# hjanime/recoup

Hardware: NVIDIA B200
Metric: reads/s through coverage + profileMatrix (reads -> per-base coverage -> regions x bins) (higher is better)
Workload: dtype int32 coverage / f64 matrix

## Files before the change

### recoup_b200/csrc/coverage_split.cu

```cuda
#include <algorithm>
#include <cstdlib>
#include <chrono>
#include <cstdio>

#include <type_traits>
#include <vector>

#include <cooperative_groups.h>

#include "cov_common.cuh"
#include "r_rng.cuh"
#include "rcp_internal.cuh"

namespace rcp {

using namespace covk;

namespace {

constexpr int BLK_SHIFT = 14;
#ifndef RCP_SUB_SHIFT
#define RCP_SUB_SHIFT 10
#endif
constexpr int SUB_SHIFT = RCP_SUB_SHIFT;
constexpr int NG = 1024;
constexpr int RING = 32;
constexpr int CH = 16;
#ifndef RCP_SPLIT_ST
#define RCP_SPLIT_ST 1024
#endif
constexpr int ST = RCP_SPLIT_ST;
constexpr int ROUND_VEC = 2048;
constexpr int VPT = ROUND_VEC / ST;
constexpr int SLAB = 64;
constexpr int MIN_P = 16, MAX_P = 22;
constexpr int GT = 1024;
constexpr int CS = 1024;
constexpr int WT = 7 * ROW;
constexpr int WT_ONE = SMALL_MAX;
static_assert(NG % ST == 0 && ROUND_VEC % ST == 0, "the flush phase maps thread t to the groups t, t + ST, ...");
static_assert(RING == 2 * CH, "a ring holds two chunks");
static_assert(SLAB >= 64, "one flush phase of a warp needs up to 64 chunks");

__device__ __forceinline__ void sp_mark_block(uint32_t* __restrict__ tab, uint32_t b) {
    atomicOr(tab + (b >> 4), 1u << (b & 15u));
    if (b > 0) atomicOr(tab + ((b - 1u) >> 4), 0x10000u << ((b - 1u) & 15u));
}

__global__ void __launch_bounds__(CTA)
sp_plan_kernel(int64_t R, const int32_t* __restrict__ chrom, const int32_t* __restrict__ start,
               const int32_t* __restrict__ end, const int8_t* __restrict__ strand,
               const uint32_t* __restrict__ chrom_off, const int64_t* __restrict__ chrom_len,
               int n_chrom, int ignore_strand, int strand_filter, uint32_t* __restrict__ gs_out,
               int32_t* __restrict__ plen, uint8_t* __restrict__ flags, int64_t* __restrict__ ntile,
               int64_t* __restrict__ padded, uint32_t* __restrict__ tab, unsigned int* __restrict__ err,
               unsigned long long* __restrict__ pstats ,
               unsigned long long* __restrict__ zero5 ) {
    const int64_t r = (int64_t)blockIdx.x * CTA + threadIdx.x;
    if (r < 5) zero5[r] = 0ull;
    unsigned long long my_len = 0;
    if (r < R) {
        const int st = strand ? (int)strand[r] : 0;
        uint32_t gs;
        int64_t L;
        const bool null = window_geometry(chrom[r], start[r], end[r], n_chrom, chrom_off, chrom_len,
                                          err, &gs, &L);
        const int32_t len = null ? 0 : (int32_t)L;
        gs_out[r] = gs;
        plen[r] = len;
        flags[r] = (uint8_t)((st < 0 ? 1u : 0u) | (class_mask(st, ignore_strand, strand_filter) << 1));
        ntile[r] = len > WT_ONE ? ((int64_t)len + WT - 1) / WT : (len > 0 ? 1 : 0);
        padded[r] = ((int64_t)len + PAD - 1) / PAD * PAD;
        my_len = (unsigned long long)len;
        if (len > 0) {
            const uint32_t b1 = (gs + (uint32_t)len - 1u) >> BLK_SHIFT;
            for (uint32_t b = gs >> BLK_SHIFT; b <= b1; b++) sp_mark_block(tab, b);
        }
    }
    unsigned long long my_max = my_len, my_inv = my_len ? 0x100000000ull - my_len : 0ull;
    for (int d = 16; d > 0; d >>= 1) {
        my_len += __shfl_xor_sync(0xffffffffu, my_len, d);
        my_max = max(my_max, __shfl_xor_sync(0xffffffffu, my_max, d));
        my_inv = max(my_inv, __shfl_xor_sync(0xffffffffu, my_inv, d));
    }
    if ((threadIdx.x & 31) == 0 && my_len) {
        atomicAdd(&pstats[0], my_len);
        atomicMax(&pstats[1], my_max);
        atomicMax(&pstats[2], my_inv);
    }
}

__device__ __forceinline__ int64_t sp_owner_of(const int64_t* __restrict__ off, int64_t R, int64_t t) {
    int64_t lo = 0, hi = R;
    while (hi - lo > 1) {
        const int64_t mid = lo + ((hi - lo) >> 1);
        if (__ldg(off + mid) <= t) lo = mid;
        else hi = mid;
    }
    return lo;
}

struct __align__(16) SpDesc {
    int64_t out;
    uint32_t c0;
    uint32_t n;
    int32_t tlen;
    uint32_t cts;
    uint32_t flags;
    uint32_t region;
};

__global__ void __launch_bounds__(CTA)
sp_tiles_kernel(int64_t R, int64_t T, const int64_t* __restrict__ off_tile, const uint32_t* __restrict__ gs,
                const int32_t* __restrict__ plen, const uint8_t* __restrict__ flags,
                const int64_t* __restrict__ cov_off ,
                const int32_t* __restrict__ edge, int n_bins,
                uint32_t max_w, uint32_t pmask, const uint32_t* __restrict__ boff, SpDesc* __restrict__ desc,
                uint32_t* __restrict__ tabs,
                const uint32_t* __restrict__ lxs, const uint32_t* __restrict__ lmax, uint32_t ln,
                uint2* __restrict__ lrange, unsigned long long* __restrict__ bound) {
    const int64_t t = (int64_t)blockIdx.x * CTA + threadIdx.x;
    const unsigned live = __ballot_sync(0xffffffffu, t < T);
    if (t >= T) return;
    const int64_t r = sp_owner_of(off_tile, R, t);
    const int L = plen[r];
    uint32_t o_lo = 0, tlen = (uint32_t)L;
    if (L > WT_ONE) {
        o_lo = (uint32_t)(t - off_tile[r]) * WT;
        tlen = (uint32_t)min(WT, L - (int)o_lo);
    }
    const uint32_t q0 = (flags[r] & 1u) ? (uint32_t)L - o_lo - tlen : o_lo;
    const uint32_t tstart = gs[r] + q0;
    const uint32_t first = tstart >= max_w ? tstart - max_w + 1u : 0u;
    SpDesc d;
    d.out = cov_off ? cov_off[r] + o_lo : (int64_t)o_lo;
    if (!cov_off) {
        int a = 0, b = n_bins;
        while (b - a > 1) {
            const int mid = (a + b) >> 1;
            if (__ldg(edge + mid) <= (int)o_lo) a = mid;
            else b = mid;
        }
        d.out |= (int64_t)a << 32;
    }
    d.c0 = __ldg(boff + (first >> SUB_SHIFT));
    d.n = __ldg(boff + ((tstart + tlen - 1u) >> SUB_SHIFT) + 1u) - d.c0;
    d.tlen = (int32_t)tlen;
    d.cts = tstart & pmask;
    d.flags = flags[r];
    d.region = (uint32_t)r;
    desc[t] = d;
    uint32_t most = d.n;
    if (ln) {
        tabs[t] = tstart;
        const uint32_t hi = tstart + tlen - 1u;
        uint32_t a = 0, b = ln;
        while (a < b) {
            const uint32_t mid = a + ((b - a) >> 1);
            if (__ldg(lxs + mid) < hi + 1u) a = mid + 1;
            else b = mid;
        }
        const uint32_t c1 = a;
        a = 0;
        b = c1;
        while (a < b) {
            const uint32_t mid = a + ((b - a) >> 1);
            if (__ldg(lmax + mid) < tstart + 1u) a = mid + 1;
            else b = mid;
        }
        lrange[t] = make_uint2(a, c1);
        most = most + (c1 - a) < most ? 0xffffffffu : most + (c1 - a);
    }
    if (bound) {
        most = __reduce_max_sync(live, most);
        if ((threadIdx.x & 31) == 0) atomicMax(bound, (unsigned long long)most);
    }
}

__device__ __forceinline__ uint2 lds64(uint32_t a) {
    uint2 v;
    asm volatile("ld.shared.v2.u32 {%0, %1}, [%2];" : "=r"(v.x), "=r"(v.y) : "r"(a));
    return v;
}
__device__ __forceinline__ uint32_t lds32(uint32_t a) {
    uint32_t v;
    asm volatile("ld.shared.u32 %0, [%1];" : "=r"(v) : "r"(a));
    return v;
}
__device__ __forceinline__ uint4 lds128(uint32_t a) {
    uint4 v;
    asm volatile("ld.shared.v4.u32 {%0, %1, %2, %3}, [%4];" : "=r"(v.x), "=r"(v.y), "=r"(v.z), "=r"(v.w) : "r"(a));
    return v;
}
__device__ __forceinline__ void sts32(uint32_t a, uint32_t v) {
    asm volatile("st.shared.u32 [%0], %1;" ::"r"(a), "r"(v) : "memory");
}
__device__ __forceinline__ void sts64(uint32_t a, uint32_t x, uint32_t y) {
    asm volatile("st.shared.v2.u32 [%0], {%1, %2};" ::"r"(a), "r"(x), "r"(y) : "memory");
}
__device__ __forceinline__ int lds_s8(uint32_t a) {
    int v;
    asm volatile("ld.shared.s8 %0, [%1];" : "=r"(v) : "r"(a));
    return v;
}
__device__ __forceinline__ void sts8(uint32_t a, int v) {
    asm volatile("st.shared.u8 [%0], %1;" ::"r"(a), "r"(v) : "memory");
}
__device__ __forceinline__ uint32_t atoms_add(uint32_t a, uint32_t v) {
    uint32_t old;
    asm volatile("atom.shared.add.u32 %0, [%1], %2;" : "=r"(old) : "r"(a), "r"(v) : "memory");
    return old;
}

struct SplitOut {
    uint32_t* pool;
    uint16_t* meta;
    uint32_t* pool_next;
};

constexpr size_t sp_split_smem(int words) {
    return (size_t)NG * RING * 4 + (size_t)NG * 4 + (size_t)words * 4;
}
constexpr size_t SP_SMEM_MAX = 232448;

template <bool STRANDED>
__global__ void __launch_bounds__(ST, 1)
sp_split_kernel(int64_t n, const uint32_t* __restrict__ g_start, const uint32_t* __restrict__ g_end1,
                const int8_t* __restrict__ strand, const uint32_t* __restrict__ tab_g, int words, int P,
                uint32_t max_pack_w, SplitOut out) {
    extern __shared__ __align__(16) unsigned char sp_smem[];
    const int tid = threadIdx.x;
    const unsigned lane = tid & 31, lt = (1u << lane) - 1u;
    const uint32_t ring_a = (uint32_t)__cvta_generic_to_shared(sp_smem);
    const uint32_t cnt_a = ring_a + NG * RING * 4;
    const uint32_t tab_a = cnt_a + NG * 4;
    for (int i = tid; i < words; i += ST) sts32(tab_a + i * 4, tab_g[i]);
    for (int i = tid; i < NG; i += ST) sts32(cnt_a + i * 4, 0u);
    __syncthreads();
    const uint32_t pmask = (1u << P) - 1u;
    const int wsh = STRANDED ? P + 2 : P;
    uint32_t slab_next = 0, slab_end = 0;
    uint32_t spare = 0;
    bool have_spare = false;
    bool hot = false;

    uint32_t a_rem = 0, a_old = 0, a_new = 0;
    auto alloc = [&](uint32_t total) {
        a_rem = slab_end - slab_next;
        a_old = slab_next;
        a_new = 0;
        if (total > a_rem) {
            if (!have_spare && lane == 0) spare = atomicAdd(out.pool_next, (uint32_t)SLAB);
            a_new = __shfl_sync(0xffffffffu, spare, 0);
            have_spare = false;
            slab_next = a_new + (total - a_rem);
            slab_end = a_new + SLAB;
        } else {
            slab_next += total;
        }
        if (!have_spare && slab_end - slab_next < (uint32_t)SLAB / 2) {
            if (lane == 0) spare = atomicAdd(out.pool_next, (uint32_t)SLAB);
            have_spare = true;
        }
    };
    auto chunk_at = [&](uint32_t i) { return i < a_rem ? a_old + i : a_new + (i - a_rem); };

    auto flush_phase = [&](bool final_pass) {
#pragma unroll 1
        for (int grp = tid; grp < NG; grp += ST) {
            const uint32_t w = lds32(cnt_a + grp * 4);
            const uint32_t raw = w & 0xffffu, start = w >> 16;
            const uint32_t nn = min(raw, (uint32_t)RING);
            const uint32_t k = final_pass ? (nn > 0u ? 1u : 0u) : nn / CH;
            const unsigned m1 = __ballot_sync(0xffffffffu, k >= 1u), m2 = __ballot_sync(0xffffffffu, k >= 2u);
            const uint32_t total = __popc(m1) + __popc(m2);
            if (total) {
                const uint32_t idx = __popc(m1 & lt) + __popc(m2 & lt);
                alloc(total);
                for (uint32_t j = 0; j < k; j++) {
                    const uint32_t c = chunk_at(idx + j);
                    const uint32_t src = ring_a + (uint32_t)grp * RING * 4 + (((start + CH * j) & (RING - 1)) << 2);
                    uint4* dst = reinterpret_cast<uint4*>(out.pool + (size_t)c * CH);
                    const uint4 a = lds128(src), b = lds128(src + 16), cc = lds128(src + 32), d = lds128(src + 48);
                    __stcs(dst, a);
                    __stcs(dst + 1, b);
                    __stcs(dst + 2, cc);
                    __stcs(dst + 3, d);
                    out.meta[c] = (uint16_t)(((uint32_t)grp << 5) | (final_pass ? nn : (uint32_t)CH));
                }
            }
            if (k || raw > (uint32_t)RING)
                sts32(cnt_a + grp * 4, final_pass ? 0u : ((((start + CH * k) & (RING - 1)) << 16) | (nn - CH * k)));
        }
    };

    auto keep_read = [&](uint32_t s, uint32_t e1) -> bool {
        const uint32_t t = lds32(tab_a + ((s >> (BLK_SHIFT + 2)) & 0xfffffffcu)) >> ((s >> BLK_SHIFT) & 15u);
        const bool cross = ((e1 - 1u) >> BLK_SHIFT) != (s >> BLK_SHIFT);
        return ((t & 1u) | (cross & ((t >> 16) & 1u))) & (e1 - s <= max_pack_w);
    };
    auto pack = [&](uint32_t s, uint32_t e1, int st) -> uint32_t {
        uint32_t word = (s & pmask) | ((e1 - s) << wsh);
        if (STRANDED) word |= (st > 0 ? 0u : (st < 0 ? 1u : 2u)) << P;
        return word;
    };
    auto insert = [&](uint32_t g, uint32_t pk) -> bool {
        const uint32_t old = atoms_add(cnt_a + g * 4, 1u);
        const uint32_t slot = old & 0xffffu;
        if (slot >= (uint32_t)RING) return false;
        sts32(ring_a + g * (RING * 4) + ((((old >> 16) + slot) & (RING - 1)) << 2), pk);
        return true;
    };
    auto direct = [&](bool want, uint32_t g, uint32_t pk) -> bool {
        const unsigned mo = __ballot_sync(0xffffffffu, want);
        if (mo == 0u) return want;
        const uint32_t g0 = __shfl_sync(0xffffffffu, g, __ffs(mo) - 1);
        const uint32_t nact = __popc(mo);
        if (nact < (uint32_t)CH || !__all_sync(0xffffffffu, !want || g == g0)) return want;
        const uint32_t nfull = nact / CH;
        alloc(nfull);
        const uint32_t r = __popc(mo & lt);
        if (want && r < nfull * CH) {
            const uint32_t c = chunk_at(r / CH);
            out.pool[(size_t)c * CH + (r & (CH - 1))] = pk;
            if ((r & (CH - 1)) == 0) out.meta[c] = (uint16_t)((g0 << 5) | (uint32_t)CH);
            return false;
        }
        return want;
    };

    constexpr int RPT = 4 * VPT;
    uint32_t fg[RPT], fp[RPT];
    uint32_t nf = 0;
    auto take = [&](uint32_t sv, uint32_t ev, int tv) {
        const uint32_t g = sv >> P, pk = pack(sv, ev, tv);
        bool want = keep_read(sv, ev);
        if (hot) want = direct(want, g, pk);
        if (want && !insert(g, pk)) {
            fg[nf] = g;
            fp[nf] = pk;
            nf++;
        }
    };
    auto finish_round = [&]() {
        for (;;) {
            hot = hot || __any_sync(0xffffffffu, nf != 0u);
            const int any = __syncthreads_or(nf != 0u);
            flush_phase(false);
            __syncthreads();
            if (!any) break;
            uint32_t mx = nf;
            for (int d = 16; d > 0; d >>= 1) mx = max(mx, __shfl_xor_sync(0xffffffffu, mx, d));
            uint32_t kept = 0;
            for (uint32_t i = 0; i < mx; i++) {
                const bool mine = i < nf;
                const uint32_t g = mine ? fg[i] : 0u, pk = mine ? fp[i] : 0u;
                bool want = mine;
                if (hot) want = direct(want, g, pk);
                if (want && !insert(g, pk)) {
                    fg[kept] = g;
                    fp[kept] = pk;
                    kept++;
                }
            }
            nf = kept;
        }
    };

    __shared__ int next_round[2];
    const int64_t n_vec = n >> 2;
    const int rounds = (int)((n_vec + ROUND_VEC - 1) / ROUND_VEC);
    if (tid == 0) {
        next_round[0] = (int)atomicAdd(out.pool_next + 1, 1u);
        next_round[1] = (int)atomicAdd(out.pool_next + 1, 1u);
    }
    __syncthreads();
    int round = next_round[0], nr = next_round[1];
    __syncthreads();
    uint4 s4[VPT], e4[VPT];
    char4 t4[VPT];
    auto load = [&](int rd, int h) {
        const int64_t v = (int64_t)rd * ROUND_VEC + h * ST + tid;
        s4[h] = e4[h] = make_uint4(0, 0, 0, 0);
        t4[h] = make_char4(0, 0, 0, 0);
        if (rd < rounds && v < n_vec) {
            s4[h] = __ldcs(reinterpret_cast<const uint4*>(g_start) + v);
            e4[h] = __ldcs(reinterpret_cast<const uint4*>(g_end1) + v);
            if (STRANDED && strand) t4[h] = __ldcs(reinterpret_cast<const char4*>(strand) + v);
        }
    };
#pragma unroll
    for (int h = 0; h < VPT; h++) load(round, h);
    for (int it = 0; round < rounds; it++) {
        unsigned after = 0;
        if (tid == 0) after = atomicAdd(out.pool_next + 1, 1u);
#pragma unroll
        for (int h = 0; h < VPT; h++) {
            take(s4[h].x, e4[h].x, t4[h].x);
            take(s4[h].y, e4[h].y, t4[h].y);
            take(s4[h].z, e4[h].z, t4[h].z);
            take(s4[h].w, e4[h].w, t4[h].w);
            load(nr, h);
        }
        if (tid == 0) next_round[it & 1] = (int)min(after, 0x7fffffffu);
        finish_round();
        round = nr;
        nr = next_round[it & 1];
    }
    if (blockIdx.x == 0) {
        const int64_t i = n_vec * 4 + tid;
        const bool in = i < n;
        const uint32_t sv = in ? g_start[i] : 0u, ev = in ? g_end1[i] : 0u;
        take(sv, ev, (in && STRANDED && strand) ? (int)strand[i] : 0);
        finish_round();
    }
    flush_phase(true);
}

__device__ __forceinline__ void sp_slot_range(uint32_t n_slots, uint32_t* lo, uint32_t* hi) {
    const uint32_t per = ((n_slots + gridDim.x - 1) / gridDim.x + CS - 1) / CS * CS;
    *lo = min(n_slots, blockIdx.x * per);
    *hi = min(n_slots, *lo + per);
}

__global__ void __launch_bounds__(CS)
sp_chunk_lists_kernel(const uint16_t* __restrict__ meta, const uint32_t* __restrict__ pool_next,
                      uint32_t* __restrict__ col , uint32_t* __restrict__ cb,
                      uint32_t* __restrict__ list ) {
    static_assert(CS == NG, "thread g of a CTA owns group g");
    __shared__ uint32_t h[NG];
    __shared__ uint32_t wsum[NG / 32];
    const int g = threadIdx.x;
    h[g] = 0;
    __syncthreads();
    uint32_t lo, hi;
    sp_slot_range(*pool_next, &lo, &hi);
    for (uint32_t i = lo + threadIdx.x; i < hi; i += CS) {
        const uint32_t m = meta[i];
        if (m & 31u) atomicAdd(&h[m >> 5], 1u);
    }
    __syncthreads();
    col[(size_t)blockIdx.x * NG + g] = h[g];
    cooperative_groups::this_grid().sync();
    uint32_t tot = 0, before = 0;
    for (unsigned c = 0; c < gridDim.x; c++) {
        const uint32_t v = __ldcg(col + (size_t)c * NG + g);
        tot += v;
        if (c < blockIdx.x) before += v;
    }
    uint32_t inc = tot;
    const unsigned lane = g & 31;
#pragma unroll
    for (int d = 1; d < 32; d <<= 1) {
        const uint32_t o = __shfl_up_sync(0xffffffffu, inc, d);
        if (lane >= (unsigned)d) inc += o;
    }
    if (lane == 31) wsum[g >> 5] = inc;
    __syncthreads();
    uint32_t run = inc - tot;
    for (int k = 0; k < (g >> 5); k++) run += wsum[k];
    if (blockIdx.x == 0) {
        cb[g] = run;
        if (g == NG - 1) cb[NG] = run + tot;
    }
    h[g] = run + before;
    __syncthreads();
    for (uint32_t i = lo + threadIdx.x; i < hi; i += CS) {
        const uint32_t m = meta[i];
        if (m & 31u) list[atomicAdd(&h[m >> 5], 1u)] = (i << 5) | (m & 31u);
    }
}

constexpr size_t GSMEM = 220 * 1024;

__global__ void __launch_bounds__(GT, 1)
sp_group_kernel(const uint32_t* __restrict__ pool, const uint32_t* __restrict__ list,
                const uint32_t* __restrict__ cb, int n_groups, int nb ,
                uint32_t pmask, uint32_t* __restrict__ cand, uint32_t* __restrict__ boff) {
    extern __shared__ __align__(16) uint32_t gsm[];
    uint32_t* h = gsm;
    uint32_t* out = gsm + nb;
    const uint32_t cap = (uint32_t)(GSMEM / 4) - (uint32_t)nb;
    __shared__ uint32_t wsum[GT / 32];
    const int tid = threadIdx.x, g = blockIdx.x;
    for (int i = tid; i < nb; i += GT) h[i] = 0;
    __syncthreads();
    const uint32_t c0 = cb[g], c1 = cb[g + 1];
    const uint32_t q4 = (tid & 3) * 4, cw = tid >> 2;
    constexpr uint32_t CPS = GT / 4, U = 4;
    auto stream = [&](auto&& use) {
        uint32_t le[U], ln[U];
        uint4 e[U];
#pragma unroll
        for (uint32_t u = 0; u < U; u++) {
            const uint32_t i = c0 + cw + u * CPS;
            ln[u] = i < c1 ? __ldg(list + i) : 0u;
        }
        for (uint32_t i0 = c0 + cw; i0 < c1; i0 += CPS * U) {
#pragma unroll
            for (uint32_t u = 0; u < U; u++) {
                le[u] = ln[u];
                e[u] = make_uint4(0u, 0u, 0u, 0u);
                if (q4 < (le[u] & 31u))
                    e[u] = __ldg(reinterpret_cast<const uint4*>(pool + (size_t)(le[u] >> 5) * CH + q4));
            }
#pragma unroll
            for (uint32_t u = 0; u < U; u++) {
                const uint32_t i = i0 + CPS * U + u * CPS;
                ln[u] = i < c1 ? __ldg(list + i) : 0u;
            }
#pragma unroll
            for (uint32_t u = 0; u < U; u++) {
                const uint32_t f = le[u] & 31u;
                use(e[u], q4 < f, q4 + 1 < f, q4 + 2 < f, q4 + 3 < f);
            }
        }
    };
    auto sub = [&](uint32_t e) { return (e & pmask) >> SUB_SHIFT; };
    stream([&](uint4 e, bool v0, bool v1, bool v2, bool v3) {
        if (v0) atomicAdd(&h[sub(e.x)], 1u);
        if (v1) atomicAdd(&h[sub(e.y)], 1u);
        if (v2) atomicAdd(&h[sub(e.z)], 1u);
        if (v3) atomicAdd(&h[sub(e.w)], 1u);
    });
    auto place = [&](uint32_t* dst) {
        stream([&](uint4 e, bool v0, bool v1, bool v2, bool v3) {
            uint32_t p0 = 0, p1 = 0, p2 = 0, p3 = 0;
            if (v0) p0 = atomicAdd(&h[sub(e.x)], 1u);
            if (v1) p1 = atomicAdd(&h[sub(e.y)], 1u);
            if (v2) p2 = atomicAdd(&h[sub(e.z)], 1u);
            if (v3) p3 = atomicAdd(&h[sub(e.w)], 1u);
            if (v0) dst[p0] = e.x;
            if (v1) dst[p1] = e.y;
            if (v2) dst[p2] = e.z;
            if (v3) dst[p3] = e.w;
        });
    };
    __syncthreads();
    constexpr int NW = GT / 32;
    const int pw = (nb + NW - 1) / NW;
    const unsigned lane = tid & 31;
    const int wb0 = (tid >> 5) * pw, wb1 = min(nb, wb0 + pw);
    uint32_t carry = 0;
    for (int b = wb0 + (int)lane; b - (int)lane < wb1; b += 32) {
        const uint32_t c = b < wb1 ? h[b] : 0u;
        uint32_t inc = c;
#pragma unroll
        for (int d = 1; d < 32; d <<= 1) {
            const uint32_t o = __shfl_up_sync(0xffffffffu, inc, d);
            if (lane >= (unsigned)d) inc += o;
        }
        if (b < wb1) h[b] = carry + inc - c;
        carry += __shfl_sync(0xffffffffu, inc, 31);
    }
    if (lane == 0) wsum[tid >> 5] = carry;
    __syncthreads();
    uint32_t wbase = 0, total = 0;
    for (int k = 0; k < NW; k++) {
        if (k < (tid >> 5)) wbase += wsum[k];
        total += wsum[k];
    }
    const uint32_t base = c0 * CH;
    for (int b = wb0 + (int)lane; b < wb1; b += 32) {
        const uint32_t o = h[b] + wbase;
        h[b] = o;
        boff[(size_t)g * nb + b] = base + o;
    }
    if (g == n_groups - 1 && tid == 0) boff[(size_t)n_groups * nb] = base + total;
    __syncthreads();
    if (total > cap) {
        place(cand + base);
        for (uint32_t i = base + total + tid; i < c1 * CH; i += GT) cand[i] = 0u;
        return;
    }
    place(out);
    const uint32_t full = (c1 - c0) * CH;
    for (uint32_t i = total + tid; i < min(full, (total + 3u) & ~3u); i += GT) out[i] = 0u;
    __syncthreads();
    const uint32_t n4 = (total + 3u) >> 2;
    uint4* dst = reinterpret_cast<uint4*>(cand + base);
    for (uint32_t i = tid; i < n4; i += GT) dst[i] = reinterpret_cast<const uint4*>(out)[i];
    for (uint32_t i = n4 * 4 + tid; i < full; i += GT) cand[base + i] = 0u;
}

struct LongIdx {
    uint32_t n;
    const uint32_t* xs;
    const uint32_t* e1;
    const int8_t* st;
    const uint32_t* maxe1;
};

constexpr int LONG_PER = CTA * 16;
__global__ void __launch_bounds__(CTA)
sp_long_collect_kernel(int64_t n, const uint32_t* __restrict__ s, const uint32_t* __restrict__ e1,
                       uint32_t max_pack_w, unsigned int* __restrict__ cursor_g, uint32_t cap,
                       uint32_t* __restrict__ keys, uint32_t* __restrict__ idx) {
    __shared__ unsigned cnt, cursor;
    if (threadIdx.x == 0) cnt = 0;
    __syncthreads();
    const unsigned lane = threadIdx.x & 31;
    const int64_t lo = (int64_t)blockIdx.x * LONG_PER, hi = min(n, lo + LONG_PER);
    unsigned c = 0;
    for (int64_t i = lo + threadIdx.x; i < hi; i += CTA) c += (e1[i] - s[i] > max_pack_w) && (e1[i] > s[i]);
    for (int d = 16; d > 0; d >>= 1) c += __shfl_xor_sync(0xffffffffu, c, d);
    if (lane == 0 && c) atomicAdd(&cnt, c);
    __syncthreads();
    if (cnt == 0) return;
    if (threadIdx.x == 0) cursor = atomicAdd(cursor_g, cnt);
    __syncthreads();
    for (int64_t b0 = lo + (threadIdx.x & ~31u); b0 < hi; b0 += CTA) {
        const int64_t i = b0 + lane;
        const bool is = i < hi && e1[i] - s[i] > max_pack_w && e1[i] > s[i];
        const unsigned m = __ballot_sync(0xffffffffu, is);
        if (m == 0u) continue;
        unsigned k = 0;
        if (lane == 0) k = atomicAdd(&cursor, (unsigned)__popc(m));
        k = __shfl_sync(0xffffffffu, k, 0) + __popc(m & ((1u << lane) - 1u));
        if (is && k < cap) {
            keys[k] = s[i];
            idx[k] = (uint32_t)i;
        }
    }
}

__global__ void __launch_bounds__(CTA)
sp_long_gather_kernel(uint32_t n, const uint32_t* __restrict__ idx, const uint32_t* __restrict__ e1,
                      const int8_t* __restrict__ st, uint32_t* __restrict__ o_e1, int8_t* __restrict__ o_st) {
    const uint32_t i = blockIdx.x * CTA + threadIdx.x;
    if (i >= n) return;
    o_e1[i] = e1[idx[i]];
    if (st) o_st[i] = st[idx[i]];
}

__device__ __forceinline__ uint32_t sp_lower_bound(const uint32_t* __restrict__ a, uint32_t lo, uint32_t hi, uint32_t v) {
    while (lo < hi) {
        const uint32_t mid = lo + ((hi - lo) >> 1);
        if (__ldg(a + mid) < v) lo = mid + 1;
        else hi = mid;
    }
    return lo;
}
__device__ __forceinline__ uint2 sp_long_range(const LongIdx& lg, uint32_t lo, uint32_t hi) {
    const uint32_t c1 = sp_lower_bound(lg.xs, 0, lg.n, hi + 1u);
    const uint32_t c0 = sp_lower_bound(lg.maxe1, 0, c1, lo + 1u);
    return make_uint2(c0, c1);
}

__device__ __forceinline__ SpDesc sp_load_desc(const SpDesc* __restrict__ p) {
    const int4 a = __ldg(reinterpret_cast<const int4*>(p));
    const int4 b = __ldg(reinterpret_cast<const int4*>(p) + 1);
    SpDesc d;
    d.out = (int64_t)(((uint64_t)(uint32_t)a.y << 32) | (uint32_t)a.x);
    d.c0 = (uint32_t)a.z;
    d.n = (uint32_t)a.w;
    d.tlen = b.x;
    d.cts = (uint32_t)b.y;
    d.flags = (uint32_t)b.z;
    d.region = (uint32_t)b.w;
    return d;
}

template <bool STRANDED>
__device__ __forceinline__ bool sp_apply(uint32_t e, const SpDesc& d, int P, int* diff) {
    const int sh = 32 - P;
    const int rel = ((int)((e - d.cts) << sh)) >> sh;
    uint32_t w = e >> (STRANDED ? P + 2 : P);
    if (STRANDED && !((d.flags >> (1u + ((e >> P) & 3u))) & 1u)) w = 0;
    int lo = max(rel, 0), hi = min(rel + (int)w, d.tlen);
    if (lo >= hi) return false;
    if (d.flags & 1u) {
        const int l2 = d.tlen - hi;
        hi = d.tlen - lo;
        lo = l2;
    }
    atomicAdd(diff + lo, 1);
    if (hi < d.tlen) atomicSub(diff + hi, 1);
    return true;
}

template <bool STRANDED, bool REV>
__device__ __forceinline__ bool sp_apply_fast(uint32_t e, uint32_t cts, int tlen, uint32_t cls, int P,
                                              uint32_t diff_a) {
    const int sh = 32 - P;
    const int rel = ((int)((e - cts) << sh)) >> sh;
    int w = (int)(e >> (STRANDED ? P + 2 : P));
    if (STRANDED) w = ((cls >> ((e >> P) & 3u)) & 1u) ? w : 0;
    const int lo = max(rel, 0), hi = min(rel + w, tlen);
    const int a = REV ? tlen - hi : lo;
    const int b = REV ? tlen - lo : hi;
    asm volatile(
        "{\n\t"
        ".reg .pred p, q;\n\t"
        "setp.lt.s32 p, %0, %1;\n\t"
        "setp.lt.and.s32 q, %2, %3, p;\n\t"
        "@p red.shared.add.s32 [%4], 1;\n\t"
        "@q red.shared.add.s32 [%5], -1;\n\t"
        "}" ::"r"(lo), "r"(hi), "r"(b), "r"(tlen), "r"(diff_a + (uint32_t)a * 4u), "r"(diff_a + (uint32_t)b * 4u)
        : "memory");
    return lo < hi;
}

template <int RPW, class O = int32_t>
__device__ __forceinline__ void warp_scan_store_fwd(int* diff, int tlen, O* __restrict__ dst) {
    const int lane = threadIdx.x & 31;
    int* mine = diff + lane * 4 * RPW;
    int4 v[RPW];
    int sum = 0;
#pragma unroll
    for (int k = 0; k < RPW; k++) {
        v[k] = *(reinterpret_cast<const int4*>(mine) + k);
        sum += (v[k].x + v[k].y) + (v[k].z + v[k].w);
    }
    const int inc = warp_inclusive_scan(sum);
    int run = inc - sum;
    if (sizeof(O) == 2) __syncwarp();
#pragma unroll
    for (int k = 0; k < RPW; k++) {
        int4 o;
// ... 302 lines not shown
    int32_t* xoff;
    uint2* lrange;
};

__global__ void __launch_bounds__(CTA)
sp_list_plan_kernel(int64_t G, ListPlan lp, const int32_t* __restrict__ chrom, const int32_t* __restrict__ start,
                    const int32_t* __restrict__ end, const uint32_t* __restrict__ chrom_off,
                    const int64_t* __restrict__ chrom_len, int n_chrom, int32_t* __restrict__ plen,
                    uint8_t* __restrict__ flags, int64_t* __restrict__ ntile, int64_t* __restrict__ padded,
                    unsigned int* __restrict__ err, unsigned long long* __restrict__ pstats, LongIdx lg) {
    const int64_t g = (int64_t)blockIdx.x * CTA + threadIdx.x;
    unsigned long long my_len = 0;
    if (g < G) {
        const int64_t a = lp.ptr[g], b = lp.ptr[g + 1];
        bool null = (b <= a);
        bool simple = true;
        int64_t L = 0;
        int st0 = 0;
        uint32_t lo = 0xffffffffu, hi = 0;
        if (!null) {
            const int c = chrom[a];
            st0 = lp.rstrand ? (int)lp.rstrand[a] : 0;
            if (c < 0 || c >= n_chrom) {
                atomicOr(err, 1u);
                null = true;
            } else {
                const int64_t clen = chrom_len[c];
                const uint32_t coff = chrom_off[c];
                int64_t prev_end = -1;
                for (int64_t i = a; i < b; i++) {
                    int64_t s = start[i], e = end[i];
                    if (s <= prev_end || e < s || (lp.rstrand && lp.rstrand[i] != lp.rstrand[a])) simple = false;
                    prev_end = e;
                    if (chrom[i] != c) atomicOr(err, 4u);
                    if (e < s - 1) { atomicOr(err, 2u); null = true; }
                    if (s < 0 || e > clen) null = true;
                    if (s == 0) s = 1;
                    int64_t w = e - s + 1;
                    if (w < 0) w = 0;
                    const uint32_t gs = coff + (uint32_t)(s > 0 ? s : 0);
                    lp.xgs[i] = gs;
                    lp.xge[i] = gs + (uint32_t)w - 1u;
                    lp.xoff[i] = (int32_t)L;
                    L += w;
                    if (w > 0) {
                        lo = min(lo, gs);
                        hi = max(hi, gs + (uint32_t)w - 1u);
                    }
                }
                if (L == 0 || L > 0x7fffffff) null = true;
            }
        }
        const int32_t len = null ? 0 : (int32_t)L;
        lp.lrange[g] = (lg.n && !null) ? sp_long_range(lg, lo, hi) : make_uint2(0u, 0u);
        plen[g] = len;
        flags[g] = (uint8_t)((st0 < 0 ? 1u : 0u) | (simple ? 2u : 0u));
        ntile[g] = len > WT_ONE ? ((int64_t)len + WT - 1) / WT : (len > 0 ? 1 : 0);
        padded[g] = ((int64_t)len + PAD - 1) / PAD * PAD;
        my_len = (unsigned long long)len;
    }
    unsigned long long my_max = my_len;
    for (int d = 16; d > 0; d >>= 1) {
        my_len += __shfl_xor_sync(0xffffffffu, my_len, d);
        my_max = max(my_max, __shfl_xor_sync(0xffffffffu, my_max, d));
    }
    if ((threadIdx.x & 31) == 0 && my_len) {
        atomicAdd(&pstats[0], my_len);
        atomicMax(&pstats[1], my_max);
    }
}

__device__ __forceinline__ int sp_multiplicity(const ListPlan& lp, int64_t a, int64_t b, int64_t q, bool simple,
                                               uint32_t rs, uint32_t re1, int rst, int ignore_strand,
                                               int strand_filter) {
    if (simple) {
        if (!strand_ok(rst, lp.rstrand ? (int)__ldg(lp.rstrand + a) : 0, ignore_strand, strand_filter)) return 0;
        int mult = 1;
        for (int64_t z = q + 1; z < b && __ldg(lp.xgs + z) < re1; z++) mult++;
        for (int64_t z = q - 1; z >= a && __ldg(lp.xge + z) >= rs; z--) mult++;
        return mult;
    }
    int mult = 0;
    for (int64_t z = a; z < b; z++) {
        const uint32_t zs = __ldg(lp.xgs + z), ze = __ldg(lp.xge + z);
        if (ze + 1u == zs) continue;
        if (rs <= ze && re1 > zs &&
            strand_ok(rst, lp.rstrand ? (int)__ldg(lp.rstrand + z) : 0, ignore_strand, strand_filter))
            mult++;
    }
    return mult;
}

__global__ void __launch_bounds__(CTA)
sp_list_tiles_kernel(int64_t G, int64_t T, const int64_t* __restrict__ off_tile, const int32_t* __restrict__ plen,
                     const uint8_t* __restrict__ flags, const int64_t* __restrict__ cov_off,
                     SpDesc* __restrict__ desc) {
    const int64_t t = (int64_t)blockIdx.x * CTA + threadIdx.x;
    if (t >= T) return;
    const int64_t g = sp_owner_of(off_tile, G, t);
    const int L = plen[g];
    uint32_t o_lo = 0, tlen = (uint32_t)L;
    if (L > WT_ONE) {
        o_lo = (uint32_t)(t - off_tile[g]) * WT;
        tlen = (uint32_t)min(WT, L - (int)o_lo);
    }
    SpDesc d;
    d.out = cov_off[g] + o_lo;
    d.c0 = d.n = 0;
    d.tlen = (int32_t)tlen;
    d.cts = (flags[g] & 1u) ? (uint32_t)L - o_lo - tlen : o_lo;
    d.flags = flags[g];
    d.region = (uint32_t)g;
    desc[t] = d;
}

template <bool STRANDED>
__global__ void __launch_bounds__(CTA, 4)
sp_ltile_kernel(int64_t T, const SpDesc* __restrict__ desc, ListPlan lp, const uint32_t* __restrict__ cand,
                const uint32_t* __restrict__ boff, int P, uint32_t max_w, int ignore_strand, int strand_filter,
                int32_t* __restrict__ cov, uint8_t* __restrict__ region_hit, LongIdx lg) {
    __shared__ __align__(16) int sm[WARPS][WT_ONE];
    const int warp = threadIdx.x >> 5;
    const uint32_t lane = threadIdx.x & 31;
    int* diff = sm[warp];
    const int64_t step = (int64_t)gridDim.x * WARPS;
    const int sh = 32 - P;
    const uint32_t pmask = (1u << P) - 1u;
    for (int64_t t = (int64_t)blockIdx.x * WARPS + warp; t < T; t += step) {
        const SpDesc d = sp_load_desc(desc + t);
        const int64_t a = lp.ptr[d.region], b = lp.ptr[d.region + 1];
        const int tlen = d.tlen, t0 = (int)d.cts, t1 = t0 + tlen;
        const bool rev = d.flags & 1u, simple = (d.flags & 2u) != 0;
        const int rows = (tlen + ROW - 1) / ROW;
        for (int k = 0; k < rows; k++) reinterpret_cast<int4*>(diff)[k * 32 + lane] = make_int4(0, 0, 0, 0);
        __syncwarp();
        int64_t qa = a, qb = b;
        while (qb - qa > 1) {
            const int64_t mid = (qa + qb) >> 1;
            if (__ldg(lp.xoff + mid) <= t0) qa = mid;
            else qb = mid;
        }
        bool hit = false;
        for (int64_t q = qa; q < b; q++) {
            const int xo = __ldg(lp.xoff + q);
            if (xo >= t1) break;
            const uint32_t s = __ldg(lp.xgs + q), e = __ldg(lp.xge + q);
            if (e + 1u == s) continue;
            const int w = (int)(e - s) + 1;
            const int k0 = max(xo, t0), k1 = min(xo + w, t1);
            if (k0 >= k1) continue;
            const uint32_t ps = s + (uint32_t)(k0 - xo), pe = s + (uint32_t)(k1 - 1 - xo);
            const uint32_t first = ps >= max_w ? ps - max_w + 1u : 0u;
            const uint32_t c0 = __ldg(boff + (first >> SUB_SHIFT)), c1 = __ldg(boff + (pe >> SUB_SHIFT) + 1);
            auto fetch = [&](uint32_t i0, uint32_t* wv) {
#pragma unroll
                for (int k = 0; k < 4; k++) {
                    const uint32_t i = i0 + (uint32_t)k * 32u + lane;
                    wv[k] = i < c1 ? __ldg(cand + i) : 0u;
                }
            };
            uint32_t wv[4], wn[4];
            if (c0 < c1) fetch(c0, wv);
            for (uint32_t i0 = c0; i0 < c1; i0 += 128) {
                if (i0 + 128 < c1) fetch(i0 + 128, wn);
#pragma unroll
                for (int k = 0; k < 4; k++) {
                    const uint32_t word = wv[k];
                    const int rel = ((int)((word - (ps & pmask)) << sh)) >> sh;
                    const uint32_t wd = word >> (STRANDED ? P + 2 : P);
                    if (wd == 0u) continue;
                    const int64_t rs64 = (int64_t)ps + rel;
                    const uint32_t rs = (uint32_t)rs64, re1 = rs + wd;
                    if (!(rs <= pe && re1 > ps)) continue;
                    int rst = 0;
                    if (STRANDED) {
                        const uint32_t cls = (word >> P) & 3u;
                        rst = cls == 0u ? 1 : (cls == 1u ? -1 : 0);
                    }
                    if (strand_filter != RCP_STRAND_ANY && rst != strand_filter) continue;
                    const int mult = sp_multiplicity(lp, a, b, q, simple, rs, re1, rst, ignore_strand, strand_filter);
                    if (mult == 0) continue;
                    hit = true;
                    const int ka = k0 + (int)(max(rs, ps) - ps) - t0;
                    const int kb1 = k0 + (int)(min(re1 - 1u, pe) - ps) + 1 - t0;
                    if (!rev) {
                        atomicAdd(diff + ka, mult);
                        if (kb1 < tlen) atomicSub(diff + kb1, mult);
                    } else {
                        atomicAdd(diff + (tlen - kb1), mult);
                        if (ka > 0) atomicSub(diff + (tlen - ka), mult);
                    }
                }
#pragma unroll
                for (int k = 0; k < 4; k++) wv[k] = wn[k];
            }
        }
        if (lg.n) {
            const uint2 lr = lp.lrange[d.region];
            for (uint32_t i = lr.x + lane; i < lr.y; i += 32) {
                const uint32_t rs = __ldg(lg.xs + i), re1 = __ldg(lg.e1 + i);
                const int rst = lg.st ? (int)__ldg(lg.st + i) : 0;
                if (strand_filter != RCP_STRAND_ANY && rst != strand_filter) continue;
                int mult = 0;
                for (int64_t z = a; z < b; z++) {
                    const uint32_t zs = __ldg(lp.xgs + z), ze = __ldg(lp.xge + z);
                    if (ze + 1u == zs) continue;
                    if (rs <= ze && re1 > zs &&
                        strand_ok(rst, lp.rstrand ? (int)__ldg(lp.rstrand + z) : 0, ignore_strand, strand_filter))
                        mult++;
                }
                if (mult == 0) continue;
                for (int64_t q = qa; q < b; q++) {
                    const int xo = __ldg(lp.xoff + q);
                    if (xo >= t1) break;
                    const uint32_t s = __ldg(lp.xgs + q), e = __ldg(lp.xge + q);
                    if (e + 1u == s || !(rs <= e && re1 > s)) continue;
                    const int pa = xo + (int)(max(rs, s) - s), pb = xo + (int)(min(re1 - 1u, e) - s);
                    if (pb < t0 || pa >= t1) continue;
                    const int ka = max(pa, t0) - t0, kb1 = min(pb, t1 - 1) + 1 - t0;
                    hit = true;
                    if (!rev) {
                        atomicAdd(diff + ka, mult);
                        if (kb1 < tlen) atomicSub(diff + kb1, mult);
                    } else {
                        atomicAdd(diff + (tlen - kb1), mult);
                        if (ka > 0) atomicSub(diff + (tlen - ka), mult);
                    }
                }
            }
        }
        hit = __any_sync(0xffffffffu, hit);
        __syncwarp();
        int32_t* dst = cov + d.out;
        switch (rows) {
            case 1: warp_scan_store_fwd<1>(diff, tlen, dst); break;
            case 2: warp_scan_store_fwd<2>(diff, tlen, dst); break;
            case 3: warp_scan_store_fwd<3>(diff, tlen, dst); break;
            case 4: warp_scan_store_fwd<4>(diff, tlen, dst); break;
            case 5: warp_scan_store_fwd<5>(diff, tlen, dst); break;
            case 6: warp_scan_store_fwd<6>(diff, tlen, dst); break;
            case 7: warp_scan_store_fwd<7>(diff, tlen, dst); break;
            default: {
                int pre = 0;
                for (int row = 0; row < rows; row++)
                    pre += warp_row_scan_store(diff + row * ROW, pre, 0, false, tlen - row * ROW, dst + row * ROW);
            }
        }
        if (hit && lane == 0) region_hit[d.region] = 1;
        if (lane == 0) tma_store_wait_read();
        __syncwarp();
    }
}

__global__ void __launch_bounds__(CTA)
sp_null_kernel(int64_t R, const int32_t* __restrict__ plen, const uint8_t* __restrict__ region_hit,
               const uint32_t* __restrict__ cb, int32_t* __restrict__ len, uint8_t* __restrict__ is_null,
               unsigned long long* __restrict__ stats ) {
    const int64_t r = (int64_t)blockIdx.x * CTA + threadIdx.x;
    unsigned long long my_null = 0, my_len = 0;
    if (r < R) {
        const bool null = plen[r] == 0 || region_hit[r] == 0;
        const int32_t out = null ? 0 : plen[r];
        len[r] = out;
        is_null[r] = null ? 1 : 0;
        my_null = null ? 1 : 0;
        my_len = (unsigned long long)out;
    }
    unsigned long long my_max = my_len;
    for (int d = 16; d > 0; d >>= 1) {
        my_null += __shfl_xor_sync(0xffffffffu, my_null, d);
        my_len += __shfl_xor_sync(0xffffffffu, my_len, d);
        my_max = max(my_max, __shfl_xor_sync(0xffffffffu, my_max, d));
    }
    if ((threadIdx.x & 31) == 0) {
        if (my_null) atomicAdd(&stats[0], my_null);
        if (my_len) atomicAdd(&stats[1], my_len);
        if (my_max) atomicMax(&stats[2], my_max);
    }
    if (r == 0) stats[3] = (unsigned long long)cb[NG] * CH;
}

}

struct DebugLap {
    bool on;
    std::chrono::steady_clock::time_point t0;
    explicit DebugLap() : on(getenv("RCP_DEBUG_TIMING") != nullptr), t0(std::chrono::steady_clock::now()) {}
    void lap(const char* what) {
        if (!on) return;
        cudaStreamSynchronize(g_ctx.stream);
        const auto now = std::chrono::steady_clock::now();
        fprintf(stderr, "[rcp split] %-32s %8.3f ms\n", what, std::chrono::duration<double, std::milli>(now - t0).count());
        t0 = now;
    }
};

struct SortedCands {
    uint32_t* cand = nullptr;
    uint32_t* boff = nullptr;
    uint32_t* cb = nullptr;
};

static int split_and_sort(ReadsIdx& rd, const uint32_t* tab, int words, int P, int n_groups, bool stranded,
                          bool st_arr, uint32_t max_pack_w, Arena& K, Arena& B, SortedCands* sc) {
    const int nb = 1 << (P - SUB_SHIFT);
    const uint32_t pmask = (1u << P) - 1u;
    const int split_grid = g_ctx.sm_count;
    const int sort_grid = 64;
    const size_t pool_cap = (size_t)(rd.n / CH + 1) + (size_t)split_grid * NG +
                            (size_t)split_grid * (ST / 32) * SLAB * 2 + SLAB;
    RCP_TRY(K.reserve(Arena::pad(pool_cap * CH * 4) + Arena::pad((NG + 1) * 4) +
                      Arena::pad(((size_t)n_groups * nb + 1) * 4)));
    sc->cand = K.take<uint32_t>(pool_cap * CH);
    sc->cb = K.take<uint32_t>(NG + 1);
    sc->boff = K.take<uint32_t>((size_t)n_groups * nb + 1);
    RCP_TRY(B.reserve(Arena::pad(pool_cap * CH * 4) + Arena::pad(pool_cap * 2) + Arena::pad(pool_cap * 4) +
                      Arena::pad(16) + Arena::pad((size_t)sort_grid * NG * 4)));
    uint32_t* pool_next = B.take<uint32_t>(4);
    uint16_t* meta = B.take<uint16_t>(pool_cap);
    const size_t zero_b = B.used;
    uint32_t* pool = B.take<uint32_t>(pool_cap * CH);
    uint32_t* list = B.take<uint32_t>(pool_cap);
    uint32_t* col = B.take<uint32_t>((size_t)sort_grid * NG);
    if (B.used > B.cap || K.used > K.cap) return fail(RCP_ERR_CUDA, "internal: split arena overrun");
    DebugLap dbg;
    dbg.lap("  split_and_sort: arenas");
    {
        StageTimer t(ST_SP_SPLIT);
        RCP_CUDA(cudaMemsetAsync(B.base, 0, zero_b, g_ctx.stream));
        const size_t smem = sp_split_smem(words);
        SplitOut out = {pool, meta, pool_next};
        if (stranded) {
            RCP_CUDA(cudaFuncSetAttribute(sp_split_kernel<true>, cudaFuncAttributeMaxDynamicSharedMemorySize, (int)smem));
            sp_split_kernel<true><<<split_grid, ST, smem, g_ctx.stream>>>(rd.n, rd.g_start, rd.g_end1,
                                                                         st_arr ? rd.d_strand : nullptr, tab, words, P,
                                                                         max_pack_w, out);
        } else {
            RCP_CUDA(cudaFuncSetAttribute(sp_split_kernel<false>, cudaFuncAttributeMaxDynamicSharedMemorySize, (int)smem));
            sp_split_kernel<false><<<split_grid, ST, smem, g_ctx.stream>>>(rd.n, rd.g_start, rd.g_end1, nullptr, tab,
                                                                          words, P, max_pack_w, out);
        }
        RCP_LAUNCHED();
    }
    dbg.lap("  split_and_sort: split kernel");
    {
        StageTimer t(ST_SP_SORT);
        {
            const uint16_t* a_meta = meta;
            const uint32_t* a_next = pool_next;
            void* args[] = {(void*)&a_meta, (void*)&a_next, (void*)&col, (void*)&sc->cb, (void*)&list};
            RCP_CUDA(cudaLaunchCooperativeKernel((const void*)sp_chunk_lists_kernel, dim3((unsigned)sort_grid), dim3(CS),
                                                 args, 0, g_ctx.stream));
            RCP_LAUNCHED();
        }
        dbg.lap("  split_and_sort: chunk lists");
        RCP_CUDA(cudaFuncSetAttribute(sp_group_kernel, cudaFuncAttributeMaxDynamicSharedMemorySize, (int)GSMEM));
        sp_group_kernel<<<n_groups, GT, GSMEM, g_ctx.stream>>>(pool, list, sc->cb, n_groups, nb, pmask, sc->cand,
                                                               sc->boff);
        RCP_LAUNCHED();
    }
    dbg.lap("  split_and_sort: group sort");
    return RCP_OK;
}

struct SplitGeom {
    int words, P, n_groups, nb;
    uint32_t pmask;
    bool ok;
};
static SplitGeom split_geometry(const ReadsIdx& rd) {
    SplitGeom g;
    const int64_t span = (int64_t)rd.chrom_off[(size_t)rd.n_chrom];
    g.words = (int)((span >> (BLK_SHIFT + 4)) + 2);
    g.P = MIN_P;
    while (g.P < MAX_P && ((span + (1ll << g.P) - 1) >> g.P) > NG) g.P++;
    g.n_groups = (int)std::max<int64_t>(1, (span + (1ll << g.P) - 1) >> g.P);
    g.nb = 1 << (g.P - SUB_SHIFT);
    g.pmask = (1u << g.P) - 1u;
    g.ok = g.n_groups <= NG && rd.n < 0x7ffffff0ll && sp_split_smem(g.words) <= SP_SMEM_MAX;
    return g;
}

static LongIdx long_index(const ReadsIdx& rd) {
    LongIdx lg;
    lg.n = (uint32_t)rd.ln_n;
    lg.xs = rd.ln_xs;
    lg.e1 = rd.ln_e1;
    lg.st = rd.ln_st;
    lg.maxe1 = rd.ln_maxe1;
    return lg;
}

static int reads_build_binned(ReadsIdx& rd) {
    if (rd.bn_cand) return RCP_OK;
    DebugLap dbg;
    RCP_TRY(reads_resolve(rd));
    dbg.lap("binned: resolve reads");
    const SplitGeom g = split_geometry(rd);
    const bool stranded = rd.d_strand != nullptr;
    const int wbits = 32 - g.P - (stranded ? 2 : 0);
    if (!g.ok || wbits < 7) return RCP_SPLIT_NOT_APPLICABLE;
    const uint32_t max_pack_w = std::min<uint32_t>((1u << wbits) - 1u, 8191u);
    rd.bn_max_pack_w = max_pack_w;
    if (rd.max_width > max_pack_w) {
        if (rd.long_thr != max_pack_w) return RCP_SPLIT_NOT_APPLICABLE;
        if (rd.n_long > rd.n / 8) return RCP_SPLIT_NOT_APPLICABLE;
        const size_t n = (size_t)rd.n_long;
        uint32_t* idx = nullptr;
        unsigned int* d_cur = nullptr;
        RCP_TRY(dalloc(&d_cur, 1));
        RCP_CUDA(cudaMemsetAsync(d_cur, 0, 4, g_ctx.stream));
        RCP_TRY(dalloc(&rd.ln_xs, n));
        RCP_TRY(dalloc(&rd.ln_e1, n));
        RCP_TRY(dalloc(&rd.ln_maxe1, n));
        if (rd.d_strand) RCP_TRY(dalloc(&rd.ln_st, n));
        RCP_TRY(dalloc(&idx, n));
        sp_long_collect_kernel<<<(unsigned)blocks_for(rd.n, LONG_PER), CTA, 0, g_ctx.stream>>>(
            rd.n, rd.g_start, rd.g_end1, max_pack_w, d_cur, (uint32_t)n, rd.ln_xs, idx);
        RCP_LAUNCHED();
        dfree(d_cur);
        dbg.lap("  long: collect");
        RCP_TRY(sort_pairs_u32(rd.ln_xs, idx, (int64_t)n, rd.key_bits));
        dbg.lap("  long: sort");
        if (n > 0) {
            sp_long_gather_kernel<<<blocks_for((int64_t)n, CTA), CTA, 0, g_ctx.stream>>>((uint32_t)n, idx, rd.g_end1,
                                                                                        rd.d_strand, rd.ln_e1, rd.ln_st);
            RCP_LAUNCHED();
        }
        RCP_TRY(running_max_u32_device(rd.ln_e1, rd.ln_maxe1, (int64_t)n));
        rd.ln_n = (int64_t)n;
        dfree(idx);
        dbg.lap("binned: long-read list");
    }
    Arena K, B, Tb;
    RCP_TRY(Tb.reserve(Arena::pad((size_t)g.words * 4)));
    uint32_t* tab = Tb.take<uint32_t>((size_t)g.words);
    RCP_CUDA(cudaMemsetAsync(tab, 0xff, (size_t)g.words * 4, g_ctx.stream));
    SortedCands sc;
    RCP_TRY(split_and_sort(rd, tab, g.words, g.P, g.n_groups, stranded, stranded, max_pack_w, K, B, &sc));
    rd.bn_base = K.base;
    K.base = nullptr;
    rd.bn_cand = sc.cand;
    rd.bn_boff = sc.boff;
    rd.bn_cb = sc.cb;
    rd.bn_P = g.P;
    rd.bn_stranded = stranded;
    dbg.lap("binned: split + sort");
    return RCP_OK;
}

struct FusedReq {
    int n_bins, seed, sample_kind;
    double scale;
    double* d_out;
    int64_t ld;
    uint8_t* d_is_null;
};

static int split_impl(ReadsIdx& rd, int64_t R, const int32_t* chrom, const int32_t* start,
                      const int32_t* end, const int8_t* strand, int ignore_strand,
                      int strand_filter, int mem, Coverage* cv, const FusedReq* fz) {
    const bool stranded = !((strand_filter == RCP_STRAND_ANY) && (ignore_strand || strand == nullptr));
    const bool st_arr = stranded && rd.d_strand != nullptr;
    const int64_t span = (int64_t)rd.chrom_off[(size_t)rd.n_chrom];
    const int words = (int)((span >> (BLK_SHIFT + 4)) + 2);
    int P = MIN_P;
    while (P < MAX_P && ((span + (1ll << P) - 1) >> P) > NG) P++;
    const int n_groups = (int)std::max<int64_t>(1, (span + (1ll << P) - 1) >> P);
    const int wbits = 32 - P - (stranded ? 2 : 0);
    if (n_groups > NG || rd.n >= 0x7ffffff0ll || sp_split_smem(words) > SP_SMEM_MAX)
        return RCP_SPLIT_NOT_APPLICABLE;
    const bool have_index = rd.bn_cand && rd.bn_P == P && (rd.bn_stranded || !stranded);
    if (!have_index && !rd.pending && (rd.max_width > 8191u || rd.max_width >= (1u << wbits)))
        return RCP_SPLIT_NOT_APPLICABLE;
    const uint32_t pmask = (1u << P) - 1u;

    DevIn<int32_t> d_chrom, d_start, d_end;
    DevIn<int8_t> d_strand;
    RCP_TRY(d_chrom.init(chrom, (size_t)R, mem));
    RCP_TRY(d_start.init(start, (size_t)R, mem));
    RCP_TRY(d_end.init(end, (size_t)R, mem));
    RCP_TRY(d_strand.init(strand, (size_t)R, mem));

    Arena A;
    const size_t r = (size_t)R;
    RCP_TRY(A.reserve(Arena::pad(64) + Arena::pad((size_t)words * 4) + Arena::pad(r * 4) * 2 + Arena::pad(r) * 2 +
                      Arena::pad(r * 8) * 2 + Arena::pad((r + 1) * 8)));
    unsigned int* err = A.take<unsigned int>(16);
    unsigned long long* pstats = reinterpret_cast<unsigned long long*>(err + 4);
    uint32_t* tab = A.take<uint32_t>((size_t)words);
    uint8_t* region_hit = A.take<uint8_t>(r);
    const size_t zero_bytes = A.used;
    uint32_t* gs = A.take<uint32_t>(r);
    int32_t* plen = A.take<int32_t>(r);
    uint8_t* flags = A.take<uint8_t>(r);
    int64_t* ntile = A.take<int64_t>(r);
    int64_t* padded = A.take<int64_t>(r);
    int64_t* off_tile = A.take<int64_t>(r + 1);
    if (A.used > A.cap) return fail(RCP_ERR_CUDA, "internal: split plan arena overrun");

    cv->n_regions = R;
    RCP_TRY(dalloc(&cv->off, r + 1));
    RCP_TRY(dalloc(&cv->len, r));
    RCP_TRY(dalloc(&cv->is_null, r));
    RCP_TRY(dalloc(&cv->d_stats, 5));
    auto give_up = [&]() {
        dfree(cv->off);
        dfree(cv->len);
        dfree(cv->is_null);
        dfree(cv->d_stats);
        return RCP_SPLIT_NOT_APPLICABLE;
    };
    {
        StageTimer t(ST_SP_PLAN);
        RCP_CUDA(cudaMemsetAsync(A.base, 0, zero_bytes, g_ctx.stream));
        if (R == 0) RCP_CUDA(cudaMemsetAsync(cv->d_stats, 0, 40, g_ctx.stream));
        if (R > 0) {
            sp_plan_kernel<<<blocks_for(R, CTA), CTA, 0, g_ctx.stream>>>(
                R, d_chrom.ptr, d_start.ptr, d_end.ptr, d_strand.ptr, rd.d_chrom_off, rd.d_chrom_len,
                rd.n_chrom, ignore_strand, strand_filter, gs, plen, flags, ntile, padded, tab, err,
                pstats, cv->d_stats);
            RCP_LAUNCHED();
        }
        RCP_TRY(exclusive_scan2_i64(ntile, off_tile, off_tile + R, padded, cv->off, cv->off + R, R));
    }
    struct Host {
        int64_t T, total_padded;
        unsigned long long pstats[3];
        unsigned int err;
    } h = {0, 0, {0, 0, 0}, 0};
    Arena K, B;
    SortedCands sc;
    {
        FetchItem items[8] = {{off_tile + R, &h.T, 8}, {cv->off + R, &h.total_padded, 8}, {pstats, h.pstats, 24},
                              {err, &h.err, 4}};
        int n_items = 4;
        reads_pending_items(rd, items, &n_items);
        RCP_TRY(fetch_begin(items, n_items));
        if (!have_index) RCP_TRY(split_and_sort(rd, tab, words, P, n_groups, stranded, st_arr, 0xffffffffu, K, B, &sc));
        RCP_TRY(fetch_end(items, n_items));
        RCP_TRY(reads_finish(rd));
    }
    if (h.err & 1u) return fail(RCP_ERR_DATA, "a region has a chromosome id outside [0, n_chrom)");
    if (h.err & 2u) return fail(RCP_ERR_DATA, "a region has end < start - 1");
    const int64_t T = h.T;
    if (T > 0x7fffffff) return fail(RCP_ERR_UNSUPPORTED, "more than 2^31-1 coverage tiles");
    const uint32_t max_w = have_index ? std::max(1u, std::min(rd.max_width, rd.bn_max_pack_w))
                                      : (rd.max_width > 0 ? rd.max_width : 1u);
    if (!have_index && (max_w > 8191u || max_w >= (1u << wbits))) return give_up();

    FusedBins fb = {nullptr, 0, R, nullptr};
    Arena F;
    if (fz) {
        const int64_t max_len = (int64_t)h.pstats[1];
        const int64_t min_len = h.pstats[2] ? 0x100000000ll - (int64_t)h.pstats[2] : 0;
        const int n = fz->n_bins;
        if (max_len != min_len || (max_len > 0 && max_len < n)) return give_up();
        const int64_t Lc = max_len > 0 ? max_len : n;
        std::vector<int32_t> edge((size_t)n + 1);
        {
            std::vector<int> perm((size_t)n), scratch((size_t)n), rank((size_t)n);
            RRng* rng = new RRng;
            rng->seed((uint32_t)fz->seed, fz->sample_kind);
            rng->sample(n, n, scratch.data(), perm.data());
            delete rng;
            for (int pos = 0; pos < n; pos++) rank[(size_t)perm[(size_t)pos] - 1] = pos + 1;
            const int64_t b = Lc / n, d = Lc - b * n;
            int64_t at = 0;
            for (int i = 0; i < n; i++) {
                edge[(size_t)i] = (int32_t)at;
                at += b + (rank[(size_t)i] <= d ? 1 : 0);
            }
            edge[(size_t)n] = (int32_t)at;
        }
        RCP_TRY(F.reserve(Arena::pad(((size_t)n + 1) * 4) + Arena::pad((size_t)n * r * 8)));
        int32_t* d_edge = F.take<int32_t>((size_t)n + 1);
        fb.acc = F.take<unsigned long long>((size_t)n * r);
        RCP_CUDA(cudaMemcpyAsync(d_edge, edge.data(), ((size_t)n + 1) * 4, cudaMemcpyHostToDevice, g_ctx.stream));
        RCP_CUDA(cudaMemsetAsync(fb.acc, 0, (size_t)n * r * 8, g_ctx.stream));
        fb.edge = d_edge;
        fb.n = n;
    } else {
        cv->path = RCP_PATH_SPLIT;
        cv->total_padded = h.total_padded;
        cv->total_len = (int64_t)h.pstats[0];
        cv->max_len = (int32_t)h.pstats[1];
        cv->n_null = 0;
        cv->stats_pending = true;
        RCP_TRY(dalloc(&cv->cov, (size_t)h.total_padded));
        if (getenv("RCP_COVERAGE_WIDE") == nullptr) cv->d_bound = cv->d_stats + 4;
    }
    unsigned long long* bound = cv->d_bound ? cv->d_stats + 4 : nullptr;

    bool words_stranded = stranded;
    if (have_index) {
        sc.cand = rd.bn_cand;
        sc.boff = rd.bn_boff;
        sc.cb = rd.bn_cb;
        words_stranded = rd.bn_stranded;
    }
    uint32_t* cand = sc.cand;
    uint32_t* boff = sc.boff;
    uint32_t* cb = sc.cb;
    LongIdx lg = long_index(rd);
    if (!have_index) lg.n = 0;
    Arena D;
    RCP_TRY(D.reserve(Arena::pad((size_t)(T + 1) * sizeof(SpDesc)) + (lg.n ? Arena::pad((size_t)(T + 1) * 4) +
                                                                            Arena::pad((size_t)(T + 1) * 8) : 0)));
    SpDesc* desc = D.take<SpDesc>((size_t)T + 1);
    uint32_t* tabs = lg.n ? D.take<uint32_t>((size_t)T + 1) : nullptr;
    uint2* lrange = lg.n ? D.take<uint2>((size_t)T + 1) : nullptr;
    if (T > 0) {
        StageTimer t(ST_SP_PLAN);
        sp_tiles_kernel<<<blocks_for(T, CTA), CTA, 0, g_ctx.stream>>>(R, T, off_tile, gs, plen, flags,
                                                                     fz ? nullptr : cv->off, fb.edge, fb.n, max_w, pmask, boff,
                                                                     desc, tabs,
                                                                     lg.xs, lg.maxe1, lg.n, lrange, bound);
        RCP_LAUNCHED();
    }
    if (T > 0) {
        {
            StageTimer t(fz ? ST_FUSED : ST_SP_TILE);
            const int64_t want = blocks_for(T, WARPS);
            auto launch = [&](auto kern) -> int {
                int per_sm = 0;
                RCP_CUDA(cudaFuncSetAttribute(kern, cudaFuncAttributeMaxDynamicSharedMemorySize, (int)WTILE_SMEM));
                RCP_CUDA(cudaOccupancyMaxActiveBlocksPerMultiprocessor(&per_sm, kern, CTA, WTILE_SMEM));
                per_sm = std::max(per_sm, 1);
                kern<<<(unsigned)std::min<int64_t>(want, (int64_t)g_ctx.sm_count * per_sm), CTA, WTILE_SMEM,
                       g_ctx.stream>>>(
                    T, desc, cand, P, cv->cov, region_hit, fb, lg, tabs, lrange, bound);
                RCP_LAUNCHED();
                return RCP_OK;
            };
            if (fz) RCP_TRY(words_stranded ? launch(sp_wtile_kernel<true, true>) : launch(sp_wtile_kernel<false, true>));
            else RCP_TRY(words_stranded ? launch(sp_wtile_kernel<true, false>) : launch(sp_wtile_kernel<false, false>));
        }
    }
    if (fz) {
        if (R > 0) {
            StageTimer t(ST_FUSED);
            sp_bins_finish_kernel<<<dim3(blocks_for(R, CTA), (unsigned)fb.n), CTA, 0, g_ctx.stream>>>(
                fb, plen, region_hit, fz->scale, fz->d_out, fz->ld, fz->d_is_null);
            RCP_LAUNCHED();
        }
        return RCP_OK;
    }
    if (R > 0) {
        StageTimer t(ST_SP_PLAN);
        sp_null_kernel<<<blocks_for(R, CTA), CTA, 0, g_ctx.stream>>>(R, plen, region_hit, cb, cv->len, cv->is_null,
                                                                    cv->d_stats);
        RCP_LAUNCHED();
    }
    return RCP_OK;
}

int coverage_ranges_split(ReadsIdx& rd, int64_t R, const int32_t* chrom, const int32_t* start,
                          const int32_t* end, const int8_t* strand, int ignore_strand,
                          int strand_filter, int mem, Coverage* cv) {
    return split_impl(rd, R, chrom, start, end, strand, ignore_strand, strand_filter, mem, cv, nullptr);
}

int coverage_profile_split(ReadsIdx& rd, int64_t R, const int32_t* chrom, const int32_t* start,
                           const int32_t* end, const int8_t* strand, int ignore_strand,
                           int strand_filter, int mem, int n_bins, int seed, int sample_kind,
                           double scale, double* d_out, int64_t ld, uint8_t* d_is_null) {
    if (n_bins < 1 || n_bins > 30000) return RCP_SPLIT_NOT_APPLICABLE;
    Coverage scratch;
    const FusedReq fz = {n_bins, seed, sample_kind, scale, d_out, ld, d_is_null};
    const int rc = split_impl(rd, R, chrom, start, end, strand, ignore_strand, strand_filter, mem, &scratch, &fz);
    coverage_release(scratch);
    return rc;
}

int coverage_list_split(ReadsIdx& rd, int64_t G, const int64_t* ptr, int64_t n_ranges, const int32_t* chrom,
                        const int32_t* start, const int32_t* end, const int8_t* strand, int ignore_strand,
                        int strand_filter, int mem, Coverage* cv) {
    DebugLap dbg;
    {
        const int rc = reads_build_binned(rd);
        if (rc != RCP_OK) return rc;
    }
    dbg.lap("list: binned index");
    const SplitGeom g = split_geometry(rd);
    const uint32_t max_w = std::max(1u, std::min(rd.max_width, rd.bn_max_pack_w));
    const LongIdx lg = long_index(rd);
    DevIn<int64_t> d_ptr;
    DevIn<int32_t> d_chrom, d_start, d_end;
    DevIn<int8_t> d_strand;
    RCP_TRY(d_ptr.init(ptr, (size_t)G + 1, mem));
    RCP_TRY(d_chrom.init(chrom, (size_t)n_ranges, mem));
    RCP_TRY(d_start.init(start, (size_t)n_ranges, mem));
    RCP_TRY(d_end.init(end, (size_t)n_ranges, mem));
    RCP_TRY(d_strand.init(strand, (size_t)n_ranges, mem));
    Arena A;
    const size_t r = (size_t)G, nr = (size_t)n_ranges;
    RCP_TRY(A.reserve(Arena::pad(64) + Arena::pad(r) * 2 + Arena::pad(r * 4) + Arena::pad(r * 8) * 3 +
                      Arena::pad((r + 1) * 8) + Arena::pad(nr * 4) * 3));
    unsigned int* err = A.take<unsigned int>(16);
    unsigned long long* pstats = reinterpret_cast<unsigned long long*>(err + 4);
    uint8_t* region_hit = A.take<uint8_t>(r);
    const size_t zero_bytes = A.used;
    uint8_t* flags = A.take<uint8_t>(r);
    int32_t* plen = A.take<int32_t>(r);
    int64_t* ntile = A.take<int64_t>(r);
    int64_t* padded = A.take<int64_t>(r);
    int64_t* off_tile = A.take<int64_t>(r + 1);
    ListPlan lp;
    lp.ptr = d_ptr.ptr;
    lp.rstrand = d_strand.ptr;
    lp.xgs = A.take<uint32_t>(nr);
    lp.xge = A.take<uint32_t>(nr);
    lp.xoff = A.take<int32_t>(nr);
    lp.lrange = A.take<uint2>(r);
    if (A.used > A.cap) return fail(RCP_ERR_CUDA, "internal: list plan arena overrun");
    cv->n_regions = G;
    RCP_TRY(dalloc(&cv->off, r + 1));
    RCP_TRY(dalloc(&cv->len, r));
    RCP_TRY(dalloc(&cv->is_null, r));
    RCP_TRY(dalloc(&cv->d_stats, 4));
    struct Host {
        int64_t T, total_padded;
        unsigned long long pstats[2];
        unsigned int err;
    } h = {0, 0, {0, 0}, 0};
    {
        StageTimer t(ST_COV_LIST);
        RCP_CUDA(cudaMemsetAsync(A.base, 0, zero_bytes, g_ctx.stream));
        RCP_CUDA(cudaMemsetAsync(cv->d_stats, 0, 32, g_ctx.stream));
        if (G > 0) {
            sp_list_plan_kernel<<<blocks_for(G, CTA), CTA, 0, g_ctx.stream>>>(
                G, lp, d_chrom.ptr, d_start.ptr, d_end.ptr, rd.d_chrom_off, rd.d_chrom_len, rd.n_chrom, plen, flags,
                ntile, padded, err, pstats, lg);
            RCP_LAUNCHED();
        }
        RCP_TRY(exclusive_scan2_i64(ntile, off_tile, off_tile + G, padded, cv->off, cv->off + G, G));
        const FetchItem items[4] = {{off_tile + G, &h.T, 8}, {cv->off + G, &h.total_padded, 8}, {pstats, h.pstats, 16},
                                    {err, &h.err, 4}};
        RCP_TRY(fetch_and_sync(items, 4));
    }
    dbg.lap("list: plan + fetch");
    if (h.err & 1u) return fail(RCP_ERR_DATA, "a range has a chromosome id outside [0, n_chrom)");
    if (h.err & 2u) return fail(RCP_ERR_DATA, "a range has end < start - 1");
    if (h.err & 4u) return fail(RCP_ERR_DATA, "the ranges of one list element lie on different chromosomes");
    const int64_t T = h.T;
    if (T > 0x7fffffff) return fail(RCP_ERR_UNSUPPORTED, "more than 2^31-1 coverage tiles");
    cv->path = 0;
    cv->total_padded = h.total_padded;
    cv->total_len = (int64_t)h.pstats[0];
    cv->max_len = (int32_t)h.pstats[1];
    cv->n_null = 0;
    cv->stats_pending = true;
    RCP_TRY(dalloc(&cv->cov, (size_t)h.total_padded));
    Arena D;
    RCP_TRY(D.reserve(Arena::pad((size_t)(T + 1) * sizeof(SpDesc))));
    SpDesc* desc = D.take<SpDesc>((size_t)T + 1);
    StageTimer t(ST_COV_LIST);
    if (T > 0) {
        sp_list_tiles_kernel<<<blocks_for(T, CTA), CTA, 0, g_ctx.stream>>>(G, T, off_tile, plen, flags, cv->off, desc);
        RCP_LAUNCHED();
        const unsigned grid = (unsigned)std::min<int64_t>(blocks_for(T, WARPS), (int64_t)g_ctx.sm_count * 4);
        if (rd.bn_stranded)
            sp_ltile_kernel<true><<<grid, CTA, 0, g_ctx.stream>>>(T, desc, lp, rd.bn_cand, rd.bn_boff, g.P, max_w,
                                                                 ignore_strand, strand_filter, cv->cov, region_hit, lg);
        else
            sp_ltile_kernel<false><<<grid, CTA, 0, g_ctx.stream>>>(T, desc, lp, rd.bn_cand, rd.bn_boff, g.P, max_w,
                                                                  ignore_strand, strand_filter, cv->cov, region_hit, lg);
        RCP_LAUNCHED();
    }
    if (G > 0) {
        sp_null_kernel<<<blocks_for(G, CTA), CTA, 0, g_ctx.stream>>>(G, plen, region_hit, rd.bn_cb, cv->len, cv->is_null,
                                                                    cv->d_stats);
        RCP_LAUNCHED();
    }
    dbg.lap("list: tiles");
    return RCP_OK;
}

}
```

### recoup_b200/csrc/import.cu

```cuda
#include <cstring>
#include <map>
#include <memory>
#include <string>
#include <vector>
#include <algorithm>

#include "cov_common.cuh"
#include "rcp_internal.cuh"

namespace rcp {

using namespace covk;

namespace {

struct Decoded {
    int64_t n = 0;
    int32_t* chrom = nullptr;
    int32_t* start = nullptr;
    int32_t* end = nullptr;
    int8_t* strand = nullptr;
};
std::map<int, std::unique_ptr<Decoded>> g_decoded;
int g_next_decoded = 1 << 20;
// ... 706 lines not shown
                                                                             wh, chunk_base, out, err);
        RCP_LAUNCHED();
        return RCP_OK;
    });
}

}

void decoded_release_all() {
    for (auto& kv : g_decoded) decoded_release(*kv.second);
    g_decoded.clear();
}

}

using namespace rcp;

extern "C" {

int rcp_bam_index(const uint8_t* rec, int64_t n_bytes, int64_t* n_records_out, int64_t* offsets_out,
                  int64_t capacity) {
    if (n_bytes < 0 || (n_bytes > 0 && rec == nullptr) || n_records_out == nullptr)
        return fail(RCP_ERR_ARG, "rcp_bam_index: bad argument");
    int64_t p = 0, n = 0;
    while (p < n_bytes) {
        if (n_bytes - p < 4) return fail(RCP_ERR_DATA, "BAM records: truncated block_size at byte %lld", (long long)p);
        int32_t bs;
        memcpy(&bs, rec + p, 4);
        if (bs < 32 || (int64_t)bs + 4 > n_bytes - p)
            return fail(RCP_ERR_DATA, "BAM records: record %lld at byte %lld has block_size %d", (long long)n,
                        (long long)p, (int)bs);
        if (offsets_out) {
            if (n + 1 >= capacity)
                return fail(RCP_ERR_ARG, "rcp_bam_index: offsets_out has %lld entries, the file more records", (long long)capacity);
            offsets_out[n] = p;
        }
        p += 4 + (int64_t)bs;
        n++;
    }
    if (offsets_out) {
        if (capacity < 1) return fail(RCP_ERR_ARG, "rcp_bam_index: offsets_out needs records + 1 entries");
        offsets_out[n] = p;
    }
    *n_records_out = n;
    return RCP_OK;
}

int rcp_bam_decode(const uint8_t* rec, int64_t n_bytes, const int64_t* offsets, int64_t n_records, int n_ref,
                   const int64_t* ref_len, int splice_split, int mem, int* decoded_out, int64_t* n_out) {
    RCP_TRY(bam_check_args("rcp_bam_decode", rec, n_bytes, offsets, n_records, n_ref, ref_len, mem, decoded_out, n_out));
    DevIn<uint8_t> d_rec;
    DevIn<int64_t> d_off, d_len;
    RCP_TRY(d_rec.init(rec, (size_t)n_bytes, mem));
    RCP_TRY(d_off.init(offsets, (size_t)n_records + 1, mem));
    RCP_TRY(d_len.init(ref_len, (size_t)std::max(n_ref, 1), RCP_MEM_HOST));
    return bam_decode_file_order<false>(d_rec.ptr, n_bytes, d_off.ptr, n_records, n_ref, d_len.ptr,
                                        splice_split ? 1 : 0, Filter{}, decoded_out, n_out);
}

int rcp_bam_decode_param(const uint8_t* rec, int64_t n_bytes, const int64_t* offsets, int64_t n_records, int n_ref,
                         const int64_t* ref_len, int splice_split, int mem, const int32_t* flag, int mapq_min,
                         int simple_cigar, int n_which, const int32_t* which_ref, const int32_t* which_start,
                         const int32_t* which_end, int n_tags, const char* tag_names, const int32_t* tag_ptr,
                         const int32_t* tag_type, const int64_t* int_values, const char* const* str_values,
                         int* decoded_out, int64_t* n_out) {
    RCP_TRY(bam_check_args("rcp_bam_decode_param", rec, n_bytes, offsets, n_records, n_ref, ref_len, mem,
                           decoded_out, n_out));
    Filter f = {};
    f.keep0 = flag ? (uint32_t)flag[0] : 0xfffu;
    f.keep1 = flag ? (uint32_t)flag[1] : 0xfffu;
    f.mapq_min = mapq_min;
    f.simple_cigar = simple_cigar ? 1 : 0;
    if (n_tags < 0 || n_tags > 32) return fail(RCP_ERR_UNSUPPORTED, "tagFilter: %d tags (at most 32)", n_tags);
    if (n_tags > 0 && (tag_names == nullptr || tag_ptr == nullptr || tag_type == nullptr))
        return fail(RCP_ERR_ARG, "rcp_bam_decode_param: bad tag filter");
    std::vector<Tag> tags((size_t)n_tags);
    std::vector<int64_t> ival;
    std::vector<uint32_t> soff(1, 0);
    std::string sbytes;
    for (int k = 0; k < n_tags; k++) {
        const int32_t a = tag_ptr[k], b = tag_ptr[k + 1];
        if (a < 0 || b < a || (k == 0 && a != 0) || (tag_type[k] != 0 && tag_type[k] != 1))
            return fail(RCP_ERR_ARG, "rcp_bam_decode_param: bad tag filter (tag %d)", k);
        Tag& t = tags[(size_t)k];
        t.name = (uint32_t)(uint8_t)tag_names[2 * k] | ((uint32_t)(uint8_t)tag_names[2 * k + 1] << 8);
        t.is_str = (uint32_t)tag_type[k];
        if (t.is_str) {
            t.v0 = (uint32_t)(soff.size() - 1);
            for (int32_t j = a; j < b; j++) {
                if (str_values == nullptr || str_values[j] == nullptr)
                    return fail(RCP_ERR_ARG, "rcp_bam_decode_param: tag %d: NULL string value", k);
                sbytes += str_values[j];
                soff.push_back((uint32_t)sbytes.size());
            }
            t.v1 = (uint32_t)(soff.size() - 1);
        } else {
            if (b > a && int_values == nullptr) return fail(RCP_ERR_ARG, "rcp_bam_decode_param: int_values is NULL");
            t.v0 = (uint32_t)ival.size();
            for (int32_t j = a; j < b; j++) ival.push_back(int_values[j]);
            t.v1 = (uint32_t)ival.size();
        }
    }
    std::vector<uint32_t> table;
    if (n_tags > 0) {
        const size_t w_tags = 4 * (size_t)n_tags, w_int = 2 * ival.size(), w_str = soff.size() + (sbytes.size() + 3) / 4;
        if ((w_tags + w_int + w_str) * 4 > 32768)
            return fail(RCP_ERR_UNSUPPORTED, "tagFilter: the filter values take more than 32 KB");
        table.assign(w_tags + w_int + w_str, 0u);
        memcpy(table.data(), tags.data(), w_tags * 4);
        memcpy(table.data() + w_tags, ival.data(), w_int * 4);
        memcpy(table.data() + w_tags + w_int, soff.data(), soff.size() * 4);
        memcpy(table.data() + w_tags + w_int + soff.size(), sbytes.data(), sbytes.size());
        f.n_tags = n_tags;
        f.n_int = (int)ival.size();
        f.n_str = (int)soff.size() - 1;
        f.table_words = (int)table.size();
    }
    if (n_which < 0 || (n_which > 0 && (which_ref == nullptr || which_start == nullptr || which_end == nullptr)))
        return fail(RCP_ERR_ARG, "rcp_bam_decode_param: bad which ranges");
    const size_t W = (size_t)n_which;
    std::vector<int32_t> wtab;
    if (n_which > 0) {
        wtab.assign(5 * W + (size_t)n_ref + 1, 0);
        std::vector<int32_t> cnt((size_t)n_ref + 1, 0);
        for (size_t i = 0; i < W; i++) {
            const int32_t c = which_ref[i], s = which_start[i], e = which_end[i];
            if (c < 0 || c >= n_ref)
                return fail(RCP_ERR_ARG, "which: range %zu is on reference %d, the header has %d", i, (int)c, n_ref);
            if (s < 1 || e < s || e > 536870912)
                return fail(RCP_ERR_ARG, "which: range %zu [%d, %d] needs 1 <= start <= end <= 536870912", i, (int)s,
                            (int)e);
            wtab[i] = c;
            wtab[W + i] = s;
            wtab[2 * W + i] = e;
            cnt[(size_t)c + 1]++;
        }
        int32_t* ref_off = wtab.data() + 5 * W;
        for (int c = 0; c < n_ref; c++) ref_off[c + 1] = ref_off[c] + cnt[(size_t)c + 1];
        std::vector<int32_t> fill(ref_off, ref_off + n_ref);
        for (size_t i = 0; i < W; i++) {
            const int32_t at = fill[(size_t)wtab[i]]++;
            wtab[3 * W + (size_t)at] = wtab[W + i];
            wtab[4 * W + (size_t)at] = wtab[2 * W + i];
        }
        for (int c = 0; c < n_ref; c++) {
            std::sort(wtab.begin() + 3 * W + ref_off[c], wtab.begin() + 3 * W + ref_off[c + 1]);
            std::sort(wtab.begin() + 4 * W + ref_off[c], wtab.begin() + 4 * W + ref_off[c + 1]);
        }
    }
    DevIn<uint8_t> d_rec;
    DevIn<int64_t> d_off, d_len;
    DevIn<uint32_t> d_table;
    RCP_TRY(d_rec.init(rec, (size_t)n_bytes, mem));
    RCP_TRY(d_off.init(offsets, (size_t)n_records + 1, mem));
    RCP_TRY(d_len.init(ref_len, (size_t)std::max(n_ref, 1), RCP_MEM_HOST));
    RCP_TRY(d_table.init(table.empty() ? nullptr : table.data(), table.size(), RCP_MEM_HOST));
    f.table = d_table.ptr;
    const int split = splice_split ? 1 : 0;
    if (n_which == 0)
        return bam_decode_file_order<true>(d_rec.ptr, n_bytes, d_off.ptr, n_records, n_ref, d_len.ptr, split, f,
                                           decoded_out, n_out);
    return bam_decode_which(d_rec.ptr, n_bytes, d_off.ptr, n_records, n_ref, d_len.ptr, split, f, wtab, n_which,
                            decoded_out, n_out);
}

int rcp_bed_decode(const char* text, int64_t n_bytes, int n_names, const char* const* names, int mem,
                   int* decoded_out, int64_t* n_out) {
    RCP_TRY(require_ready());
    if (n_bytes < 0 || (n_bytes > 0 && text == nullptr) || n_names < 1 || names == nullptr ||
        decoded_out == nullptr || n_out == nullptr)
        return fail(RCP_ERR_ARG, "rcp_bed_decode: bad argument");
    if (mem != RCP_MEM_HOST && mem != RCP_MEM_DEVICE) return fail(RCP_ERR_ARG, "bad mem kind");
    std::vector<int32_t> order((size_t)n_names);
    for (int i = 0; i < n_names; i++) {
        if (names[i] == nullptr) return fail(RCP_ERR_ARG, "rcp_bed_decode: names[%d] is NULL", i);
        order[(size_t)i] = i;
    }
    std::sort(order.begin(), order.end(), [&](int32_t x, int32_t y) {
        const size_t lx = strlen(names[x]), ly = strlen(names[y]);
        const int c = memcmp(names[x], names[y], std::min(lx, ly));
        return c != 0 ? c < 0 : lx < ly;
    });
    std::string blob;
    std::vector<int32_t> noff((size_t)n_names + 1);
    for (int i = 0; i < n_names; i++) {
        noff[(size_t)i] = (int32_t)blob.size();
        blob += names[order[(size_t)i]];
        if (i > 0 && blob.compare((size_t)noff[(size_t)i - 1], (size_t)(noff[(size_t)i] - noff[(size_t)i - 1]),
                                  names[order[(size_t)i]]) == 0)
            return fail(RCP_ERR_ARG, "rcp_bed_decode: seqlevel '%s' appears twice", names[order[(size_t)i]]);
    }
    noff[(size_t)n_names] = (int32_t)blob.size();
    const size_t padded = ((size_t)n_bytes + 15) / 16 * 16 + 16;
    uint8_t* d_text = nullptr;
    RCP_TRY(dalloc(&d_text, padded));
    struct Free {
        uint8_t*& p;
        ~Free() { dfree(p); }
    } free_text{d_text};
    if (n_bytes > 0)
        RCP_CUDA(cudaMemcpyAsync(d_text, text, (size_t)n_bytes,
                                 mem == RCP_MEM_HOST ? cudaMemcpyHostToDevice : cudaMemcpyDeviceToDevice, g_ctx.stream));
    const int64_t n_vec = (n_bytes + 15) / 16;
    const unsigned blocks = std::max(1u, blocks_for(n_vec, CTA));
    Arena A;
    RCP_TRY(A.reserve(Arena::pad(16) + Arena::pad(((size_t)blocks + 1) * 4) * 2 + Arena::pad(blob.size() + 1) +
                      Arena::pad(((size_t)n_names + 1) * 4) * 2));
    unsigned int* err = A.take<unsigned int>(4);
    uint32_t* bcnt = A.take<uint32_t>((size_t)blocks + 1);
    uint32_t* bbase = A.take<uint32_t>((size_t)blocks + 1);
    char* d_blob = A.take<char>(blob.size() + 1);
    int32_t* d_noff = A.take<int32_t>((size_t)n_names + 1);
    int32_t* d_id = A.take<int32_t>((size_t)n_names + 1);
    RCP_CUDA(cudaMemsetAsync(err, 0, 16, g_ctx.stream));
    RCP_CUDA(cudaMemcpyAsync(d_blob, blob.data(), blob.size(), cudaMemcpyHostToDevice, g_ctx.stream));
    RCP_CUDA(cudaMemcpyAsync(d_noff, noff.data(), noff.size() * 4, cudaMemcpyHostToDevice, g_ctx.stream));
    RCP_CUDA(cudaMemcpyAsync(d_id, order.data(), order.size() * 4, cudaMemcpyHostToDevice, g_ctx.stream));
    bed_nl_count_kernel<<<blocks, CTA, 0, g_ctx.stream>>>(reinterpret_cast<const uint4*>(d_text), n_bytes, bcnt);
    RCP_LAUNCHED();
    RCP_TRY(exclusive_scan_u32(bcnt, bbase, (int64_t)blocks, err + 1));
    unsigned int h_nl = 0;
    uint8_t last = '\n';
    {
        FetchItem it[1] = {{err + 1, &h_nl, 4}};
        RCP_TRY(fetch_and_sync(it, 1));
        if (n_bytes > 0) {
            RCP_CUDA(cudaMemcpyAsync(&last, d_text + n_bytes - 1, 1, cudaMemcpyDeviceToHost, g_ctx.stream));
            RCP_CUDA(cudaStreamSynchronize(g_ctx.stream));
        }
    }
    const int64_t n_nl = (int64_t)h_nl, n_lines = n_nl + ((n_bytes > 0 && last != '\n') ? 1 : 0);
    if (n_lines >= 0x7ffffff0ll) return fail(RCP_ERR_UNSUPPORTED, "more than 2^31 - 17 lines");
    Arena B;
    RCP_TRY(B.reserve(Arena::pad(((size_t)n_nl + 2) * 8) + Arena::pad(((size_t)n_lines + 1) * 4) * 2));
    int64_t* starts = B.take<int64_t>((size_t)n_nl + 2);
    uint32_t* counts = B.take<uint32_t>((size_t)n_lines + 1);
    uint32_t* where = B.take<uint32_t>((size_t)n_lines + 1);
    bed_nl_write_kernel<<<blocks, CTA, 0, g_ctx.stream>>>(reinterpret_cast<const uint4*>(d_text), n_bytes, bbase, starts);
    RCP_LAUNCHED();
    const NameTable nt = {d_blob, d_noff, d_id, n_names};
    const Out none = {nullptr, nullptr, nullptr, nullptr};
    if (n_lines > 0) {
        bed_lines_kernel<false><<<blocks_for(n_lines, CTA), CTA, 0, g_ctx.stream>>>(d_text, n_bytes, starts, n_nl, n_lines,
                                                                                  nt, counts, nullptr, none, err);
        RCP_LAUNCHED();
        RCP_TRY(exclusive_scan_u32(counts, where, n_lines, err + 2));
    }
    unsigned int h_err = 0, h_total = 0;
    FetchItem items[2] = {{err, &h_err, 4}, {err + 2, &h_total, 4}};
    RCP_TRY(fetch_and_sync(items, 2));
    if (h_err & 1u) return fail(RCP_ERR_DATA, "BED: a chromosome name is not among the %d seqlevels", n_names);
    if (h_err & 2u) return fail(RCP_ERR_DATA, "BED: a data line has fewer than three fields or a bad coordinate");
    if (h_err & 4u) return fail(RCP_ERR_DATA, "BED: a strand field is not one of + - . *");
    Decoded* d;
    int h;
    RCP_TRY(new_decoded(&d, &h));
    int rc = alloc_out(*d, (int64_t)h_total);
    if (rc == RCP_OK && n_lines > 0) {
        const Out out = {d->chrom, d->start, d->end, d->strand};
        bed_lines_kernel<true><<<blocks_for(n_lines, CTA), CTA, 0, g_ctx.stream>>>(d_text, n_bytes, starts, n_nl, n_lines, nt,
                                                                                 nullptr, where, out, err);
        g_ctx.launches++;
        if (cudaGetLastError() != cudaSuccess) rc = fail(RCP_ERR_CUDA, "bed_lines_kernel launch failed");
    }
    if (rc != RCP_OK) {
        decoded_release(*d);
        g_decoded.erase(h);
        return rc;
    }
    *decoded_out = h;
    *n_out = (int64_t)h_total;
    return RCP_OK;
}

int rcp_decoded_fetch(int decoded, int32_t* chrom, int32_t* start, int32_t* end, int8_t* strand, int64_t capacity) {
    RCP_TRY(require_ready());
    auto it = g_decoded.find(decoded);
    if (it == g_decoded.end()) return fail(RCP_ERR_HANDLE, "unknown decoded handle %d", decoded);
    const Decoded& d = *it->second;
    if (capacity < d.n) return fail(RCP_ERR_ARG, "rcp_decoded_fetch: capacity %lld < %lld ranges", (long long)capacity, (long long)d.n);
    const size_t n = (size_t)d.n;
    if (n == 0) return RCP_OK;
    if (chrom) RCP_CUDA(cudaMemcpyAsync(chrom, d.chrom, n * 4, cudaMemcpyDeviceToHost, g_ctx.stream));
    if (start) RCP_CUDA(cudaMemcpyAsync(start, d.start, n * 4, cudaMemcpyDeviceToHost, g_ctx.stream));
    if (end) RCP_CUDA(cudaMemcpyAsync(end, d.end, n * 4, cudaMemcpyDeviceToHost, g_ctx.stream));
    if (strand) RCP_CUDA(cudaMemcpyAsync(strand, d.strand, n, cudaMemcpyDeviceToHost, g_ctx.stream));
    RCP_CUDA(cudaStreamSynchronize(g_ctx.stream));
    return RCP_OK;
}

int rcp_decoded_free(int decoded) {
    auto it = g_decoded.find(decoded);
    if (it == g_decoded.end()) return fail(RCP_ERR_HANDLE, "unknown decoded handle %d", decoded);
    decoded_release(*it->second);
    g_decoded.erase(it);
    return RCP_OK;
}

int rcp_reads_load_decoded(int decoded, int n_chrom, const int64_t* chrom_len, int frag_len, int* reads_out) {
    RCP_TRY(require_ready());
    auto it = g_decoded.find(decoded);
    if (it == g_decoded.end()) return fail(RCP_ERR_HANDLE, "unknown decoded handle %d", decoded);
    const Decoded& d = *it->second;
    return rcp_reads_load(d.n, d.chrom, d.start, d.end, d.strand, n_chrom, chrom_len, frag_len, RCP_MEM_DEVICE,
                          reads_out);
}

int rcp_decoded_width_quantile(int decoded, double prob, double* quantile_out, int64_t* n_le_out) {
    RCP_TRY(require_ready());
    auto it = g_decoded.find(decoded);
    if (it == g_decoded.end()) return fail(RCP_ERR_HANDLE, "unknown decoded handle %d", decoded);
    const Decoded& d = *it->second;
    return rcp_reads_width_quantile(d.n, d.start, d.end, prob, RCP_MEM_DEVICE, quantile_out, n_le_out);
}

int rcp_reads_load_decoded_select(int decoded, double max_width, int64_t k, const int32_t* idx, int n_chrom,
                                  const int64_t* chrom_len, int frag_len, int64_t* n_kept_out, int* reads_out) {
    RCP_TRY(require_ready());
    auto it = g_decoded.find(decoded);
    if (it == g_decoded.end()) return fail(RCP_ERR_HANDLE, "unknown decoded handle %d", decoded);
    if (k < 0 || (k > 0 && idx == nullptr)) return fail(RCP_ERR_ARG, "rcp_reads_load_decoded_select: bad index");
    const Decoded& d = *it->second;
    DevIn<int32_t> d_idx;
    RCP_TRY(d_idx.init(idx, (size_t)k, RCP_MEM_HOST));
    return rcp_reads_load_select(d.n, d.chrom, d.start, d.end, d.strand, max_width, k, d_idx.ptr, n_chrom, chrom_len,
                                 frag_len, RCP_MEM_DEVICE, n_kept_out, reads_out);
}

}
```

### recoup_b200/csrc/index.cu

```cuda
#include <algorithm>
#include <chrono>
#include <cstdio>
#include <cstdlib>

#include "rcp_internal.cuh"

namespace rcp {

namespace {

constexpr int TPB = 256;

struct ExcBuf {
    uint32_t* xw;
    uint32_t* e1;
    int8_t* st;
    uint32_t cap;
    unsigned int* count;
    uint32_t* w_out;
};

__device__ __forceinline__ bool map_read(int c, int64_t s, int64_t e, int st, int n_chrom,
                                         const uint32_t* __restrict__ chrom_off,
                                         const int64_t* __restrict__ chrom_len, int frag_len,
                                         uint32_t* gs, uint32_t* ge1, unsigned int* err) {
    if (c < 0 || c >= n_chrom) { *err |= 1u; return false; }
    if (s < 1 || e < s) { *err |= 2u; return false; }
    const int64_t len = chrom_len[c];
    if (frag_len > 0) {
        if (st < 0) s = e - frag_len + 1;
        else e = s + frag_len - 1;
    }
    if (s < 1) s = 1;
    if (e > len) e = len;
    if (s > len || e < s) { *err |= 4u; return false; }
    *gs = chrom_off[c] + (uint32_t)s;
    *ge1 = chrom_off[c] + (uint32_t)e + 1u;
    return true;
}

__global__ void __launch_bounds__(TPB)
chrom_max_end_kernel(int64_t n, const int32_t* __restrict__ chrom, const int32_t* __restrict__ start,
                     const int32_t* __restrict__ end, const int8_t* __restrict__ strand, int n_chrom,
                     int frag_len, int fixed_width, unsigned long long* __restrict__ max_end) {
    const int64_t stride = (int64_t)gridDim.x * TPB;
    int last_c = -1;
    long long best = 0;
    for (int64_t i = (int64_t)blockIdx.x * TPB + threadIdx.x; i < n; i += stride) {
        const int c = chrom[i];
        if (c < 0 || c >= n_chrom) continue;
        const long long s = start[i];
        long long e = end ? (long long)end[i] : s + fixed_width - 1;
        if (frag_len > 0 && !(strand && strand[i] < 0)) e = s + frag_len - 1;
        if (c != last_c) {
            if (last_c >= 0 && best > 0) atomicMax(max_end + last_c, (unsigned long long)best);
            last_c = c;
            best = 0;
        }
        best = max(best, e);
    }
    if (last_c >= 0 && best > 0) atomicMax(max_end + last_c, (unsigned long long)best);
}

template <int VEC, bool HAS_END>
__global__ void __launch_bounds__(TPB)
reads_to_global_kernel(int64_t n, const int32_t* __restrict__ chrom,
                       const int32_t* __restrict__ start, const int32_t* __restrict__ end,
                       const int8_t* __restrict__ strand, const uint32_t* __restrict__ chrom_off,
                       const int64_t* __restrict__ chrom_len, int n_chrom, int frag_len,
                       int fixed_width ,
                       uint32_t long_thr ,
                       uint32_t* __restrict__ g_start, uint32_t* __restrict__ g_end1,
                       uint32_t* __restrict__ xs_out, int8_t* __restrict__ strand_out,
                       unsigned int* __restrict__ err, unsigned long long* __restrict__ cls_count,
                       ExcBuf exc) {
    unsigned int my_err = 0;
    unsigned int np = 0, nm = 0, ns = 0, wmax = 0, nlong = 0;
    bool exc_full = false;
    uint32_t w = (uint32_t)frag_len;
    if (frag_len <= 0) {
        uint32_t a = 0, b = 0;
        unsigned int e0 = 0;
        if (map_read(chrom[0], start[0], HAS_END ? (int64_t)end[0] : (int64_t)start[0] + fixed_width - 1,
                     strand ? (int)strand[0] : 0, n_chrom, chrom_off,
                     chrom_len, 0, &a, &b, &e0))
            w = b - a;
    }
    if (blockIdx.x == 0 && threadIdx.x == 0) *exc.w_out = w;

    auto one = [&](int c, int s, int64_t e, int st, uint32_t* gs, uint32_t* ge1) {
        *gs = 0;
        *ge1 = 0;
        if (map_read(c, s, e, st, n_chrom, chrom_off, chrom_len, frag_len, gs, ge1, &my_err)) {
            wmax = max(wmax, *ge1 - *gs);
            nlong += (*ge1 - *gs > long_thr);
            if (*ge1 - *gs != w && !exc_full) {
                if (*reinterpret_cast<volatile unsigned int*>(exc.count) > exc.cap) {
                    exc_full = true;
                } else {
                    const unsigned int k = atomicAdd(exc.count, 1u);
                    if (k < exc.cap) {
                        exc.xw[k] = *gs + w;
                        exc.e1[k] = *ge1;
                        exc.st[k] = (int8_t)(st > 0 ? 1 : (st < 0 ? -1 : 0));
                    }
                }
            }
        }
        np += st > 0;
        nm += st < 0;
        ns += st == 0;
    };
    auto sgn = [](int st) { return (int8_t)(st > 0 ? 1 : (st < 0 ? -1 : 0)); };

    const int64_t stride = (int64_t)gridDim.x * TPB;
    const int64_t n_vec = (VEC == 4) ? (n >> 2) : 0;
    for (int64_t v = (int64_t)blockIdx.x * TPB + threadIdx.x; v < n_vec; v += stride) {
        const int4 c4 = __ldg(reinterpret_cast<const int4*>(chrom) + v);
        const int4 s4 = __ldg(reinterpret_cast<const int4*>(start) + v);
        int4 e4 = make_int4(0, 0, 0, 0);
        if (HAS_END) e4 = __ldg(reinterpret_cast<const int4*>(end) + v);
        const int64_t wm1 = (int64_t)fixed_width - 1;
        char4 t4 = make_char4(0, 0, 0, 0);
        if (strand) t4 = __ldg(reinterpret_cast<const char4*>(strand) + v);
        uint4 gs, ge;
        one(c4.x, s4.x, HAS_END ? (int64_t)e4.x : s4.x + wm1, t4.x, &gs.x, &ge.x);
        one(c4.y, s4.y, HAS_END ? (int64_t)e4.y : s4.y + wm1, t4.y, &gs.y, &ge.y);
        one(c4.z, s4.z, HAS_END ? (int64_t)e4.z : s4.z + wm1, t4.z, &gs.z, &ge.z);
        one(c4.w, s4.w, HAS_END ? (int64_t)e4.w : s4.w + wm1, t4.w, &gs.w, &ge.w);
        reinterpret_cast<uint4*>(g_start)[v] = gs;
        reinterpret_cast<uint4*>(g_end1)[v] = ge;
        if (xs_out) reinterpret_cast<uint4*>(xs_out)[v] = gs;
        if (strand_out)
            reinterpret_cast<char4*>(strand_out)[v] = make_char4(sgn(t4.x), sgn(t4.y), sgn(t4.z), sgn(t4.w));
    }
    for (int64_t i = n_vec * 4 + (int64_t)blockIdx.x * TPB + threadIdx.x; i < n; i += stride) {
        const int st = strand ? (int)strand[i] : 0;
        uint32_t gs, ge1;
        one(chrom[i], start[i], HAS_END ? (int64_t)end[i] : (int64_t)start[i] + fixed_width - 1, st, &gs, &ge1);
        g_start[i] = gs;
        g_end1[i] = ge1;
        if (xs_out) xs_out[i] = gs;
        if (strand_out) strand_out[i] = sgn(st);
    }
    __shared__ unsigned int sh[6];
    if (threadIdx.x < 6) sh[threadIdx.x] = 0;
    __syncthreads();
    for (int d = 16; d > 0; d >>= 1) {
        np += __shfl_xor_sync(0xffffffffu, np, d);
        nm += __shfl_xor_sync(0xffffffffu, nm, d);
        ns += __shfl_xor_sync(0xffffffffu, ns, d);
        my_err |= __shfl_xor_sync(0xffffffffu, my_err, d);
        wmax = max(wmax, __shfl_xor_sync(0xffffffffu, wmax, d));
        nlong += __shfl_xor_sync(0xffffffffu, nlong, d);
    }
    if ((threadIdx.x & 31) == 0) {
        if (nlong) atomicAdd(&sh[5], nlong);
        atomicAdd(&sh[0], np);
        atomicAdd(&sh[1], nm);
        atomicAdd(&sh[2], ns);
        atomicOr(&sh[3], my_err);
        atomicMax(&sh[4], wmax);
    }
    __syncthreads();
    if (threadIdx.x == 0) {
        if (sh[0]) atomicAdd(&cls_count[0], (unsigned long long)sh[0]);
        if (sh[1]) atomicAdd(&cls_count[1], (unsigned long long)sh[1]);
        if (sh[2]) atomicAdd(&cls_count[2], (unsigned long long)sh[2]);
        if (sh[3]) atomicOr(err, sh[3]);
        if (sh[4]) atomicMax(&cls_count[3], (unsigned long long)sh[4]);
        if (sh[5]) atomicAdd(exc.count + 2, sh[5]);
    }
}

__global__ void __launch_bounds__(TPB)
exc_select_kernel(uint32_t n_exc, const uint32_t* __restrict__ xw, const uint32_t* __restrict__ e1,
                  const int8_t* __restrict__ st, int want ,
                  uint32_t* __restrict__ cxs, uint32_t* __restrict__ cye) {
    const uint32_t i = blockIdx.x * TPB + threadIdx.x;
    if (i >= n_exc) return;
    const bool keep = (want == 2) || ((int)st[i] == want);
    cxs[i] = keep ? xw[i] : 0xffffffffu;
    cye[i] = keep ? e1[i] : 0xffffffffu;
}

__global__ void __launch_bounds__(TPB)
compact_strand_kernel(int64_t n, const uint32_t* __restrict__ g_start,
                      const uint32_t* __restrict__ g_end1, const int8_t* __restrict__ strand,
                      int want, uint32_t* __restrict__ xs, uint32_t* __restrict__ ye ,
                      unsigned long long* __restrict__ cursor) {
    const int64_t stride = (int64_t)gridDim.x * TPB;
    const unsigned lane = threadIdx.x & 31;
    const int64_t n_round = (n + 31) & ~(int64_t)31;
    for (int64_t i = (int64_t)blockIdx.x * TPB + threadIdx.x; i < n_round; i += stride) {
        const bool keep = (i < n) && ((int)strand[i] == want);
        const unsigned m = __ballot_sync(0xffffffffu, keep);
        if (m == 0) continue;
        unsigned long long base = 0;
        if (lane == 0) base = atomicAdd(cursor, (unsigned long long)__popc(m));
        base = __shfl_sync(0xffffffffu, base, 0);
        if (keep) {
            const unsigned long long o = base + __popc(m & ((1u << lane) - 1u));
            xs[o] = g_start[i];
            if (ye) ye[o] = g_end1[i];
        }
    }
}

__global__ void __launch_bounds__(TPB) iota_kernel(int64_t n, uint32_t* __restrict__ v) {
    const int64_t stride = (int64_t)gridDim.x * TPB;
    for (int64_t i = (int64_t)blockIdx.x * TPB + threadIdx.x; i < n; i += stride)
        v[i] = (uint32_t)i;
}

__global__ void __launch_bounds__(TPB)
gather_pairs_kernel(int64_t n, const uint32_t* __restrict__ perm,
                    const uint32_t* __restrict__ g_end1, const int8_t* __restrict__ strand,
                    uint32_t* __restrict__ p_end1, int8_t* __restrict__ p_strand) {
    const int64_t stride = (int64_t)gridDim.x * TPB;
    for (int64_t i = (int64_t)blockIdx.x * TPB + threadIdx.x; i < n; i += stride) {
        const uint32_t j = perm[i];
        p_end1[i] = g_end1[j];
        if (p_strand) p_strand[i] = strand[j];
    }
}

constexpr int MX_ITEMS = 8;
constexpr int MX_TILE = TPB * MX_ITEMS;

__device__ __forceinline__ uint32_t block_max_scan(uint32_t v, uint32_t* total) {
    __shared__ uint32_t wmax[TPB / 32];
    const unsigned lane = threadIdx.x & 31, warp = threadIdx.x >> 5;
#pragma unroll
    for (int d = 1; d < 32; d <<= 1) {
        uint32_t o = __shfl_up_sync(0xffffffffu, v, d);
        if (lane >= d) v = max(v, o);
    }
    if (lane == 31) wmax[warp] = v;
    __syncthreads();
    uint32_t pre = 0, tot = 0;
#pragma unroll
    for (int w = 0; w < TPB / 32; w++) {
        uint32_t s = wmax[w];
        if (w < (int)warp) pre = max(pre, s);
        tot = max(tot, s);
    }
    __syncthreads();
    *total = tot;
    return max(pre, v);
}

__global__ void __launch_bounds__(TPB)
max_reduce_kernel(const uint32_t* __restrict__ in, int64_t n, uint32_t* __restrict__ partial) {
    const int64_t base = (int64_t)blockIdx.x * MX_TILE;
    uint32_t m = 0;
#pragma unroll
    for (int k = 0; k < MX_ITEMS; k++) {
        int64_t i = base + (int64_t)k * TPB + threadIdx.x;
        if (i < n) m = max(m, in[i]);
    }
    uint32_t tot;
    block_max_scan(m, &tot);
    if (threadIdx.x == 0) partial[blockIdx.x] = tot;
}

__global__ void __launch_bounds__(TPB)
max_partials_kernel(uint32_t* __restrict__ partial, int64_t nb) {
    uint32_t carry = 0;
    for (int64_t b0 = 0; b0 < nb; b0 += TPB) {
        int64_t i = b0 + threadIdx.x;
        uint32_t v = (i < nb) ? partial[i] : 0;
        uint32_t tot;
        uint32_t inc = block_max_scan(v, &tot);
        uint32_t prev = __shfl_up_sync(0xffffffffu, inc, 1);
        __shared__ uint32_t last_of_warp[TPB / 32];
        if ((threadIdx.x & 31) == 31) last_of_warp[threadIdx.x >> 5] = inc;
        __syncthreads();
        uint32_t ex;
        if ((threadIdx.x & 31) != 0) ex = prev;
        else ex = (threadIdx.x == 0) ? 0u : last_of_warp[(threadIdx.x >> 5) - 1];
        __syncthreads();
        if (i < nb) partial[i] = max(carry, ex);
        carry = max(carry, tot);
    }
}

__global__ void __launch_bounds__(TPB)
max_apply_kernel(const uint32_t* __restrict__ in, uint32_t* __restrict__ out, int64_t n,
                 const uint32_t* __restrict__ partial) {
    const int64_t base = (int64_t)blockIdx.x * MX_TILE + (int64_t)threadIdx.x * MX_ITEMS;
    uint32_t v[MX_ITEMS];
    uint32_t m = 0;
#pragma unroll
    for (int k = 0; k < MX_ITEMS; k++) {
        int64_t i = base + k;
        v[k] = (i < n) ? in[i] : 0;
        m = max(m, v[k]);
    }
    uint32_t tot;
    uint32_t inc = block_max_scan(m, &tot);
    uint32_t prev = __shfl_up_sync(0xffffffffu, inc, 1);
    __shared__ uint32_t last_of_warp[TPB / 32];
    if ((threadIdx.x & 31) == 31) last_of_warp[threadIdx.x >> 5] = inc;
    __syncthreads();
    uint32_t run;
    if ((threadIdx.x & 31) != 0) run = prev;
    else run = (threadIdx.x == 0) ? 0u : last_of_warp[(threadIdx.x >> 5) - 1];
    run = max(run, partial[blockIdx.x]);
#pragma unroll
    for (int k = 0; k < MX_ITEMS; k++) {
        int64_t i = base + k;
        run = max(run, v[k]);
        if (i < n) out[i] = run;
    }
}

int running_max_u32(const uint32_t* in, uint32_t* out, int64_t n) {
    if (n <= 0) return RCP_OK;
    const int64_t nb = (n + MX_TILE - 1) / MX_TILE;
    uint32_t* partial = nullptr;
    RCP_TRY(dalloc(&partial, (size_t)nb));
    max_reduce_kernel<<<(unsigned)nb, TPB, 0, g_ctx.stream>>>(in, n, partial);
    RCP_LAUNCHED();
    max_partials_kernel<<<1, TPB, 0, g_ctx.stream>>>(partial, nb);
    RCP_LAUNCHED();
    max_apply_kernel<<<(unsigned)nb, TPB, 0, g_ctx.stream>>>(in, out, n, partial);
    RCP_LAUNCHED();
    dfree(partial);
    return RCP_OK;
}

inline unsigned grid_for(int64_t n) {
    int64_t b = (n + TPB - 1) / TPB;
    int64_t cap = (int64_t)g_ctx.sm_count * 16;
    if (b > cap) b = cap;
    if (b < 1) b = 1;
    return (unsigned)b;
}

}

int running_max_u32_device(const uint32_t* in, uint32_t* out, int64_t n) { return running_max_u32(in, out, n); }

void reads_release(ReadsIdx& r) {
    if (r.bn_base) device_free(r.bn_base);
    r.bn_base = nullptr;
    r.bn_cand = r.bn_boff = r.bn_cb = nullptr;
    dfree(r.ln_xs);
    dfree(r.ln_e1);
    dfree(r.ln_st);
    dfree(r.ln_maxe1);
    r.ln_n = 0;
    dfree(r.pd_err);
    dfree(r.pd_cnt);
    dfree(r.pd_w);
    dfree(r.pd_run_first);
    r.pending = false;
    dfree(r.d_chrom_len);
    dfree(r.d_chrom_off);
    dfree(r.d_len_na);
    dfree(r.g_start);
    dfree(r.g_end1);
    dfree(r.d_strand);
    for (int c = 0; c < CLS_N; c++) {
        dfree(r.cls[c].xs);
        dfree(r.cls[c].ye);
        dfree(r.cls[c].cxs);
        dfree(r.cls[c].cye);
        r.cls[c].built = false;
        r.cls[c].xs_sorted = false;
    }
    dfree(r.exc_xw);
    dfree(r.exc_e1);
    dfree(r.exc_st);
    dfree(r.p_end1);
    dfree(r.p_strand);
    dfree(r.p_maxend1);
    r.pairs_built = false;
}

int reads_build_class(ReadsIdx& r, int cls) {
    SortedClass& sc = r.cls[cls];
    if (sc.built) return RCP_OK;
    const bool uni = r.uniform_w != 0;
    const bool xs_done = sc.xs_sorted;
    if (cls == CLS_ALL) {
        sc.n = r.n;
        if (sc.xs == nullptr) {
            RCP_TRY(dalloc(&sc.xs, (size_t)r.n));
            RCP_CUDA(cudaMemcpyAsync(sc.xs, r.g_start, (size_t)r.n * 4, cudaMemcpyDeviceToDevice,
                                     g_ctx.stream));
        }
        if (!uni) {
            RCP_TRY(dalloc(&sc.ye, (size_t)r.n));
            RCP_CUDA(cudaMemcpyAsync(sc.ye, r.g_end1, (size_t)r.n * 4, cudaMemcpyDeviceToDevice,
                                     g_ctx.stream));
        }
    } else {
        RCP_TRY(dalloc(&sc.xs, (size_t)sc.n));
        if (!uni) RCP_TRY(dalloc(&sc.ye, (size_t)sc.n));
        if (sc.n > 0) {
            if (!r.has_strand) {
                RCP_CUDA(cudaMemcpyAsync(sc.xs, r.g_start, (size_t)r.n * 4,
                                         cudaMemcpyDeviceToDevice, g_ctx.stream));
                if (!uni)
                    RCP_CUDA(cudaMemcpyAsync(sc.ye, r.g_end1, (size_t)r.n * 4,
                                             cudaMemcpyDeviceToDevice, g_ctx.stream));
            } else {
                unsigned long long* cursor = nullptr;
                RCP_TRY(dalloc(&cursor, 1));
                RCP_CUDA(cudaMemsetAsync(cursor, 0, sizeof(unsigned long long), g_ctx.stream));
                const int want = cls == CLS_PLUS ? 1 : (cls == CLS_MINUS ? -1 : 0);
                compact_strand_kernel<<<grid_for(r.n), TPB, 0, g_ctx.stream>>>(
                    r.n, r.g_start, r.g_end1, r.d_strand, want, sc.xs, sc.ye, cursor);
                RCP_LAUNCHED();
                dfree(cursor);
            }
        }
    }
    if (uni && r.n_exc > 0) {
        sc.cn = r.n_exc;
        RCP_TRY(dalloc(&sc.cxs, (size_t)sc.cn));
        RCP_TRY(dalloc(&sc.cye, (size_t)sc.cn));
        const int want = cls == CLS_ALL ? 2 : (cls == CLS_PLUS ? 1 : (cls == CLS_MINUS ? -1 : 0));
        exc_select_kernel<<<(unsigned)((sc.cn + TPB - 1) / TPB), TPB, 0, g_ctx.stream>>>(
            (uint32_t)sc.cn, r.exc_xw, r.exc_e1, r.exc_st, r.has_strand ? want : 2, sc.cxs, sc.cye);
        RCP_LAUNCHED();
    }
    {
        StageTimer t(ST_INDEX_SORT);
        if (!xs_done) RCP_TRY(sort_keys_u32(sc.xs, sc.n, r.key_bits));
        sc.xs_sorted = true;
        if (!uni) RCP_TRY(sort_keys_u32(sc.ye, sc.n, r.key_bits));
        if (sc.cn > 0) {
            RCP_TRY(sort_keys_u32(sc.cxs, sc.cn, 32));
            RCP_TRY(sort_keys_u32(sc.cye, sc.cn, 32));
        }
    }
    r.device_bytes += (size_t)sc.n * (uni ? 4 : 8);
    sc.built = true;
    return RCP_OK;
}

int reads_build_pairs(ReadsIdx& r) {
    if (r.pairs_built) return RCP_OK;
    SortedClass& all = r.cls[CLS_ALL];
    uint32_t *keys = nullptr, *perm = nullptr;
    RCP_TRY(dalloc(&keys, (size_t)r.n));
    RCP_TRY(dalloc(&perm, (size_t)r.n));
    RCP_CUDA(cudaMemcpyAsync(keys, r.g_start, (size_t)r.n * 4, cudaMemcpyDeviceToDevice,
                             g_ctx.stream));
    iota_kernel<<<grid_for(r.n), TPB, 0, g_ctx.stream>>>(r.n, perm);
    RCP_LAUNCHED();
    {
        StageTimer t(ST_INDEX_SORT);
        RCP_TRY(sort_pairs_u32(keys, perm, r.n, r.key_bits));
    }
    if (!all.xs_sorted) {
        dfree(all.xs);
        all.xs = keys;
        all.n = r.n;
        all.xs_sorted = true;
        keys = nullptr;
    }
    RCP_TRY(dalloc(&r.p_end1, (size_t)r.n));
    if (r.has_strand) RCP_TRY(dalloc(&r.p_strand, (size_t)r.n));
    gather_pairs_kernel<<<grid_for(r.n), TPB, 0, g_ctx.stream>>>(r.n, perm, r.g_end1, r.d_strand,
                                                                r.p_end1, r.p_strand);
    RCP_LAUNCHED();
    RCP_TRY(dalloc(&r.p_maxend1, (size_t)r.n));
    RCP_TRY(running_max_u32(r.p_end1, r.p_maxend1, r.n));
    if (keys) dfree(keys);
    dfree(perm);
    r.device_bytes += (size_t)r.n * (8 + (r.has_strand ? 1 : 0));
    r.pairs_built = true;
    return RCP_OK;
}

__global__ void __launch_bounds__(TPB)
rle_expand_kernel(int64_t n, int64_t n_runs, const int32_t* __restrict__ run_value,
                  const uint32_t* __restrict__ run_first ,
                  int32_t* __restrict__ dense ) {
    const int64_t stride = (int64_t)gridDim.x * TPB;
    const int64_t n_vec = (n + 3) >> 2;
    for (int64_t v = (int64_t)blockIdx.x * TPB + threadIdx.x; v < n_vec; v += stride) {
        const uint32_t i0 = (uint32_t)(v * 4);
        int64_t a = 0, b = n_runs;
        while (b - a > 1) {
            const int64_t mid = (a + b) >> 1;
            if (__ldg(run_first + mid) <= i0) a = mid;
            else b = mid;
        }
        int64_t r = a;
        uint32_t next = __ldg(run_first + r + 1);
        int32_t val = __ldg(run_value + r);
        int32_t o[4];
#pragma unroll
        for (int k = 0; k < 4; k++) {
            while (i0 + k >= next && r + 1 < n_runs) {
                r++;
                next = __ldg(run_first + r + 1);
                val = __ldg(run_value + r);
            }
            o[k] = (i0 + k < next) ? val : -1;
        }
        reinterpret_cast<int4*>(dense)[v] = make_int4(o[0], o[1], o[2], o[3]);
    }
}

__global__ void __launch_bounds__(TPB)
rle_check_kernel(int64_t n_runs, const int32_t* __restrict__ run_len, unsigned int* __restrict__ err) {
    const int64_t i = (int64_t)blockIdx.x * TPB + threadIdx.x;
    if (i < n_runs && run_len[i] < 0) atomicOr(err, 8u);
}

int reads_load_impl(ReadsIdx& r, int64_t n, const int32_t* chrom, int64_t n_runs,
                    const int32_t* run_chrom, const int32_t* run_len, const int32_t* start,
                    const int32_t* end, const int8_t* strand, int n_chrom,
                    const int64_t* chrom_len, int frag_len, int mem, int fixed_width) {
    const bool dbg = getenv("RCP_DEBUG_TIMING") != nullptr;
    auto t_start = std::chrono::steady_clock::now();
    auto lap = [&](const char* what) {
        if (!dbg) return;
        auto now = std::chrono::steady_clock::now();
        fprintf(stderr, "[rcp_reads_load] %-28s %8.3f ms\n", what,
                std::chrono::duration<double, std::milli>(now - t_start).count());
        t_start = now;
    };
    r.n = n;
    r.n_chrom = n_chrom;
    r.has_strand = strand != nullptr;
    r.chrom_len.assign(chrom_len, chrom_len + n_chrom);
    r.chrom_off.resize((size_t)n_chrom + 1);
    r.len_na.assign((size_t)n_chrom, 0);
    r.any_na = false;
    for (int c = 0; c < n_chrom; c++)
        if (chrom_len[c] <= 0) {
            r.len_na[(size_t)c] = 1;
            r.any_na = true;
        }
    auto layout = [&]() -> int {
        uint64_t off = 0;
        for (int c = 0; c < n_chrom; c++) {
            r.chrom_off[c] = (uint32_t)off;
            off += (uint64_t)r.chrom_len[(size_t)c] + 2;
            if (off >= 0xfffffff0ull)
                return fail(RCP_ERR_UNSUPPORTED,
                            "genome longer than 2^32 positions: 64-bit coordinates not implemented");
        }
        r.chrom_off[n_chrom] = (uint32_t)off;
        r.key_bits = 1;
        while (r.key_bits < 32 && (1ull << r.key_bits) <= off) r.key_bits++;
        RCP_CUDA(cudaMemcpyAsync(r.d_chrom_len, r.chrom_len.data(), (size_t)n_chrom * 8,
                                 cudaMemcpyHostToDevice, g_ctx.stream));
        RCP_CUDA(cudaMemcpyAsync(r.d_chrom_off, r.chrom_off.data(), ((size_t)n_chrom + 1) * 4,
                                 cudaMemcpyHostToDevice, g_ctx.stream));
        return RCP_OK;
    };
    RCP_TRY(dalloc(&r.d_chrom_len, (size_t)n_chrom));
    RCP_TRY(dalloc(&r.d_chrom_off, (size_t)n_chrom + 1));
    if (!r.any_na) RCP_TRY(layout());

    DevIn<int32_t> d_chrom, d_start, d_end, d_run_chrom, d_run_len;
    DevIn<int8_t> d_strand;
    const bool rle = chrom == nullptr && n > 0;
    if (rle) {
        RCP_TRY(d_run_chrom.init(run_chrom, (size_t)n_runs, mem));
        RCP_TRY(d_run_len.init(run_len, (size_t)n_runs, mem));
    } else {
        RCP_TRY(d_chrom.init(chrom, (size_t)n, mem));
    }
    RCP_TRY(d_start.init(start, (size_t)n, mem));
    RCP_TRY(d_end.init(end, (size_t)n, mem));
    RCP_TRY(d_strand.init(strand, (size_t)n, mem));
    lap("staging copies enqueued");

    RCP_TRY(dalloc(&r.g_start, (size_t)n));
    RCP_TRY(dalloc(&r.g_end1, (size_t)n));
    if (r.has_strand) RCP_TRY(dalloc(&r.d_strand, (size_t)n));
    unsigned int* d_err = nullptr;
    unsigned long long* d_cnt = nullptr;
    unsigned int* d_w = nullptr;
    RCP_TRY(dalloc(&d_err, 1));
    RCP_TRY(dalloc(&d_cnt, 4));
    RCP_TRY(dalloc(&d_w, 4));
    RCP_CUDA(cudaMemsetAsync(d_err, 0, sizeof(unsigned int), g_ctx.stream));
    RCP_CUDA(cudaMemsetAsync(d_cnt, 0, 4 * sizeof(unsigned long long), g_ctx.stream));
    RCP_CUDA(cudaMemsetAsync(d_w, 0, 4 * sizeof(unsigned int), g_ctx.stream));
    uint32_t* run_first = nullptr;
    if (rle) {
        StageTimer t(ST_INDEX_MAP);
        RCP_TRY(dalloc(&run_first, (size_t)n_runs + 1));
        RCP_TRY(dalloc(&d_chrom.owned, ((size_t)n + 3) & ~(size_t)3));
        d_chrom.ptr = d_chrom.owned;
        rle_check_kernel<<<(unsigned)((n_runs + TPB - 1) / TPB), TPB, 0, g_ctx.stream>>>(n_runs, d_run_len.ptr, d_err);
        RCP_LAUNCHED();
        RCP_TRY(exclusive_scan_u32(reinterpret_cast<const uint32_t*>(d_run_len.ptr), run_first, n_runs,
                                   run_first + n_runs));
        rle_expand_kernel<<<grid_for((n + 3) / 4), TPB, 0, g_ctx.stream>>>(
            n, n_runs, d_run_chrom.ptr, run_first, d_chrom.owned);
        RCP_LAUNCHED();
    }
    if (r.any_na) {
        unsigned long long* d_max = nullptr;
        RCP_TRY(dalloc(&d_max, (size_t)n_chrom));
        RCP_CUDA(cudaMemsetAsync(d_max, 0, (size_t)n_chrom * 8, g_ctx.stream));
        if (n > 0) {
            chrom_max_end_kernel<<<grid_for(n), TPB, 0, g_ctx.stream>>>(n, d_chrom.ptr, d_start.ptr, d_end.ptr,
                                                                       d_strand.ptr, n_chrom, frag_len, fixed_width,
                                                                       d_max);
            RCP_LAUNCHED();
        }
        std::vector<unsigned long long> h_max((size_t)n_chrom, 0ull);
        RCP_CUDA(cudaMemcpyAsync(h_max.data(), d_max, (size_t)n_chrom * 8, cudaMemcpyDeviceToHost, g_ctx.stream));
        RCP_CUDA(cudaStreamSynchronize(g_ctx.stream));
        dfree(d_max);
        for (int c = 0; c < n_chrom; c++)
            if (r.len_na[(size_t)c])
                r.chrom_len[(size_t)c] = (int64_t)std::min<unsigned long long>(std::max<unsigned long long>(h_max[(size_t)c], 1ull),
                                                                               0x7ffffff0ull);
        RCP_TRY(layout());
        RCP_TRY(dalloc(&r.d_len_na, (size_t)n_chrom));
        RCP_CUDA(cudaMemcpyAsync(r.d_len_na, r.len_na.data(), (size_t)n_chrom, cudaMemcpyHostToDevice, g_ctx.stream));
    }
    {
        const int wbits = 32 - split_position_bits((int64_t)r.chrom_off[(size_t)n_chrom]) - (r.has_strand ? 2 : 0);
        r.long_thr = wbits >= 7 ? std::min<uint32_t>((1u << wbits) - 1u, 8191u) : 0xffffffffu;
    }
    ExcBuf exc;
    exc.cap = (uint32_t)std::min<int64_t>(std::max<int64_t>(n / 64, 4096), 65536);
    RCP_TRY(dalloc(&r.exc_xw, (size_t)exc.cap));
    RCP_TRY(dalloc(&r.exc_e1, (size_t)exc.cap));
    RCP_TRY(dalloc(&r.exc_st, (size_t)exc.cap));
    exc.xw = r.exc_xw;
    exc.e1 = r.exc_e1;
    exc.st = r.exc_st;
    exc.count = d_w;
    exc.w_out = d_w + 1;
    const bool eager_index = g_ctx.coverage_path == RCP_PATH_INDEX;
    if (eager_index) RCP_TRY(dalloc(&r.cls[CLS_ALL].xs, (size_t)n));
    if (n > 0) {
        StageTimer t(ST_INDEX_MAP);
        auto al16 = [](const void* q) { return (reinterpret_cast<uintptr_t>(q) & 15u) == 0; };
        const bool vec = al16(d_chrom.ptr) && al16(d_start.ptr) && (d_end.ptr == nullptr || al16(d_end.ptr)) &&
                         (d_strand.ptr == nullptr || (reinterpret_cast<uintptr_t>(d_strand.ptr) & 3u) == 0);
        const unsigned grid = grid_for(vec ? (n + 3) / 4 : n);
        auto launch = [&](auto kern) {
            kern<<<grid, TPB, 0, g_ctx.stream>>>(n, d_chrom.ptr, d_start.ptr, d_end.ptr, d_strand.ptr, r.d_chrom_off,
                                                 r.d_chrom_len, n_chrom, frag_len, fixed_width, r.long_thr, r.g_start,
                                                 r.g_end1,
                                                 r.cls[CLS_ALL].xs, r.d_strand, d_err, d_cnt, exc);
        };
        if (d_end.ptr) {
            if (vec) launch(reads_to_global_kernel<4, true>);
            else launch(reads_to_global_kernel<1, true>);
        } else {
            if (vec) launch(reads_to_global_kernel<4, false>);
            else launch(reads_to_global_kernel<1, false>);
        }
        RCP_LAUNCHED();
    }
    lap("map kernel enqueued");
    r.pending = true;
    r.pd_rle = rle;
    r.pd_err = d_err;
    r.pd_cnt = d_cnt;
    r.pd_w = d_w;
    r.pd_run_first = run_first;
    r.pd_run_total = rle ? run_first + n_runs : nullptr;
    r.pd_exc_cap = exc.cap;
    r.pd_eager_index = eager_index;
    r.device_bytes += (size_t)n * (8 + (r.has_strand ? 1 : 0));
    if (g_ctx.deferred_validation && !eager_index) return RCP_OK;
    RCP_TRY(reads_resolve(r));
    lap("sync (copies + map kernel)");
    return RCP_OK;
}

int reads_pending_items(ReadsIdx& r, FetchItem* items, int* n) {
    if (!r.pending) return RCP_OK;
    items[(*n)++] = {r.pd_err, &r.h_err, 4};
    items[(*n)++] = {r.pd_cnt, r.h_cnt, 32};
    items[(*n)++] = {r.pd_w, r.h_w, 16};
    if (r.pd_rle) items[(*n)++] = {r.pd_run_total, &r.h_total, 4};
    return RCP_OK;
}

int reads_resolve(ReadsIdx& r) {
    if (!r.pending) return RCP_OK;
    FetchItem items[4];
    int n = 0;
    reads_pending_items(r, items, &n);
    RCP_TRY(fetch_and_sync(items, n));
    return reads_finish(r);
}

int reads_finish(ReadsIdx& r) {
    if (!r.pending) return RCP_OK;
    r.pending = false;
    const int64_t n = r.n;
    const unsigned int h_err = r.h_err;
    dfree(r.pd_err);
    dfree(r.pd_cnt);
    dfree(r.pd_w);
    dfree(r.pd_run_first);
    r.pd_run_total = nullptr;
    if (h_err & 8u) return fail(RCP_ERR_DATA, "a seqnames run has a negative length");
    if (r.pd_rle && (int64_t)r.h_total != n)
        return fail(RCP_ERR_DATA, "the seqnames run lengths sum to %u, not to the %lld reads", r.h_total,
                    (long long)n);
    if (h_err == 0 && n > 0 && r.h_w[1] > 0 && r.h_w[0] <= r.pd_exc_cap) {
        r.uniform_w = r.h_w[1];
        r.n_exc = (int64_t)r.h_w[0];
    } else {
        r.uniform_w = 0;
        r.n_exc = 0;
    }
    if (r.n_exc == 0) {
        dfree(r.exc_xw);
        dfree(r.exc_e1);
        dfree(r.exc_st);
    }
    if (h_err & 1u) return fail(RCP_ERR_DATA, "a read has a chromosome id outside [0, n_chrom)");
    if (h_err & 2u) return fail(RCP_ERR_DATA, "a read violates 1 <= start <= end");
    if (h_err & 4u) return fail(RCP_ERR_DATA, "a read starts beyond the end of its chromosome");
    r.cls[CLS_PLUS].n = (int64_t)r.h_cnt[0];
    r.cls[CLS_MINUS].n = (int64_t)r.h_cnt[1];
    r.cls[CLS_STAR].n = (int64_t)r.h_cnt[2];
    r.max_width = (uint32_t)r.h_cnt[3];
    r.n_long = (int64_t)r.h_w[2];
    if (r.pd_eager_index) RCP_TRY(reads_build_class(r, CLS_ALL));
    return RCP_OK;
}

namespace {

__global__ void __launch_bounds__(TPB)
keep_flags_kernel(int64_t n, const int32_t* __restrict__ start, const int32_t* __restrict__ end,
                  double max_width, uint32_t* __restrict__ flag) {
    const int64_t i = (int64_t)blockIdx.x * TPB + threadIdx.x;
    if (i >= n) return;
    const double w = (double)end[i] - (double)start[i] + 1.0;
    flag[i] = !(w > max_width);
}

__global__ void __launch_bounds__(TPB)
kept_positions_kernel(int64_t n, const uint32_t* __restrict__ flag, const uint32_t* __restrict__ rank,
                      uint32_t* __restrict__ kept_pos) {
    const int64_t i = (int64_t)blockIdx.x * TPB + threadIdx.x;
    if (i < n && flag[i]) kept_pos[rank[i]] = (uint32_t)i;
}

__global__ void __launch_bounds__(TPB)
select_gather_kernel(int64_t k, int64_t n_kept, const int32_t* __restrict__ idx,
                     const uint32_t* __restrict__ kept_pos, const int32_t* __restrict__ chrom,
                     const int32_t* __restrict__ start, const int32_t* __restrict__ end,
                     const int8_t* __restrict__ strand, int32_t* __restrict__ o_chrom,
                     int32_t* __restrict__ o_start, int32_t* __restrict__ o_end,
                     int8_t* __restrict__ o_strand, unsigned int* __restrict__ err) {
    const int64_t j = (int64_t)blockIdx.x * TPB + threadIdx.x;
    if (j >= k) return;
    int64_t p = idx ? (int64_t)idx[j] - 1 : j;
    if (p < 0 || p >= n_kept) {
        atomicOr(err, 1u);
        p = 0;
    }
    const int64_t i = kept_pos ? (int64_t)kept_pos[p] : p;
    o_chrom[j] = chrom[i];
    o_start[j] = start[i];
    o_end[j] = end[i];
    if (o_strand) o_strand[j] = strand[i];
}

}

int reads_load_select_impl(ReadsIdx& r, int64_t n, const int32_t* chrom, const int32_t* start,
                           const int32_t* end, const int8_t* strand, double max_width, int64_t k,
                           const int32_t* idx, int n_chrom, const int64_t* chrom_len, int frag_len,
                           int mem, int64_t* n_kept_out) {
    DevIn<int32_t> d_chrom, d_start, d_end, d_idx;
    DevIn<int8_t> d_strand;
    RCP_TRY(d_chrom.init(chrom, (size_t)n, mem));
    RCP_TRY(d_start.init(start, (size_t)n, mem));
    RCP_TRY(d_end.init(end, (size_t)n, mem));
    RCP_TRY(d_strand.init(strand, (size_t)n, mem));
    RCP_TRY(d_idx.init(idx, (size_t)k, mem));
    const bool filter = max_width >= 0.0 && n > 0;
    int64_t n_kept = n;
    uint32_t *flag = nullptr, *rank = nullptr, *kept_pos = nullptr;
    unsigned int* d_err = nullptr;
    RCP_TRY(dalloc(&d_err, 1));
    RCP_CUDA(cudaMemsetAsync(d_err, 0, 4, g_ctx.stream));
    int rc = RCP_OK;
    if (filter) {
        StageTimer t(ST_INDEX_MAP);
        rc = dalloc(&flag, (size_t)n);
        if (rc == RCP_OK) rc = dalloc(&rank, (size_t)n + 1);
        if (rc == RCP_OK) {
            keep_flags_kernel<<<(unsigned)((n + TPB - 1) / TPB), TPB, 0, g_ctx.stream>>>(n, d_start.ptr, d_end.ptr, max_width, flag);
            g_ctx.launches++;
            rc = exclusive_scan_u32(flag, rank, n, rank + n);
        }
        uint32_t h_kept = 0;
        if (rc == RCP_OK) {
            cudaError_t e = cudaMemcpyAsync(&h_kept, rank + n, 4, cudaMemcpyDeviceToHost, g_ctx.stream);
            if (e == cudaSuccess) e = cudaStreamSynchronize(g_ctx.stream);
            if (e != cudaSuccess) rc = fail(RCP_ERR_CUDA, "width filter failed: %s", cudaGetErrorString(e));
        }
        n_kept = (int64_t)h_kept;
        if (rc == RCP_OK) rc = dalloc(&kept_pos, (size_t)n_kept);
        if (rc == RCP_OK && n_kept > 0) {
            kept_positions_kernel<<<(unsigned)((n + TPB - 1) / TPB), TPB, 0, g_ctx.stream>>>(n, flag, rank, kept_pos);
            g_ctx.launches++;
        }
    }
    if (n_kept_out) *n_kept_out = n_kept;
    const int64_t m = idx ? k : n_kept;
    int32_t *o_chrom = nullptr, *o_start = nullptr, *o_end = nullptr;
    int8_t* o_strand = nullptr;
    if (rc == RCP_OK) rc = dalloc(&o_chrom, (size_t)m);
    if (rc == RCP_OK) rc = dalloc(&o_start, (size_t)m);
    if (rc == RCP_OK) rc = dalloc(&o_end, (size_t)m);
    if (rc == RCP_OK && strand) rc = dalloc(&o_strand, (size_t)m);
    unsigned int h_err = 0;
    if (rc == RCP_OK && m > 0) {
        if (n_kept == 0) {
            rc = fail(RCP_ERR_DATA, "an index selects from an empty set of reads");
        } else {
            StageTimer t(ST_INDEX_MAP);
            select_gather_kernel<<<(unsigned)((m + TPB - 1) / TPB), TPB, 0, g_ctx.stream>>>(
                m, n_kept, d_idx.ptr, kept_pos, d_chrom.ptr, d_start.ptr, d_end.ptr, d_strand.ptr, o_chrom,
                o_start, o_end, o_strand, d_err);
            g_ctx.launches++;
            cudaError_t e = cudaMemcpyAsync(&h_err, d_err, 4, cudaMemcpyDeviceToHost, g_ctx.stream);
            if (e == cudaSuccess) e = cudaStreamSynchronize(g_ctx.stream);
            if (e != cudaSuccess) rc = fail(RCP_ERR_CUDA, "read selection failed: %s", cudaGetErrorString(e));
            if (rc == RCP_OK && h_err)
                rc = fail(RCP_ERR_DATA, "a selection index is outside 1..%lld", (long long)n_kept);
        }
    }
    if (rc == RCP_OK)
        rc = reads_load_impl(r, m, o_chrom, 0, nullptr, nullptr, o_start, o_end, o_strand, n_chrom, chrom_len,
                             frag_len, RCP_MEM_DEVICE, 0);
    dfree(flag);
    dfree(rank);
    dfree(kept_pos);
    dfree(d_err);
    dfree(o_chrom);
    dfree(o_start);
    dfree(o_end);
    dfree(o_strand);
    return rc;
}

}
```

### recoup_b200/csrc/rcp_internal.cuh

```cuda
#pragma once
#include <cuda_runtime.h>
#include <stdint.h>

#include <string>
#include <vector>

#include "recoup_b200.h"

namespace rcp {

struct Ctx {
    bool ready = false;
    int device = -1;
    int sm_count = 0;
    int cc_major = 0, cc_minor = 0;
    size_t mem_bytes = 0;
    cudaStream_t stream = nullptr;
    int64_t launches = 0;
    int coverage_path = RCP_PATH_AUTO;
    bool deferred_validation = false;
};
extern Ctx g_ctx;

int fail(int code, const char* fmt, ...);
constexpr int RCP_SWITCH_TO_INDEX = -1000;
constexpr int RCP_SPLIT_NOT_APPLICABLE = -1001;
int require_ready();

#define RCP_CUDA(call)                                                                         \
    do {                                                                                       \
        cudaError_t _e = (call);                                                               \
        if (_e != cudaSuccess)                                                                 \
            return ::rcp::fail(RCP_ERR_CUDA, "%s failed at %s:%d: %s", #call, __FILE__,        \
                               __LINE__, cudaGetErrorString(_e));                              \
    } while (0)

#define RCP_TRY(expr)                                                                          \
    do {                                                                                       \
        int _rc = (expr);                                                                      \
        if (_rc != RCP_OK) return _rc;                                                         \
    } while (0)

#define RCP_LAUNCHED()                                                                         \
    do {                                                                                       \
        ::rcp::g_ctx.launches++;                                                               \
        RCP_CUDA(cudaGetLastError());                                                          \
    } while (0)

enum Stage {
    ST_INDEX_MAP = 0,
    ST_INDEX_SORT,
    ST_COV_PLAN,
    ST_COV_TILE,
    ST_COV_SMALL,
    ST_COV_LIST,
    ST_COV_CONCAT,
    ST_PROF_BIN,
    ST_PROF_INTERP,
    ST_PROF_BASE,
    ST_FUSED,
    ST_BKT_PLAN,
    ST_BKT_COUNT,
    ST_BKT_SCATTER,
    ST_BKT_TILE,
    ST_BKT_SMALL,
    ST_BLK_FILTER,
    ST_BLK_HIST,
    ST_BLK_SCATTER,
    ST_BLK_TILE,
    ST_BLK_SMALL,
    ST_SP_PLAN,
    ST_SP_SPLIT,
    ST_SP_SORT,
    ST_SP_TILE,
    ST_SP_SMALL,
    ST_N
};
struct StageTimer {
    int slot;
    explicit StageTimer(int stage);
    ~StageTimer();
};

int device_alloc(void** p, size_t bytes);
void device_free(void* p);

template <class T>
inline int dalloc(T** p, size_t n) {
    *p = nullptr;
    if (n == 0) n = 1;
    return device_alloc((void**)p, n * sizeof(T));
}
template <class T>
inline void dfree(T*& p) {
    if (p) device_free((void*)p);
    p = nullptr;
}

struct FetchItem {
    const void* dev;
    void* host;
    int bytes;
};
int fetch_and_sync(const FetchItem* items, int n);
int fetch_begin(const FetchItem* items, int n);
int fetch_end(const FetchItem* items, int n);

struct Arena {
    char* base = nullptr;
    size_t used = 0, cap = 0;
    static size_t pad(size_t bytes) { return (bytes + 255) & ~(size_t)255; }
    int reserve(size_t bytes) {
        cap = bytes;
        used = 0;
        return device_alloc(reinterpret_cast<void**>(&base), bytes > 0 ? bytes : 1);
    }
    template <class T>
    T* take(size_t n) {
        T* p = reinterpret_cast<T*>(base + used);
        used += pad(n * sizeof(T));
        return p;
    }
    ~Arena() {
        if (base) device_free(base);
    }
};

template <class T>
struct DevIn {
    const T* ptr = nullptr;
    T* owned = nullptr;
    int init(const T* src, size_t n, int mem) {
        if (mem == RCP_MEM_DEVICE || src == nullptr) {
            ptr = src;
            return RCP_OK;
        }
        RCP_TRY(dalloc(&owned, n));
        RCP_CUDA(cudaMemcpyAsync(owned, src, n * sizeof(T), cudaMemcpyHostToDevice, g_ctx.stream));
        ptr = owned;
        return RCP_OK;
    }
    ~DevIn() { dfree(owned); }
};

struct InflateJob {
    int64_t in_off = 0, in_len = 0, out_off = 0;
    uint32_t out_cap = 0, out_len = 0;
    uint32_t crc = 0;
};
enum {
    INFLATE_RAW_CRC = 0,
    INFLATE_ZLIB = 1,
    INFLATE_COPY = 2
};
int64_t inflate_jobs(const uint8_t* data, InflateJob* jobs, int64_t n_jobs, uint8_t* out, int n_threads,
                     int kind);

enum { CLS_ALL = 0, CLS_PLUS = 1, CLS_MINUS = 2, CLS_STAR = 3, CLS_N = 4 };

struct SortedClass {
    bool built = false;
    bool xs_sorted = false;
    int64_t n = 0;
    uint32_t* xs = nullptr;
    uint32_t* ye = nullptr;
    int64_t cn = 0;
    uint32_t* cxs = nullptr;
    uint32_t* cye = nullptr;
};

struct ReadsIdx {
    int64_t n = 0;
    int n_chrom = 0;
    bool has_strand = false;
    uint32_t max_width = 0;
    uint32_t uniform_w = 0;
    int64_t n_exc = 0;
    uint32_t* exc_xw = nullptr;
    uint32_t* exc_e1 = nullptr;
    int8_t* exc_st = nullptr;
    int key_bits = 32;
    std::vector<int64_t> chrom_len;
    std::vector<uint32_t> chrom_off;
    int64_t* d_chrom_len = nullptr;
    uint32_t* d_chrom_off = nullptr;
    bool any_na = false;
    std::vector<uint8_t> len_na;
    uint8_t* d_len_na = nullptr;
    uint32_t* g_start = nullptr;
    uint32_t* g_end1 = nullptr;
    int8_t* d_strand = nullptr;
    SortedClass cls[CLS_N];
    bool pairs_built = false;
    uint32_t* p_end1 = nullptr;
    int8_t* p_strand = nullptr;
    uint32_t* p_maxend1 = nullptr;
    size_t device_bytes = 0;
    char* bn_base = nullptr;
    uint32_t* bn_cand = nullptr;
    uint32_t* bn_boff = nullptr;
    uint32_t* bn_cb = nullptr;
    int bn_P = 0;
    bool bn_stranded = false;
    int64_t ln_n = 0;
    uint32_t bn_max_pack_w = 0;
    uint32_t* ln_xs = nullptr;
    uint32_t* ln_e1 = nullptr;
    int8_t* ln_st = nullptr;
    uint32_t* ln_maxe1 = nullptr;
    bool pending = false;
    bool pd_rle = false;
    unsigned int* pd_err = nullptr;
    unsigned long long* pd_cnt = nullptr;
    unsigned int* pd_w = nullptr;
    uint32_t* pd_run_total = nullptr;
    uint32_t* pd_run_first = nullptr;
    uint32_t pd_exc_cap = 0;
    bool pd_eager_index = false;
    unsigned int h_err = 0, h_w[4] = {0, 0, 0, 0}, h_total = 0;
    uint32_t long_thr = 0;
    int64_t n_long = 0;
    unsigned long long h_cnt[4] = {0, 0, 0, 0};
};

inline int split_position_bits(int64_t span) {
    int P = 16;
    while (P < 22 && ((span + (1ll << P) - 1) >> P) > 1024) P++;
    return P;
}

int reads_pending_items(ReadsIdx& r, FetchItem* items, int* n);
int reads_finish(ReadsIdx& r);
int reads_resolve(ReadsIdx& r);

int reads_build_class(ReadsIdx& r, int cls);
int reads_build_pairs(ReadsIdx& r);
void reads_release(ReadsIdx& r);

struct Coverage {
    int64_t n_regions = 0;
    int64_t total_padded = 0;
    int64_t total_len = 0;
    int64_t n_null = 0;
    int32_t max_len = 0;
    int path = 0;
    int64_t candidates = 0;
    unsigned long long* d_stats = nullptr;
    bool stats_pending = false;
    double scale = 1.0;
    int value_type = RCP_VALUE_INT32;
    const unsigned long long* d_bound = nullptr;
    int32_t* cov = nullptr;
    int64_t* off = nullptr;
    int32_t* len = nullptr;
    uint8_t* is_null = nullptr;
};
void coverage_release(Coverage& c);
int coverage_resolve_stats(Coverage& c);

constexpr unsigned long long NARROW_MAX = 0xffffull;
__device__ __forceinline__ bool cov_narrow(const unsigned long long* bound) {
    return bound != nullptr && *bound <= NARROW_MAX;
}
__device__ __forceinline__ int32_t cov_at(const int32_t* cov, int64_t i, bool narrow) {
    return narrow ? (int32_t)reinterpret_cast<const uint16_t*>(cov)[i] : cov[i];
}
int coverage_na_rule(const ReadsIdx& rd, Coverage& cv, int64_t R, const int32_t* d_chrom, const int8_t* d_strand,
                     const int64_t* d_end_pos);

ReadsIdx* get_reads(int h);
Coverage* get_coverage(int h);
int new_coverage(Coverage** out, int* handle);

int sort_keys_u32(uint32_t* keys_in_out, int64_t n, int end_bit);
int sort_pairs_u32(uint32_t* keys_in_out, uint32_t* vals_in_out, int64_t n, int end_bit);
int running_max_u32_device(const uint32_t* in, uint32_t* out, int64_t n);
int exclusive_scan_i64(const int64_t* in, int64_t* out, int64_t n, int64_t* d_total);
int exclusive_scan_u32(const uint32_t* in, uint32_t* out, int64_t n, uint32_t* d_total);
int exclusive_scan_u32_bounded(const uint32_t* in, uint32_t* out, int64_t n_upper, const uint32_t* n_dev,
                               uint32_t* d_total);
int sort_pairs_u64_i32(unsigned long long*& keys, int32_t*& vals, int64_t n);
struct RRng;
void r_sample_int(RRng& rng, int64_t n, int64_t k, int32_t* out);
int exclusive_scan2_i64(const int64_t* in0, int64_t* out0, int64_t* d_total0, const int64_t* in1,
                        int64_t* out1, int64_t* d_total1, int64_t n);

}
```

Measured before the change: 52.31 billion.

## Fuse read mapping into split kernel with cp.async staging and L2 prefetch

Defers the read-to-genome mapping kernel and, when shared memory allows, performs mapping inside the split kernel. Raw chrom/start/end/strand are staged into shared memory with cp.async, and the next round is prefetched into L2. This removes a separate launch and the round trip of writing and re-reading mapped coordinates before splitting. The mapped arrays are still written for later stages. The fused path uses smaller rounds (one vector per thread), and the exception and statistics accounting moves into a per-block commit, which adds complexity and some risk of correctness mismatches.

```diff
diff --git a/recoup_b200/csrc/coverage_split.cu b/recoup_b200/csrc/coverage_split.cu
--- a/recoup_b200/csrc/coverage_split.cu
+++ b/recoup_b200/csrc/coverage_split.cu
@@ -3,6 +3,7 @@
 #include <chrono>
 #include <cstdio>
 
+#include <functional>
 #include <type_traits>
 #include <vector>
 
@@ -11,6 +12,7 @@
 #include "cov_common.cuh"
 #include "r_rng.cuh"
 #include "rcp_internal.cuh"
+#include "reads_map.cuh"
 
 namespace rcp {
 
@@ -218,22 +220,53 @@
     uint32_t* pool_next;
 };
 
-constexpr size_t sp_split_smem(int words) {
-    return (size_t)NG * RING * 4 + (size_t)NG * 4 + (size_t)words * 4;
+constexpr int MAP_STAGE_BYTES = ST * (3 * 16 + 4);
+constexpr size_t sp_split_smem(int n_groups, int words, bool map = false) {
+    return (size_t)n_groups * RING * 4 + (size_t)NG * 4 + (((size_t)words * 4 + 15) & ~(size_t)15) +
+           (map ? (size_t)MAP_STAGE_BYTES : 0);
 }
 constexpr size_t SP_SMEM_MAX = 232448;
 
-template <bool STRANDED>
-__global__ void __launch_bounds__(ST, 1)
-sp_split_kernel(int64_t n, const uint32_t* __restrict__ g_start, const uint32_t* __restrict__ g_end1,
-                const int8_t* __restrict__ strand, const uint32_t* __restrict__ tab_g, int words, int P,
-                uint32_t max_pack_w, SplitOut out) {
+struct MapIn {
+    const int32_t* chrom;
+    const int32_t* start;
+    const int32_t* end;
+    const int8_t* strand;
+    int fixed_width;
+    MapArgs a;
+    uint32_t* g_start;
+    uint32_t* g_end1;
+    int8_t* strand_out;
+    unsigned int* err;
+    unsigned long long* cls_count;
+};
+
+__device__ __forceinline__ void cp_async16_zf(uint32_t dst, const void* src, bool ok) {
+    asm volatile("cp.async.cg.shared.global [%0], [%1], 16, %2;" ::"r"(dst), "l"(src), "r"(ok ? 16 : 0) : "memory");
+}
+__device__ __forceinline__ void prefetch_l2(const void* src, uint32_t bytes) {
+    asm volatile("cp.async.bulk.prefetch.L2.global [%0], %1;" ::"l"(src), "r"(bytes) : "memory");
+}
+#ifndef RCP_MAP_PREFETCH
+#define RCP_MAP_PREFETCH 1
+#endif
+
+__device__ __forceinline__ void cp_async4_zf(uint32_t dst, const void* src, bool ok) {
+    asm volatile("cp.async.ca.shared.global [%0], [%1], 4, %2;" ::"r"(dst), "l"(src), "r"(ok ? 4 : 0) : "memory");
+}
+
+template <bool STRANDED, bool MAP, bool HAS_END>
+__device__ __forceinline__ void
+sp_split_body(int64_t n, const uint32_t* __restrict__ g_start, const uint32_t* __restrict__ g_end1,
+              const int8_t* __restrict__ strand, const uint32_t* __restrict__ tab_g, int words, int P, int n_groups,
+              uint32_t max_pack_w, const SplitOut& out, const MapIn& mi) {
     extern __shared__ __align__(16) unsigned char sp_smem[];
     const int tid = threadIdx.x;
     const unsigned lane = tid & 31, lt = (1u << lane) - 1u;
     const uint32_t ring_a = (uint32_t)__cvta_generic_to_shared(sp_smem);
-    const uint32_t cnt_a = ring_a + NG * RING * 4;
+    const uint32_t cnt_a = ring_a + (uint32_t)n_groups * RING * 4;
     const uint32_t tab_a = cnt_a + NG * 4;
+    const uint32_t stage_a = tab_a + (((uint32_t)words * 4u + 15u) & ~15u);
     for (int i = tid; i < words; i += ST) sts32(tab_a + i * 4, tab_g[i]);
     for (int i = tid; i < NG; i += ST) sts32(cnt_a + i * 4, 0u);
     __syncthreads();
@@ -332,9 +365,9 @@
     constexpr int RPT = 4 * VPT;
     uint32_t fg[RPT], fp[RPT];
     uint32_t nf = 0;
-    auto take = [&](uint32_t sv, uint32_t ev, int tv) {
+    auto take = [&](uint32_t sv, uint32_t ev, int tv, bool valid = true) {
         const uint32_t g = sv >> P, pk = pack(sv, ev, tv);
-        bool want = keep_read(sv, ev);
+        bool want = valid && keep_read(sv, ev);
         if (hot) want = direct(want, g, pk);
         if (want && !insert(g, pk)) {
             fg[nf] = g;
@@ -368,8 +401,10 @@
     };
 
     __shared__ int next_round[2];
+    constexpr int RV = MAP ? ST : ROUND_VEC;
+    constexpr int NV = RV / ST;
     const int64_t n_vec = n >> 2;
-    const int rounds = (int)((n_vec + ROUND_VEC - 1) / ROUND_VEC);
+    const int rounds = (int)((n_vec + RV - 1) / RV);
     if (tid == 0) {
         next_round[0] = (int)atomicAdd(out.pool_next + 1, 1u);
         next_round[1] = (int)atomicAdd(out.pool_next + 1, 1u);
@@ -377,8 +412,50 @@
     __syncthreads();
     int round = next_round[0], nr = next_round[1];
     __syncthreads();
-    uint4 s4[VPT], e4[VPT];
-    char4 t4[VPT];
+    MapAcc acc;
+    uint32_t w_cand = 0;
+    if (MAP) {
+        w_cand = map_candidate_width<HAS_END>(mi.a, mi.chrom, mi.start, mi.end, mi.strand, mi.fixed_width);
+        if (blockIdx.x == 0 && tid == 0) *mi.a.exc.w_out = w_cand;
+    }
+    const uint32_t st_c = stage_a + tid * 16u, st_s = st_c + ST * 16u, st_e = st_s + ST * 16u,
+                   st_t = stage_a + 3u * ST * 16u + tid * 4u;
+    auto stage = [&](int rd) {
+        const int64_t v = (int64_t)rd * RV + tid;
+        const bool ok = rd < rounds && v < n_vec;
+        const int64_t q = ok ? v : 0;
+        cp_async16_zf(st_c, reinterpret_cast<const int4*>(mi.chrom) + q, ok);
+        cp_async16_zf(st_s, reinterpret_cast<const int4*>(mi.start) + q, ok);
+        if (HAS_END) cp_async16_zf(st_e, reinterpret_cast<const int4*>(mi.end) + q, ok);
+        if (mi.strand) cp_async4_zf(st_t, reinterpret_cast<const char4*>(mi.strand) + q, ok);
+        asm volatile("cp.async.commit_group;" ::: "memory");
+    };
+    auto map_take = [&](int64_t v) {
+        asm volatile("cp.async.wait_all;" ::: "memory");
+        const bool ok = v < n_vec;
+        const uint4 c4 = lds128(st_c), s4 = lds128(st_s);
+        const uint4 e4 = HAS_END ? lds128(st_e) : make_uint4(0, 0, 0, 0);
+        const uint32_t tw = mi.strand ? lds32(st_t) : 0u;
+        const int t0 = (int8_t)tw, t1 = (int8_t)(tw >> 8), t2 = (int8_t)(tw >> 16), t3 = (int8_t)(tw >> 24);
+        uint4 gs = make_uint4(0, 0, 0, 0), ge = make_uint4(0, 0, 0, 0);
+        if (ok) {
+            map_one(mi.a, w_cand, acc, (int)c4.x, (int)s4.x, HAS_END ? (int64_t)(int)e4.x : (int64_t)(int)s4.x + (mi.fixed_width - 1), t0, &gs.x, &ge.x);
+            map_one(mi.a, w_cand, acc, (int)c4.y, (int)s4.y, HAS_END ? (int64_t)(int)e4.y : (int64_t)(int)s4.y + (mi.fixed_width - 1), t1, &gs.y, &ge.y);
+            map_one(mi.a, w_cand, acc, (int)c4.z, (int)s4.z, HAS_END ? (int64_t)(int)e4.z : (int64_t)(int)s4.z + (mi.fixed_width - 1), t2, &gs.z, &ge.z);
+            map_one(mi.a, w_cand, acc, (int)c4.w, (int)s4.w, HAS_END ? (int64_t)(int)e4.w : (int64_t)(int)s4.w + (mi.fixed_width - 1), t3, &gs.w, &ge.w);
+            reinterpret_cast<uint4*>(mi.g_start)[v] = gs;
+            reinterpret_cast<uint4*>(mi.g_end1)[v] = ge;
+            if (mi.strand_out)
+                reinterpret_cast<char4*>(mi.strand_out)[v] =
+                    make_char4(strand_sign(t0), strand_sign(t1), strand_sign(t2), strand_sign(t3));
+        }
+        take(gs.x, ge.x, t0, ok);
+        take(gs.y, ge.y, t1, ok);
+        take(gs.z, ge.z, t2, ok);
+        take(gs.w, ge.w, t3, ok);
+    };
+    uint4 s4[NV], e4[NV];
+    char4 t4[NV];
     auto load = [&](int rd, int h) {
         const int64_t v = (int64_t)rd * ROUND_VEC + h * ST + tid;
         s4[h] = e4[h] = make_uint4(0, 0, 0, 0);
@@ -389,32 +466,82 @@
             if (STRANDED && strand) t4[h] = __ldcs(reinterpret_cast<const char4*>(strand) + v);
         }
     };
+    if (MAP) {
+        stage(round);
+    } else {
 #pragma unroll
-    for (int h = 0; h < VPT; h++) load(round, h);
+        for (int h = 0; h < NV; h++) load(round, h);
+    }
     for (int it = 0; round < rounds; it++) {
         unsigned after = 0;
         if (tid == 0) after = atomicAdd(out.pool_next + 1, 1u);
+        if (MAP) {
+            map_take((int64_t)round * RV + tid);
+            stage(nr);
+            if (RCP_MAP_PREFETCH && tid == 0 && after < (unsigned)rounds) {
+                const int64_t v0 = (int64_t)after * RV;
+                const uint32_t nv = (uint32_t)min((int64_t)RV, n_vec - v0);
+                prefetch_l2(reinterpret_cast<const int4*>(mi.chrom) + v0, nv * 16u);
+                prefetch_l2(reinterpret_cast<const int4*>(mi.start) + v0, nv * 16u);
+                if (HAS_END) prefetch_l2(reinterpret_cast<const int4*>(mi.end) + v0, nv * 16u);
+                const char4* t = reinterpret_cast<const char4*>(mi.strand) + v0;
+                if (mi.strand && (reinterpret_cast<uintptr_t>(t) & 15u) == 0 && nv >= 4u) prefetch_l2(t, (nv * 4u) & ~15u);
+            }
+        } else {
 #pragma unroll
-        for (int h = 0; h < VPT; h++) {
-            take(s4[h].x, e4[h].x, t4[h].x);
-            take(s4[h].y, e4[h].y, t4[h].y);
-            take(s4[h].z, e4[h].z, t4[h].z);
-            take(s4[h].w, e4[h].w, t4[h].w);
-            load(nr, h);
+            for (int h = 0; h < NV; h++) {
+                take(s4[h].x, e4[h].x, t4[h].x);
+                take(s4[h].y, e4[h].y, t4[h].y);
+                take(s4[h].z, e4[h].z, t4[h].z);
+                take(s4[h].w, e4[h].w, t4[h].w);
+                load(nr, h);
+            }
         }
         if (tid == 0) next_round[it & 1] = (int)min(after, 0x7fffffffu);
         finish_round();
         round = nr;
         nr = next_round[it & 1];
     }
+    if (MAP) asm volatile("cp.async.wait_all;" ::: "memory");
     if (blockIdx.x == 0) {
         const int64_t i = n_vec * 4 + tid;
         const bool in = i < n;
-        const uint32_t sv = in ? g_start[i] : 0u, ev = in ? g_end1[i] : 0u;
-        take(sv, ev, (in && STRANDED && strand) ? (int)strand[i] : 0);
+        if (MAP) {
+            const int tv = (in && mi.strand) ? (int)mi.strand[i] : 0;
+            uint32_t sv = 0, ev = 0;
+            if (in) {
+                map_one(mi.a, w_cand, acc, mi.chrom[i], mi.start[i], HAS_END ? (int64_t)mi.end[i] : (int64_t)mi.start[i] + (mi.fixed_width - 1),
+                        tv, &sv, &ev);
+                mi.g_start[i] = sv;
+                mi.g_end1[i] = ev;
+                if (mi.strand_out) mi.strand_out[i] = strand_sign(tv);
+            }
+            take(sv, ev, tv, in);
+        } else {
+            const uint32_t sv = in ? g_start[i] : 0u, ev = in ? g_end1[i] : 0u;
+            take(sv, ev, (in && STRANDED && strand) ? (int)strand[i] : 0);
+        }
         finish_round();
     }
     flush_phase(true);
+    if (MAP) map_acc_commit(acc, mi.a, mi.err, mi.cls_count);
+}
+
+template <bool STRANDED>
+__global__ void __launch_bounds__(ST, 1)
+sp_split_kernel(int64_t n, const uint32_t* __restrict__ g_start, const uint32_t* __restrict__ g_end1,
+                const int8_t* __restrict__ strand, const uint32_t* __restrict__ tab_g, int words, int P, int n_groups,
+                uint32_t max_pack_w, SplitOut out) {
+    sp_split_body<STRANDED, false, false>(n, g_start, g_end1, strand, tab_g, words, P, n_groups, max_pack_w, out,
+                                          MapIn{});
+}
+
+template <bool STRANDED, bool HAS_END>
+__global__ void __launch_bounds__(ST, 1)
+sp_map_split_kernel(int64_t n, MapIn mi, const uint32_t* __restrict__ tab_g, int words, int P, int n_groups,
+                    uint32_t max_pack_w, SplitOut out) {
+    sp_split_body<STRANDED, true, HAS_END>(n, nullptr, nullptr, nullptr, tab_g, words, P, n_groups, max_pack_w, out,
+                                           mi);
 }
 
 __device__ __forceinline__ void sp_slot_range(uint32_t n_slots, uint32_t* lo, uint32_t* hi) {
@@ -1323,7 +1450,8 @@
 };
 
 static int split_and_sort(ReadsIdx& rd, const uint32_t* tab, int words, int P, int n_groups, bool stranded,
-                          bool st_arr, uint32_t max_pack_w, Arena& K, Arena& B, SortedCands* sc) {
+                          bool st_arr, uint32_t max_pack_w, Arena& K, Arena& B, SortedCands* sc,
+                          const std::function<int()>& fetch = nullptr) {
     const int nb = 1 << (P - SUB_SHIFT);
     const uint32_t pmask = (1u << P) - 1u;
     const int split_grid = g_ctx.sm_count;
@@ -1346,23 +1474,63 @@
     if (B.used > B.cap || K.used > K.cap) return fail(RCP_ERR_CUDA, "internal: split arena overrun");
     DebugLap dbg;
     dbg.lap("  split_and_sort: arenas");
+    const bool fuse = rd.map_pending && sp_split_smem(n_groups, words, true) <= SP_SMEM_MAX && map_split_enabled();
+    if (!fuse) {
+        RCP_TRY(reads_ensure_mapped(rd));
+        if (fetch) RCP_TRY(fetch());
+    }
     {
         StageTimer t(ST_SP_SPLIT);
         RCP_CUDA(cudaMemsetAsync(B.base, 0, zero_b, g_ctx.stream));
-        const size_t smem = sp_split_smem(words);
         SplitOut out = {pool, meta, pool_next};
-        if (stranded) {
-            RCP_CUDA(cudaFuncSetAttribute(sp_split_kernel<true>, cudaFuncAttributeMaxDynamicSharedMemorySize, (int)smem));
-            sp_split_kernel<true><<<split_grid, ST, smem, g_ctx.stream>>>(rd.n, rd.g_start, rd.g_end1,
-                                                                         st_arr ? rd.d_strand : nullptr, tab, words, P,
-                                                                         max_pack_w, out);
+        if (fuse) {
+            rd.map_pending = false;
+            MapIn mi;
+            mi.chrom = rd.mp_chrom;
+            mi.start = rd.mp_start;
+            mi.end = rd.mp_end;
+            mi.strand = rd.mp_strand;
+            mi.fixed_width = rd.mp_fixed_width;
+            ExcBuf exc;
+            exc.xw = rd.exc_xw;
+            exc.e1 = rd.exc_e1;
+            exc.st = rd.exc_st;
+            exc.cap = rd.pd_exc_cap;
+            exc.count = rd.pd_w;
+            exc.w_out = rd.pd_w + 1;
+            mi.a = {rd.d_chrom_ol, rd.n_chrom, rd.mp_frag_len, rd.long_thr, exc};
+            mi.g_start = rd.g_start;
+            mi.g_end1 = rd.g_end1;
+            mi.strand_out = rd.d_strand;
+            mi.err = rd.pd_err;
+            mi.cls_count = rd.pd_cnt;
+            const size_t smem = sp_split_smem(n_groups, words, true);
+            auto launch = [&](auto kern) -> int {
+                RCP_CUDA(cudaFuncSetAttribute(kern, cudaFuncAttributeMaxDynamicSharedMemorySize, (int)smem));
+                kern<<<split_grid, ST, smem, g_ctx.stream>>>(rd.n, mi, tab, words, P, n_groups, max_pack_w, out);
+                return RCP_OK;
+            };
+            if (stranded) RCP_TRY(mi.end ? launch(sp_map_split_kernel<true, true>) : launch(sp_map_split_kernel<true, false>));
+            else RCP_TRY(mi.end ? launch(sp_map_split_kernel<false, true>) : launch(sp_map_split_kernel<false, false>));
+            rd.mp_chrom = rd.mp_start = rd.mp_end = nullptr;
+            rd.mp_strand = nullptr;
+            dfree(rd.mp_chrom_owned);
         } else {
-            RCP_CUDA(cudaFuncSetAttribute(sp_split_kernel<false>, cudaFuncAttributeMaxDynamicSharedMemorySize, (int)smem));
-            sp_split_kernel<false><<<split_grid, ST, smem, g_ctx.stream>>>(rd.n, rd.g_start, rd.g_end1, nullptr, tab,
-                                                                          words, P, max_pack_w, out);
+            const size_t smem = sp_split_smem(n_groups, words);
+            if (stranded) {
+                RCP_CUDA(cudaFuncSetAttribute(sp_split_kernel<true>, cudaFuncAttributeMaxDynamicSharedMemorySize, (int)smem));
+                sp_split_kernel<true><<<split_grid, ST, smem, g_ctx.stream>>>(rd.n, rd.g_start, rd.g_end1,
+                                                                             st_arr ? rd.d_strand : nullptr, tab, words,
+                                                                             P, n_groups, max_pack_w, out);
+            } else {
+                RCP_CUDA(cudaFuncSetAttribute(sp_split_kernel<false>, cudaFuncAttributeMaxDynamicSharedMemorySize, (int)smem));
+                sp_split_kernel<false><<<split_grid, ST, smem, g_ctx.stream>>>(rd.n, rd.g_start, rd.g_end1, nullptr, tab,
+                                                                              words, P, n_groups, max_pack_w, out);
+            }
         }
         RCP_LAUNCHED();
     }
+    if (fuse && fetch) RCP_TRY(fetch());
     dbg.lap("  split_and_sort: split kernel");
     {
         StageTimer t(ST_SP_SORT);
@@ -1398,7 +1566,7 @@
     g.n_groups = (int)std::max<int64_t>(1, (span + (1ll << g.P) - 1) >> g.P);
     g.nb = 1 << (g.P - SUB_SHIFT);
     g.pmask = (1u << g.P) - 1u;
-    g.ok = g.n_groups <= NG && rd.n < 0x7ffffff0ll && sp_split_smem(g.words) <= SP_SMEM_MAX;
+    g.ok = g.n_groups <= NG && rd.n < 0x7ffffff0ll && sp_split_smem(NG, g.words) <= SP_SMEM_MAX;
     return g;
 }
 
@@ -1489,7 +1657,7 @@
     while (P < MAX_P && ((span + (1ll << P) - 1) >> P) > NG) P++;
     const int n_groups = (int)std::max<int64_t>(1, (span + (1ll << P) - 1) >> P);
     const int wbits = 32 - P - (stranded ? 2 : 0);
-    if (n_groups > NG || rd.n >= 0x7ffffff0ll || sp_split_smem(words) > SP_SMEM_MAX)
+    if (n_groups > NG || rd.n >= 0x7ffffff0ll || sp_split_smem(NG, words) > SP_SMEM_MAX)
         return RCP_SPLIT_NOT_APPLICABLE;
     const bool have_index = rd.bn_cand && rd.bn_P == P && (rd.bn_stranded || !stranded);
     if (!have_index && !rd.pending && (rd.max_width > 8191u || rd.max_width >= (1u << wbits)))
@@ -1557,8 +1725,10 @@
                               {err, &h.err, 4}};
         int n_items = 4;
         reads_pending_items(rd, items, &n_items);
-        RCP_TRY(fetch_begin(items, n_items));
-        if (!have_index) RCP_TRY(split_and_sort(rd, tab, words, P, n_groups, stranded, st_arr, 0xffffffffu, K, B, &sc));
+        auto begin = [&]() { return fetch_begin(items, n_items); };
+        if (!have_index) RCP_TRY(split_and_sort(rd, tab, words, P, n_groups, stranded, st_arr, 0xffffffffu, K, B, &sc,
+                                                begin));
+        else RCP_TRY(begin());
         RCP_TRY(fetch_end(items, n_items));
         RCP_TRY(reads_finish(rd));
     }
diff --git a/recoup_b200/csrc/import.cu b/recoup_b200/csrc/import.cu
--- a/recoup_b200/csrc/import.cu
+++ b/recoup_b200/csrc/import.cu
@@ -1032,8 +1032,9 @@
     auto it = g_decoded.find(decoded);
     if (it == g_decoded.end()) return fail(RCP_ERR_HANDLE, "unknown decoded handle %d", decoded);
     const Decoded& d = *it->second;
-    return rcp_reads_load(d.n, d.chrom, d.start, d.end, d.strand, n_chrom, chrom_len, frag_len, RCP_MEM_DEVICE,
-                          reads_out);
+    RCP_TRY(rcp_reads_load(d.n, d.chrom, d.start, d.end, d.strand, n_chrom, chrom_len, frag_len, RCP_MEM_DEVICE,
+                           reads_out));
+    return reads_ensure_mapped(*get_reads(*reads_out));
 }
 
 int rcp_decoded_width_quantile(int decoded, double prob, double* quantile_out, int64_t* n_le_out) {
diff --git a/recoup_b200/csrc/index.cu b/recoup_b200/csrc/index.cu
--- a/recoup_b200/csrc/index.cu
+++ b/recoup_b200/csrc/index.cu
@@ -2,42 +2,16 @@
 #include <chrono>
 #include <cstdio>
 #include <cstdlib>
+#include <cstring>
 
 #include "rcp_internal.cuh"
+#include "reads_map.cuh"
 
 namespace rcp {
 
 namespace {
 
 constexpr int TPB = 256;
-
-struct ExcBuf {
-    uint32_t* xw;
-    uint32_t* e1;
-    int8_t* st;
-    uint32_t cap;
-    unsigned int* count;
-    uint32_t* w_out;
-};
-
-__device__ __forceinline__ bool map_read(int c, int64_t s, int64_t e, int st, int n_chrom,
-                                         const uint32_t* __restrict__ chrom_off,
-                                         const int64_t* __restrict__ chrom_len, int frag_len,
-                                         uint32_t* gs, uint32_t* ge1, unsigned int* err) {
-    if (c < 0 || c >= n_chrom) { *err |= 1u; return false; }
-    if (s < 1 || e < s) { *err |= 2u; return false; }
-    const int64_t len = chrom_len[c];
-    if (frag_len > 0) {
-        if (st < 0) s = e - frag_len + 1;
-        else e = s + frag_len - 1;
-    }
-    if (s < 1) s = 1;
-    if (e > len) e = len;
-    if (s > len || e < s) { *err |= 4u; return false; }
-    *gs = chrom_off[c] + (uint32_t)s;
-    *ge1 = chrom_off[c] + (uint32_t)e + 1u;
-    return true;
-}
 
 __global__ void __launch_bounds__(TPB)
 chrom_max_end_kernel(int64_t n, const int32_t* __restrict__ chrom, const int32_t* __restrict__ start,
@@ -66,52 +40,14 @@
 __global__ void __launch_bounds__(TPB)
 reads_to_global_kernel(int64_t n, const int32_t* __restrict__ chrom,
                        const int32_t* __restrict__ start, const int32_t* __restrict__ end,
-                       const int8_t* __restrict__ strand, const uint32_t* __restrict__ chrom_off,
-                       const int64_t* __restrict__ chrom_len, int n_chrom, int frag_len,
+                       const int8_t* __restrict__ strand,
                        int fixed_width ,
-                       uint32_t long_thr ,
-                       uint32_t* __restrict__ g_start, uint32_t* __restrict__ g_end1,
+                       MapArgs a, uint32_t* __restrict__ g_start, uint32_t* __restrict__ g_end1,
                        uint32_t* __restrict__ xs_out, int8_t* __restrict__ strand_out,
-                       unsigned int* __restrict__ err, unsigned long long* __restrict__ cls_count,
-                       ExcBuf exc) {
-    unsigned int my_err = 0;
-    unsigned int np = 0, nm = 0, ns = 0, wmax = 0, nlong = 0;
-    bool exc_full = false;
-    uint32_t w = (uint32_t)frag_len;
-    if (frag_len <= 0) {
-        uint32_t a = 0, b = 0;
-        unsigned int e0 = 0;
-        if (map_read(chrom[0], start[0], HAS_END ? (int64_t)end[0] : (int64_t)start[0] + fixed_width - 1,
-                     strand ? (int)strand[0] : 0, n_chrom, chrom_off,
-                     chrom_len, 0, &a, &b, &e0))
-            w = b - a;
-    }
-    if (blockIdx.x == 0 && threadIdx.x == 0) *exc.w_out = w;
-
-    auto one = [&](int c, int s, int64_t e, int st, uint32_t* gs, uint32_t* ge1) {
-        *gs = 0;
-        *ge1 = 0;
-        if (map_read(c, s, e, st, n_chrom, chrom_off, chrom_len, frag_len, gs, ge1, &my_err)) {
-            wmax = max(wmax, *ge1 - *gs);
-            nlong += (*ge1 - *gs > long_thr);
-            if (*ge1 - *gs != w && !exc_full) {
-                if (*reinterpret_cast<volatile unsigned int*>(exc.count) > exc.cap) {
-                    exc_full = true;
-                } else {
-                    const unsigned int k = atomicAdd(exc.count, 1u);
-                    if (k < exc.cap) {
-                        exc.xw[k] = *gs + w;
-                        exc.e1[k] = *ge1;
-                        exc.st[k] = (int8_t)(st > 0 ? 1 : (st < 0 ? -1 : 0));
-                    }
-                }
-            }
-        }
-        np += st > 0;
-        nm += st < 0;
-        ns += st == 0;
-    };
-    auto sgn = [](int st) { return (int8_t)(st > 0 ? 1 : (st < 0 ? -1 : 0)); };
+                       unsigned int* __restrict__ err, unsigned long long* __restrict__ cls_count) {
+    MapAcc acc;
+    const uint32_t w = map_candidate_width<HAS_END>(a, chrom, start, end, strand, fixed_width);
+    if (blockIdx.x == 0 && threadIdx.x == 0) *a.exc.w_out = w;
 
     const int64_t stride = (int64_t)gridDim.x * TPB;
     const int64_t n_vec = (VEC == 4) ? (n >> 2) : 0;
@@ -124,53 +60,28 @@
         char4 t4 = make_char4(0, 0, 0, 0);
         if (strand) t4 = __ldg(reinterpret_cast<const char4*>(strand) + v);
         uint4 gs, ge;
-        one(c4.x, s4.x, HAS_END ? (int64_t)e4.x : s4.x + wm1, t4.x, &gs.x, &ge.x);
-        one(c4.y, s4.y, HAS_END ? (int64_t)e4.y : s4.y + wm1, t4.y, &gs.y, &ge.y);
-        one(c4.z, s4.z, HAS_END ? (int64_t)e4.z : s4.z + wm1, t4.z, &gs.z, &ge.z);
-        one(c4.w, s4.w, HAS_END ? (int64_t)e4.w : s4.w + wm1, t4.w, &gs.w, &ge.w);
+        map_one(a, w, acc, c4.x, s4.x, HAS_END ? (int64_t)e4.x : s4.x + wm1, t4.x, &gs.x, &ge.x);
+        map_one(a, w, acc, c4.y, s4.y, HAS_END ? (int64_t)e4.y : s4.y + wm1, t4.y, &gs.y, &ge.y);
+        map_one(a, w, acc, c4.z, s4.z, HAS_END ? (int64_t)e4.z : s4.z + wm1, t4.z, &gs.z, &ge.z);
+        map_one(a, w, acc, c4.w, s4.w, HAS_END ? (int64_t)e4.w : s4.w + wm1, t4.w, &gs.w, &ge.w);
         reinterpret_cast<uint4*>(g_start)[v] = gs;
         reinterpret_cast<uint4*>(g_end1)[v] = ge;
         if (xs_out) reinterpret_cast<uint4*>(xs_out)[v] = gs;
         if (strand_out)
-            reinterpret_cast<char4*>(strand_out)[v] = make_char4(sgn(t4.x), sgn(t4.y), sgn(t4.z), sgn(t4.w));
+            reinterpret_cast<char4*>(strand_out)[v] =
+                make_char4(strand_sign(t4.x), strand_sign(t4.y), strand_sign(t4.z), strand_sign(t4.w));
     }
     for (int64_t i = n_vec * 4 + (int64_t)blockIdx.x * TPB + threadIdx.x; i < n; i += stride) {
         const int st = strand ? (int)strand[i] : 0;
         uint32_t gs, ge1;
-        one(chrom[i], start[i], HAS_END ? (int64_t)end[i] : (int64_t)start[i] + fixed_width - 1, st, &gs, &ge1);
+        map_one(a, w, acc, chrom[i], start[i], HAS_END ? (int64_t)end[i] : (int64_t)start[i] + fixed_width - 1, st,
+                &gs, &ge1);
         g_start[i] = gs;
         g_end1[i] = ge1;
         if (xs_out) xs_out[i] = gs;
-        if (strand_out) strand_out[i] = sgn(st);
-    }
-    __shared__ unsigned int sh[6];
-    if (threadIdx.x < 6) sh[threadIdx.x] = 0;
-    __syncthreads();
-    for (int d = 16; d > 0; d >>= 1) {
-        np += __shfl_xor_sync(0xffffffffu, np, d);
-        nm += __shfl_xor_sync(0xffffffffu, nm, d);
-        ns += __shfl_xor_sync(0xffffffffu, ns, d);
-        my_err |= __shfl_xor_sync(0xffffffffu, my_err, d);
-        wmax = max(wmax, __shfl_xor_sync(0xffffffffu, wmax, d));
-        nlong += __shfl_xor_sync(0xffffffffu, nlong, d);
-    }
-    if ((threadIdx.x & 31) == 0) {
-        if (nlong) atomicAdd(&sh[5], nlong);
-        atomicAdd(&sh[0], np);
-        atomicAdd(&sh[1], nm);
-        atomicAdd(&sh[2], ns);
-        atomicOr(&sh[3], my_err);
-        atomicMax(&sh[4], wmax);
-    }
-    __syncthreads();
-    if (threadIdx.x == 0) {
-        if (sh[0]) atomicAdd(&cls_count[0], (unsigned long long)sh[0]);
-        if (sh[1]) atomicAdd(&cls_count[1], (unsigned long long)sh[1]);
-        if (sh[2]) atomicAdd(&cls_count[2], (unsigned long long)sh[2]);
-        if (sh[3]) atomicOr(err, sh[3]);
-        if (sh[4]) atomicMax(&cls_count[3], (unsigned long long)sh[4]);
-        if (sh[5]) atomicAdd(exc.count + 2, sh[5]);
-    }
+        if (strand_out) strand_out[i] = strand_sign(st);
+    }
+    map_acc_commit(acc, a, err, cls_count);
 }
 
 __global__ void __launch_bounds__(TPB)
@@ -356,8 +267,11 @@
     dfree(r.pd_w);
     dfree(r.pd_run_first);
     r.pending = false;
+    r.map_pending = false;
+    dfree(r.mp_chrom_owned);
     dfree(r.d_chrom_len);
     dfree(r.d_chrom_off);
+    dfree(r.d_chrom_ol);
     dfree(r.d_len_na);
     dfree(r.g_start);
     dfree(r.g_end1);
@@ -475,6 +389,47 @@
     r.device_bytes += (size_t)r.n * (8 + (r.has_strand ? 1 : 0));
     r.pairs_built = true;
     return RCP_OK;
+}
+
+int reads_ensure_mapped(ReadsIdx& r) {
+    if (!r.map_pending) return RCP_OK;
+    r.map_pending = false;
+    StageTimer t(ST_INDEX_MAP);
+    ExcBuf exc;
+    exc.xw = r.exc_xw;
+    exc.e1 = r.exc_e1;
+    exc.st = r.exc_st;
+    exc.cap = r.pd_exc_cap;
+    exc.count = r.pd_w;
+    exc.w_out = r.pd_w + 1;
+    const MapArgs a = {r.d_chrom_ol, r.n_chrom, r.mp_frag_len, r.long_thr, exc};
+    auto al16 = [](const void* q) { return (reinterpret_cast<uintptr_t>(q) & 15u) == 0; };
+    const bool vec = al16(r.mp_chrom) && al16(r.mp_start) && (r.mp_end == nullptr || al16(r.mp_end)) &&
+                     (r.mp_strand == nullptr || (reinterpret_cast<uintptr_t>(r.mp_strand) & 3u) == 0);
+    const int64_t n = r.n;
+    const unsigned grid = grid_for(vec ? (n + 3) / 4 : n);
+    auto launch = [&](auto kern) {
+        kern<<<grid, TPB, 0, g_ctx.stream>>>(n, r.mp_chrom, r.mp_start, r.mp_end, r.mp_strand, r.mp_fixed_width, a,
+                                             r.g_start, r.g_end1, r.cls[CLS_ALL].xs, r.d_strand, r.pd_err,
+                                             r.pd_cnt);
+    };
+    if (r.mp_end) {
+        if (vec) launch(reads_to_global_kernel<4, true>);
+        else launch(reads_to_global_kernel<1, true>);
+    } else {
+        if (vec) launch(reads_to_global_kernel<4, false>);
+        else launch(reads_to_global_kernel<1, false>);
+    }
+    RCP_LAUNCHED();
+    r.mp_chrom = r.mp_start = r.mp_end = nullptr;
+    r.mp_strand = nullptr;
+    dfree(r.mp_chrom_owned);
+    return RCP_OK;
+}
+
+bool map_split_enabled() {
+    const char* v = getenv("RCP_MAP_SPLIT");
+    return v == nullptr || strcmp(v, "0") != 0;
 }
 
 __global__ void __launch_bounds__(TPB)
@@ -555,10 +510,16 @@
                                  cudaMemcpyHostToDevice, g_ctx.stream));
         RCP_CUDA(cudaMemcpyAsync(r.d_chrom_off, r.chrom_off.data(), ((size_t)n_chrom + 1) * 4,
                                  cudaMemcpyHostToDevice, g_ctx.stream));
+        r.h_chrom_ol.resize((size_t)n_chrom);
+        for (int c = 0; c < n_chrom; c++)
+            r.h_chrom_ol[(size_t)c] = make_uint2(r.chrom_off[(size_t)c], (uint32_t)r.chrom_len[(size_t)c]);
+        RCP_CUDA(cudaMemcpyAsync(r.d_chrom_ol, r.h_chrom_ol.data(), (size_t)n_chrom * 8, cudaMemcpyHostToDevice,
+                                 g_ctx.stream));
         return RCP_OK;
     };
     RCP_TRY(dalloc(&r.d_chrom_len, (size_t)n_chrom));
     RCP_TRY(dalloc(&r.d_chrom_off, (size_t)n_chrom + 1));
+    RCP_TRY(dalloc(&r.d_chrom_ol, (size_t)n_chrom));
     if (!r.any_na) RCP_TRY(layout());
 
     DevIn<int32_t> d_chrom, d_start, d_end, d_run_chrom, d_run_len;
@@ -627,40 +588,10 @@
         const int wbits = 32 - split_position_bits((int64_t)r.chrom_off[(size_t)n_chrom]) - (r.has_strand ? 2 : 0);
         r.long_thr = wbits >= 7 ? std::min<uint32_t>((1u << wbits) - 1u, 8191u) : 0xffffffffu;
     }
-    ExcBuf exc;
-    exc.cap = (uint32_t)std::min<int64_t>(std::max<int64_t>(n / 64, 4096), 65536);
-    RCP_TRY(dalloc(&r.exc_xw, (size_t)exc.cap));
-    RCP_TRY(dalloc(&r.exc_e1, (size_t)exc.cap));
-    RCP_TRY(dalloc(&r.exc_st, (size_t)exc.cap));
-    exc.xw = r.exc_xw;
-    exc.e1 = r.exc_e1;
-    exc.st = r.exc_st;
-    exc.count = d_w;
-    exc.w_out = d_w + 1;
-    const bool eager_index = g_ctx.coverage_path == RCP_PATH_INDEX;
-    if (eager_index) RCP_TRY(dalloc(&r.cls[CLS_ALL].xs, (size_t)n));
-    if (n > 0) {
-        StageTimer t(ST_INDEX_MAP);
-        auto al16 = [](const void* q) { return (reinterpret_cast<uintptr_t>(q) & 15u) == 0; };
-        const bool vec = al16(d_chrom.ptr) && al16(d_start.ptr) && (d_end.ptr == nullptr || al16(d_end.ptr)) &&
-                         (d_strand.ptr == nullptr || (reinterpret_cast<uintptr_t>(d_strand.ptr) & 3u) == 0);
-        const unsigned grid = grid_for(vec ? (n + 3) / 4 : n);
-        auto launch = [&](auto kern) {
-            kern<<<grid, TPB, 0, g_ctx.stream>>>(n, d_chrom.ptr, d_start.ptr, d_end.ptr, d_strand.ptr, r.d_chrom_off,
-                                                 r.d_chrom_len, n_chrom, frag_len, fixed_width, r.long_thr, r.g_start,
-                                                 r.g_end1,
-                                                 r.cls[CLS_ALL].xs, r.d_strand, d_err, d_cnt, exc);
-        };
-        if (d_end.ptr) {
-            if (vec) launch(reads_to_global_kernel<4, true>);
-            else launch(reads_to_global_kernel<1, true>);
-        } else {
-            if (vec) launch(reads_to_global_kernel<4, false>);
-            else launch(reads_to_global_kernel<1, false>);
-        }
-        RCP_LAUNCHED();
-    }
-    lap("map kernel enqueued");
+    const uint32_t exc_cap = (uint32_t)std::min<int64_t>(std::max<int64_t>(n / 64, 4096), 65536);
+    RCP_TRY(dalloc(&r.exc_xw, (size_t)exc_cap));
+    RCP_TRY(dalloc(&r.exc_e1, (size_t)exc_cap));
+    RCP_TRY(dalloc(&r.exc_st, (size_t)exc_cap));
     r.pending = true;
     r.pd_rle = rle;
     r.pd_err = d_err;
@@ -668,8 +599,29 @@
     r.pd_w = d_w;
     r.pd_run_first = run_first;
     r.pd_run_total = rle ? run_first + n_runs : nullptr;
-    r.pd_exc_cap = exc.cap;
+    r.pd_exc_cap = exc_cap;
+    const bool eager_index = g_ctx.coverage_path == RCP_PATH_INDEX;
     r.pd_eager_index = eager_index;
+    if (eager_index) RCP_TRY(dalloc(&r.cls[CLS_ALL].xs, (size_t)n));
+    r.mp_chrom = d_chrom.ptr;
+    r.mp_start = d_start.ptr;
+    r.mp_end = d_end.ptr;
+    r.mp_strand = d_strand.ptr;
+    r.mp_frag_len = frag_len;
+    r.mp_fixed_width = fixed_width;
+    r.map_pending = n > 0;
+    auto al16 = [](const void* q) { return (reinterpret_cast<uintptr_t>(q) & 15u) == 0; };
+    const bool defer_map = g_ctx.deferred_validation && !eager_index && !r.any_na && n > 0 &&
+                           mem == RCP_MEM_DEVICE && al16(d_chrom.ptr) && al16(d_start.ptr) &&
+                           (d_end.ptr == nullptr || al16(d_end.ptr)) &&
+                           (d_strand.ptr == nullptr || (reinterpret_cast<uintptr_t>(d_strand.ptr) & 3u) == 0);
+    if (defer_map) {
+        r.mp_chrom_owned = d_chrom.owned;
+        d_chrom.owned = nullptr;
+    } else {
+        RCP_TRY(reads_ensure_mapped(r));
+    }
+    lap("map kernel enqueued");
     r.device_bytes += (size_t)n * (8 + (r.has_strand ? 1 : 0));
     if (g_ctx.deferred_validation && !eager_index) return RCP_OK;
     RCP_TRY(reads_resolve(r));
@@ -687,6 +639,7 @@
 }
 
 int reads_resolve(ReadsIdx& r) {
+    RCP_TRY(reads_ensure_mapped(r));
     if (!r.pending) return RCP_OK;
     FetchItem items[4];
     int n = 0;
@@ -726,7 +679,7 @@
     if (h_err & 4u) return fail(RCP_ERR_DATA, "a read starts beyond the end of its chromosome");
     r.cls[CLS_PLUS].n = (int64_t)r.h_cnt[0];
     r.cls[CLS_MINUS].n = (int64_t)r.h_cnt[1];
-    r.cls[CLS_STAR].n = (int64_t)r.h_cnt[2];
+    r.cls[CLS_STAR].n = n - (int64_t)r.h_cnt[0] - (int64_t)r.h_cnt[1];
     r.max_width = (uint32_t)r.h_cnt[3];
     r.n_long = (int64_t)r.h_w[2];
     if (r.pd_eager_index) RCP_TRY(reads_build_class(r, CLS_ALL));
@@ -842,6 +795,7 @@
     if (rc == RCP_OK)
         rc = reads_load_impl(r, m, o_chrom, 0, nullptr, nullptr, o_start, o_end, o_strand, n_chrom, chrom_len,
                              frag_len, RCP_MEM_DEVICE, 0);
+    if (rc == RCP_OK) rc = reads_ensure_mapped(r);
     dfree(flag);
     dfree(rank);
     dfree(kept_pos);
diff --git a/recoup_b200/csrc/rcp_internal.cuh b/recoup_b200/csrc/rcp_internal.cuh
--- a/recoup_b200/csrc/rcp_internal.cuh
+++ b/recoup_b200/csrc/rcp_internal.cuh
@@ -182,8 +182,10 @@
     int key_bits = 32;
     std::vector<int64_t> chrom_len;
     std::vector<uint32_t> chrom_off;
+    std::vector<uint2> h_chrom_ol;
     int64_t* d_chrom_len = nullptr;
     uint32_t* d_chrom_off = nullptr;
+    uint2* d_chrom_ol = nullptr;
     bool any_na = false;
     std::vector<uint8_t> len_na;
     uint8_t* d_len_na = nullptr;
@@ -217,6 +219,13 @@
     uint32_t* pd_run_first = nullptr;
     uint32_t pd_exc_cap = 0;
     bool pd_eager_index = false;
+    bool map_pending = false;
+    const int32_t* mp_chrom = nullptr;
+    const int32_t* mp_start = nullptr;
+    const int32_t* mp_end = nullptr;
+    const int8_t* mp_strand = nullptr;
+    int32_t* mp_chrom_owned = nullptr;
+    int mp_frag_len = 0, mp_fixed_width = 0;
     unsigned int h_err = 0, h_w[4] = {0, 0, 0, 0}, h_total = 0;
     uint32_t long_thr = 0;
     int64_t n_long = 0;
@@ -232,6 +241,8 @@
 int reads_pending_items(ReadsIdx& r, FetchItem* items, int* n);
 int reads_finish(ReadsIdx& r);
 int reads_resolve(ReadsIdx& r);
+int reads_ensure_mapped(ReadsIdx& r);
+bool map_split_enabled();
 
 int reads_build_class(ReadsIdx& r, int cls);
 int reads_build_pairs(ReadsIdx& r);
diff --git a/recoup_b200/csrc/reads_map.cuh b/recoup_b200/csrc/reads_map.cuh
--- /dev/null
+++ b/recoup_b200/csrc/reads_map.cuh
@@ -0,0 +1,119 @@
+#pragma once
+#include <stdint.h>
+
+namespace rcp {
+
+struct ExcBuf {
+    uint32_t* xw;
+    uint32_t* e1;
+    int8_t* st;
+    uint32_t cap;
+    unsigned int* count;
+    uint32_t* w_out;
+};
+
+struct MapArgs {
+    const uint2* chrom_ol;
+    int n_chrom;
+    int frag_len;
+    uint32_t long_thr;
+    ExcBuf exc;
+};
+
+constexpr unsigned int MAP_EXC_FULL = 0x80000000u;
+struct MapAcc {
+    unsigned int err = 0, np = 0, nm = 0, wmax = 0, nlong = 0;
+};
+
+__device__ __forceinline__ bool map_read(int c, int64_t s, int64_t e, int st, int n_chrom,
+                                         const uint2* __restrict__ chrom_ol, int frag_len,
+                                         uint32_t* gs, uint32_t* ge1, unsigned int* err) {
+    if (c < 0 || c >= n_chrom) { *err |= 1u; return false; }
+    if (s < 1 || e < s) { *err |= 2u; return false; }
+    const uint2 ol = __ldg(chrom_ol + c);
+    const int64_t len = ol.y;
+    if (frag_len > 0) {
+        if (st < 0) s = e - frag_len + 1;
+        else e = s + frag_len - 1;
+    }
+    if (s < 1) s = 1;
+    if (e > len) e = len;
+    if (s > len || e < s) { *err |= 4u; return false; }
+    *gs = ol.x + (uint32_t)s;
+    *ge1 = ol.x + (uint32_t)e + 1u;
+    return true;
+}
+
+template <bool HAS_END>
+__device__ __forceinline__ uint32_t map_candidate_width(const MapArgs& a, const int32_t* __restrict__ chrom,
+                                                        const int32_t* __restrict__ start,
+                                                        const int32_t* __restrict__ end,
+                                                        const int8_t* __restrict__ strand, int fixed_width) {
+    uint32_t w = (uint32_t)a.frag_len;
+    if (a.frag_len <= 0) {
+        uint32_t x = 0, y = 0;
+        unsigned int e0 = 0;
+        if (map_read(chrom[0], start[0], HAS_END ? (int64_t)end[0] : (int64_t)start[0] + fixed_width - 1,
+                     strand ? (int)strand[0] : 0, a.n_chrom, a.chrom_ol, 0, &x, &y, &e0))
+            w = y - x;
+    }
+    return w;
+}
+
+__device__ __forceinline__ int8_t strand_sign(int st) { return (int8_t)(st > 0 ? 1 : (st < 0 ? -1 : 0)); }
+
+__device__ __forceinline__ void map_one(const MapArgs& a, uint32_t w, MapAcc& acc, int c, int s, int64_t e, int st,
+                                        uint32_t* gs, uint32_t* ge1) {
+    *gs = 0;
+    *ge1 = 0;
+    if (map_read(c, s, e, st, a.n_chrom, a.chrom_ol, a.frag_len, gs, ge1, &acc.err)) {
+        acc.wmax = max(acc.wmax, *ge1 - *gs);
+        acc.nlong += (*ge1 - *gs > a.long_thr);
+        if (*ge1 - *gs != w && !(acc.err & MAP_EXC_FULL)) {
+            if (*reinterpret_cast<volatile unsigned int*>(a.exc.count) > a.exc.cap) {
+                acc.err |= MAP_EXC_FULL;
+            } else {
+                const unsigned int k = atomicAdd(a.exc.count, 1u);
+                if (k < a.exc.cap) {
+                    a.exc.xw[k] = *gs + w;
+                    a.exc.e1[k] = *ge1;
+                    a.exc.st[k] = strand_sign(st);
+                }
+            }
+        }
+    }
+    acc.np += st > 0;
+    acc.nm += st < 0;
+}
+
+__device__ __forceinline__ void map_acc_commit(MapAcc& acc, const MapArgs& a, unsigned int* __restrict__ err,
+                                               unsigned long long* __restrict__ cls_count) {
+    __shared__ unsigned int sh[6];
+    if (threadIdx.x < 6) sh[threadIdx.x] = 0;
+    acc.err &= ~MAP_EXC_FULL;
+    __syncthreads();
+    for (int d = 16; d > 0; d >>= 1) {
+        acc.np += __shfl_xor_sync(0xffffffffu, acc.np, d);
+        acc.nm += __shfl_xor_sync(0xffffffffu, acc.nm, d);
+        acc.err |= __shfl_xor_sync(0xffffffffu, acc.err, d);
+        acc.wmax = max(acc.wmax, __shfl_xor_sync(0xffffffffu, acc.wmax, d));
+        acc.nlong += __shfl_xor_sync(0xffffffffu, acc.nlong, d);
+    }
+    if ((threadIdx.x & 31) == 0) {
+        if (acc.nlong) atomicAdd(&sh[5], acc.nlong);
+        atomicAdd(&sh[0], acc.np);
+        atomicAdd(&sh[1], acc.nm);
+        atomicOr(&sh[3], acc.err);
+        atomicMax(&sh[4], acc.wmax);
+    }
+    __syncthreads();
+    if (threadIdx.x == 0) {
+        if (sh[0]) atomicAdd(&cls_count[0], (unsigned long long)sh[0]);
+        if (sh[1]) atomicAdd(&cls_count[1], (unsigned long long)sh[1]);
+        if (sh[3]) atomicOr(err, sh[3]);
+        if (sh[4]) atomicMax(&cls_count[3], (unsigned long long)sh[4]);
+        if (sh[5]) atomicAdd(a.exc.count + 2, sh[5]);
+    }
+}
+
+}
```

Measured after the change: 50.99 billion, median of 6. 0.975x the previous value.
